# LiangZhaoPKUImperial/LinearSFM

Measured on AMD Instinct MI355X. Metric: hierarchical linear map-joining solve wall-clock, NC3500-like stereo (all transforms + joins), lower is better.
Workload: dtype f64

## Files before the change

### linearsfm_amd/csrc/lsfm_chol.hip

```cpp
#include <algorithm>
#include <climits>
#include <cmath>
#include <cstdlib>
#include <numeric>

#include "lsfm_device.hpp"
#include "lsfm_symbolic.hpp"
#include "lsfm_chol.hpp"

namespace lsfm {

#define FX_ONE 0x1p61
#define FX_INV 0x1p-61
__device__ __forceinline__ long long fx_from(double v) { return __double2ll_rn(fmin(fmax(v, -2.0), 2.0) * FX_ONE); }
__device__ __forceinline__ double fx_to(long long a) { return (double)a * FX_INV; }
__device__ __forceinline__ void fx_atomic_sub(double* slot, double t)
{
	__hip_atomic_fetch_add(reinterpret_cast<unsigned long long*>(slot), (unsigned long long)fx_from(-t), __ATOMIC_RELAXED, __HIP_MEMORY_SCOPE_AGENT);
}
__device__ __forceinline__ int scale_exp(double d)
{
	if (!(d > 0) || !(d < 1e300)) return 0;
	return (__builtin_amdgcn_frexp_exp(d) + 1) >> 1;
}
// ... 1076 lines not shown
	{
		const int k0 = 6 * t;
		if (tid >= k0 && tid < k0 + 6) sA[tid - k0] = acc;
		__syncthreads();
		if (tid >= k0 && tid < k0 + 6)
		{
			const int c = tid - k0;
			double x = 0.0;
			for (int k = c; k < 6; k++) x = fma(sDi[t * 36 + k * 6 + c], sA[k], x);
			sX[tid] = x;
		}
		__syncthreads();
		if (tid < k0)
		{
#pragma unroll
			for (int k = 0; k < 6; k++) acc = fma(-Ls[(k0 + k) * SN_XS + tid], sX[k0 + k], acc);
		}
	}
	if (tid < n6) v[(size_t)c0 * 6 + tid] = sX[tid];
}

__global__ void k_to_float(size_t n, const double* __restrict__ a, float* __restrict__ b)
{
	size_t i = (size_t)blockIdx.x * blockDim.x + threadIdx.x;
	if (i < n) b[i] = (float)a[i];
}

__global__ void k_perm_in(int M, const int* __restrict__ perm, const double* __restrict__ r, const unsigned char* __restrict__ fixed,
                          const double* __restrict__ dscale, double* __restrict__ v, int zero_from)
{
	size_t i = (size_t)blockIdx.x * blockDim.x + threadIdx.x;
	if (i >= (size_t)M * 6) return;
	const size_t src = (size_t)perm[i / 6] * 6 + i % 6;
	v[i] = ((fixed && fixed[src]) || (long)(i / 6) >= (long)zero_from) ? 0.0 : r[src] * dscale[i];
}
__global__ void k_perm_out_dot(int M, const int* __restrict__ pinv, const double* __restrict__ v, const double* __restrict__ r,
                               const unsigned char* __restrict__ fixed, const double* __restrict__ dscale, const int* __restrict__ pose_seg,
                               double* __restrict__ z, double* dot, int dot_stride, const int* __restrict__ col_owner, int rank)
{
	int row = blockIdx.x * blockDim.x + threadIdx.x;
	const bool ok = row < M;
	double acc = 0;
	int sg = 0;
	if (ok)
	{
		sg = pose_seg[row];
		const double* src = v + (size_t)pinv[row] * 6;
		const double* sc = dscale + (size_t)pinv[row] * 6;
		for (int i = 0; i < 6; i++)
		{
			double zz = src[i] * sc[i];
			if (fixed && fixed[(size_t)row * 6 + i]) zz = 0.0;
			if (col_owner) { const int ow = col_owner[pinv[row]]; if (!(ow == rank || (ow < 0 && rank == 0))) zz = 0.0; }
			z[(size_t)row * 6 + i] = zz;
			acc = fma(zz, r[(size_t)row * 6 + i], acc);
		}
	}
	if (dot) wave_scatter_add<1>(dot + (size_t)sg * dot_stride, &acc, ok);
}
__global__ void k_rz_dot(int M, const double* __restrict__ z, const double* __restrict__ r, const int* __restrict__ pose_seg, double* dot, int dot_stride)
{
	int row = blockIdx.x * blockDim.x + threadIdx.x;
	const bool ok = row < M;
	double acc = 0;
	int sg = 0;
	if (ok)
	{
		sg = pose_seg[row];
		for (int i = 0; i < 6; i++) acc = fma(z[(size_t)row * 6 + i], r[(size_t)row * 6 + i], acc);
	}
	wave_scatter_add<1>(dot + (size_t)sg * dot_stride, &acc, ok);
}

void chol_fetch(lsfm_context* ctx, const SchurSystem& sy, const int* d_origin, CholHostIn& in)
{
	const int M = sy.M, nnzb = sy.nnzb;
	in.keys.resize(nnzb);
	in.origin.resize(M);
	if (d_origin) LSFM_CHECK_HIP(hipMemcpyAsync(in.origin.data(), d_origin, (size_t)M * sizeof(int), hipMemcpyDeviceToHost, ctx->stream));
	else std::iota(in.origin.begin(), in.origin.end(), 0);
	d2h(ctx, in.keys.data(), sy.upper_keys, (size_t)nnzb * sizeof(unsigned long long));
}

void chol_alloc_values(lsfm_context* ctx, CholDev& ch)
{
	Arena& sc = ctx->scratch;
	ch.L = sc.alloc<double>((size_t)ch.nnzL * 36); ch.Dinv = sc.alloc<double>((size_t)ch.M * 36);
	ch.wv = sc.alloc<double>((size_t)ch.M * 6);
	ch.diag0 = sc.alloc<double>((size_t)ch.M * 6);
	ch.dscale = sc.alloc<double>((size_t)ch.M * 6);
	ch.Lg = ch.ngroups ? sc.alloc<double>((size_t)ch.nnzL * 36) : nullptr;
	dev_zero(ctx, ch.L, (size_t)ch.nnzL * 36 * sizeof(double));
	static const bool digest = getenv("LSFM_FACTOR_DIGEST") != nullptr;
	if (digest && ch.Lg) dev_zero(ctx, ch.Lg, (size_t)ch.nnzL * 36 * sizeof(double));
	ch.d_err = sc.alloc<int>(1);
	dev_zero(ctx, ch.d_err, sizeof(int));
}

static size_t chol_task_lds(const CholDev& ch) { return (size_t)ch.task0_maxsize * CHOL_TASK_LDS_PER_COL + 8; }
void chol_upload_index(lsfm_context* ctx, const CholSymbolic& sym, CholDev& ch)
{
	Arena& sc = ctx->scratch;
	ch.M = sym.M; ch.nnzL = sym.nnzL; ch.nlevels = sym.nlevels; ch.tail_begin = sym.tail_begin;
	ch.level_ptr = sym.level_ptr;
	if (!sym.tlevel_ptr.empty())
	{
		ch.ntask0 = sym.tlevel_ptr[1]; ch.ncol0 = sym.tlevel_col0[1];
		ch.task0_maxsize = sym.tlevel_maxsize[0]; ch.task0_lds = sym.tlevel_small_lds[0]; ch.task0_outer = sym.tlevel_outer[0];
		if (sym.tlevel_nsmall[0] != ch.ntask0 || chol_task_lds(ch) > CHOL_SOLVE_LDS)
			LSFM_FAIL(LSFM_ERR_INTERNAL, "a leaf task of the factorisation does not fit LDS (" + std::to_string(sym.tlevel_nsmall[0]) + " of " + std::to_string(ch.ntask0) +
			                                 " fit, " + std::to_string(ch.task0_maxsize) + " columns at most)");
	}
	ch.ngroups = sym.ngroups; ch.glevel_ptr = sym.glevel_ptr; ch.glevel_maxnr = sym.glevel_maxnr; ch.glevel_maxs = sym.glevel_maxs;
	ch.work_total = sym.work_total; ch.work_shared = sym.work_shared;
	ch.first_shared = sym.first_shared; ch.shared_blk0 = sym.colptr[sym.first_shared]; ch.glevel_owned = sym.glevel_owned; ch.glevel_shared = sym.glevel_shared;
	const struct { int** dst; const std::vector<int>* v; } parts[] = {
		{ &ch.grp_c0, &sym.grp_c0 }, { &ch.grp_s, &sym.grp_s }, { &ch.grp_nr, &sym.grp_nr }, { &ch.col_nin, &sym.col_nin }, { &ch.col_task, &sym.col_task },
		{ &ch.col_lpos, &sym.col_lpos }, { &ch.task_cols, &sym.task_cols }, { &ch.task_ptr, &sym.task_ptr }, { &ch.colptr, &sym.colptr },
		{ &ch.rowidx, &sym.rowidx }, { &ch.perm, &sym.perm }, { &ch.pinv, &sym.pinv }, { &ch.order, &sym.order }, { &ch.col_owner, &sym.col_owner } };
	size_t total = 0;
	for (const auto& pt : parts) total += pt.v->size();
	static thread_local std::vector<int> blob;
	blob.resize(total);
	int* d_blob = sc.alloc<int>(total);
	size_t off = 0;
	for (const auto& pt : parts)
	{
		if (!pt.v->empty()) memcpy(blob.data() + off, pt.v->data(), pt.v->size() * sizeof(int));
		*pt.dst = pt.v->empty() ? nullptr : d_blob + off;
		off += pt.v->size();
	}
	h2d(ctx, d_blob, blob.data(), total * sizeof(int));
	ch.blob = d_blob; ch.blob_ints = total;
}
void chol_upload_symbolic(lsfm_context* ctx, const CholSymbolic& sym, CholDev& ch)
{
	chol_upload_index(ctx, sym, ch);
	chol_alloc_values(ctx, ch);
	if (getenv("LSFM_DEBUG") && sym.ngroups > 50)
	{
		int hist[CHOL_GS + 1] = { 0 };
		for (int g = 0; g < sym.ngroups; g++) hist[sym.grp_s[g]]++;
		fprintf(stderr, "[lsfm] groups %d, group levels %d, sizes:", sym.ngroups, (int)sym.glevel_ptr.size() - 1);
		for (int q = 1; q <= CHOL_GS; q++) fprintf(stderr, " %d", hist[q]);
		fprintf(stderr, " | groups per level:");
		for (size_t l = 0; l + 1 < sym.glevel_ptr.size(); l++) fprintf(stderr, " %d", sym.glevel_ptr[l + 1] - sym.glevel_ptr[l]);
		fprintf(stderr, "\n");
	}
}
void chol_analyse(lsfm_context* ctx, const SchurSystem& sy, const CholHostIn& in, CholDev& ch)
{
	static thread_local CholSymbolic sym;
	chol_symbolic(in.keys.data(), sy.nnzb, in.origin.data(), sy.M, sym, ctx->comm ? ctx->comm->block_maps : 0);
	chol_upload_symbolic(ctx, sym, ch);
}

bool chol_distributed(const lsfm_context* ctx, const CholDev& ch)
{
	return ctx->comm && ctx->comm->world > 1 && ch.col_owner && ch.first_shared < ch.M;
}
static void comm_sum(lsfm_context* ctx, void* p, size_t count, int dtype)
{
	if (!count) return;
	Comm& cm = *ctx->comm;
	const size_t mk = cm.off;
	void* b = cm.alloc_bytes(count * 8);
	LSFM_CHECK_HIP(hipMemcpyAsync(b, p, count * 8, hipMemcpyDeviceToDevice, ctx->stream));
	cm.allreduce(ctx->stream, b, count, dtype);
	LSFM_CHECK_HIP(hipMemcpyAsync(p, b, count * 8, hipMemcpyDeviceToDevice, ctx->stream));
	cm.off = mk;
}
void comm_sum_host(lsfm_context* ctx, long long* h, int n)
{
	hipStream_t s = ctx->stream;
	Comm& cm = *ctx->comm;
	const size_t mk = cm.off;
	long long* d = cm.alloc<long long>(n);
	LSFM_CHECK_HIP(hipMemcpyAsync(d, h, n * sizeof(long long), hipMemcpyHostToDevice, s));
	LSFM_CHECK_HIP(hipStreamSynchronize(s));
// ... 226 lines not shown
```

### linearsfm_amd/csrc/lsfm_chol.hpp

```cpp
#pragma once
#include <vector>

#include "lsfm_internal.hpp"
#include "lsfm_solve.hpp"

namespace lsfm {

struct CholDev {
	int M = 0, nnzL = 0, nlevels = 0, tail_begin = 0;
	int* colptr = nullptr;
	int* rowidx = nullptr;
	int* perm = nullptr;
	int* pinv = nullptr;
	int* order = nullptr;
	std::vector<int> level_ptr;
	int* task_cols = nullptr;
	int* task_ptr = nullptr;
	int* col_task = nullptr;
	int* col_lpos = nullptr;
	int* col_nin = nullptr;
	int ntask0 = 0, ncol0 = 0;
	int task0_maxsize = 0;
	int task0_lds = 0;
	int task0_outer = 0;
	int ngroups = 0;
	int *grp_c0 = nullptr, *grp_s = nullptr, *grp_nr = nullptr;
	std::vector<int> glevel_ptr;
	std::vector<int> glevel_maxnr;
	std::vector<int> glevel_maxs;
	int sn_fused_levels = 0, sn_split_levels = 0;
	int* col_owner = nullptr;
	int first_shared = 0, shared_blk0 = 0;
	double work_total = 0, work_shared = 0;
	std::vector<char> glevel_owned, glevel_shared;
	int* blob = nullptr;
	size_t blob_ints = 0;
	float *Lf = nullptr, *Dinvf = nullptr;
	double* wv = nullptr;
	double* Lg = nullptr;
	float* Lgf = nullptr;
	double* L = nullptr;
	double* Dinv = nullptr;
	double* diag0 = nullptr;
	double* dscale = nullptr;
	int* d_err = nullptr;
};

struct OwnFilter {
	const int* col_owner = nullptr;
	int want = 0;
	__device__ __forceinline__ bool skip(int col) const { return col_owner && col_owner[col] != want; }
};
__device__ __forceinline__ int find_row(const int* __restrict__ rowidx, int lo, int hi, int target)
{
	while (lo < hi) { int mid = (lo + hi) >> 1; if (rowidx[mid] < target) lo = mid + 1; else hi = mid; }
	return lo;
}


struct CholSymbolic;
struct CholHostIn {
	std::vector<unsigned long long> keys;
	std::vector<int> origin;
};

void chol_fetch(lsfm_context* ctx, const SchurSystem& sy, const int* d_origin, CholHostIn& in);
void chol_analyse(lsfm_context* ctx, const SchurSystem& sy, const CholHostIn& in, CholDev& ch);
void chol_upload_index(lsfm_context* ctx, const CholSymbolic& sym, CholDev& ch);
void chol_upload_symbolic(lsfm_context* ctx, const CholSymbolic& sym, CholDev& ch);
void chol_alloc_values(lsfm_context* ctx, CholDev& ch);
void chol_scatter(lsfm_context* ctx, const SchurSystem& sy, const unsigned char* fixed, CholDev& ch);
void chol_factor(lsfm_context* ctx, const SchurSystem& sy, const unsigned char* fixed, CholDev& ch, double* fwd_v = nullptr);
void chol_merge_groups(lsfm_context* ctx, const CholDev& ch);
void chol_round_to_float(lsfm_context* ctx, CholDev& ch);
void chol_perm_in(lsfm_context* ctx, const CholDev& ch, const double* r, const unsigned char* fixed, double* v);
void chol_apply(lsfm_context* ctx, const CholDev& ch, const double* r, double* v, double* z, const unsigned char* fixed, const int* pose_seg, double* dot, int dot_stride, bool fwd_done = false);
bool chol_distributed(const lsfm_context* ctx, const CholDev& ch);
void comm_sum_host(lsfm_context* ctx, long long* h, int n);

}
```

### linearsfm_amd/csrc/lsfm_internal.hpp

```cpp
#pragma once
#include <hip/hip_runtime.h>

#include <cstdint>
#include <cstdio>
#include <condition_variable>
#include <cstring>
#include <exception>
#include <functional>
#include <memory>
#include <mutex>
#include <thread>
#include <string>
#include <vector>

#include "../../include/lsfm.h"

namespace lsfm {

struct Error { int code; std::string msg; };
struct DevBatch;
struct IndexHold;
struct SolvePlan;
struct PreLevel;
struct EarlyPattern;
// ... 131 lines not shown
			th = std::thread([this] {
				std::unique_lock<std::mutex> lk(m);
				for (;;)
				{
					cv.wait(lk, [&] { return quit || (busy && job); });
					if (quit) return;
					std::function<void()> j = std::move(job);
					job = nullptr;
					lk.unlock();
					std::exception_ptr e;
					try { j(); } catch (...) { e = std::current_exception(); }
					lk.lock();
					err = e; busy = false;
					cv.notify_all();
				}
			});
		cv.notify_all();
	}
	void wait()
	{
		std::unique_lock<std::mutex> l(m);
		cv.wait(l, [&] { return !busy; });
		if (err) { std::exception_ptr e = err; err = nullptr; std::rethrow_exception(e); }
	}
};

}

namespace lsfm {
struct Roctx {
	int (*push)(const char*) = nullptr;
	int (*pop)() = nullptr;
	void (*mark)(const char*) = nullptr;
	Roctx();
};
Roctx& roctx();
struct Range {
	bool on;
	explicit Range(const char* name) : on(roctx().push != nullptr) { if (on) roctx().push(name); }
	~Range() { if (on) roctx().pop(); }
	Range(const Range&) = delete;
	Range& operator=(const Range&) = delete;
};
}

struct lsfm_context {
	int device = 0;
	hipStream_t stream = nullptr;
	lsfm::Arena arena[3];
	lsfm::Arena scratch;
	int cur = 0;
	size_t arena_bytes = 0, arena_req = 0;
	lsfm::PcgOptions pcg;
	int covcols_panel = 0;
	int small_max = 5;
	std::string last_error;
	int* h_pinned = nullptr;
	char* h_stage = nullptr;
	char* d_stage = nullptr;
	size_t stage_size = 0, stage_off = 0;
	hipEvent_t ev_half[2] = { nullptr, nullptr };
	hipEvent_t ev0 = nullptr, ev1 = nullptr, ev2 = nullptr, ev3 = nullptr;
	hipEvent_t evs[4] = { nullptr, nullptr, nullptr, nullptr };
	unsigned long long generation = 0;
	hipStream_t stream2 = nullptr;
	hipEvent_t evA = nullptr, evB = nullptr;
	bool pattern_dep = false;
	const lsfm::DevBatch* tr_in = nullptr;
	const int* tr_hub = nullptr;
	std::shared_ptr<lsfm::EarlyPattern> early;
	hipEvent_t ev_k9[2] = { nullptr, nullptr };
	hipStream_t stream3 = nullptr;
	lsfm::Arena sarena[2];
	std::shared_ptr<lsfm::PreLevel> pre;
	lsfm::LevelPlan pre_plan;
	int pre_plan_level = -1;
	std::unique_ptr<lsfm::HostWorker> worker;
	void drop_prepared() { pre.reset(); pre_plan = lsfm::LevelPlan(); pre_plan_level = -1; }
	hipEvent_t ev_solve_end = nullptr;
	double dbg_gap_ms = 0.0;
	hipEvent_t evY = nullptr, evP = nullptr;
	hipEvent_t evU = nullptr;
	hipEvent_t evK = nullptr;
	const unsigned long long* solved_keys = nullptr;
	int solved_nnzb = 0;
	std::vector<std::pair<const char*, double>> timeline;
	bool timeline_on = false;
	void mark(const char* what);
	bool in_tree_run = false;
	int inject_level = -1;
	bool level_syncs = false;
	int step_hint = 0, steps_used = 0;
	hipEvent_t evC = nullptr;
	lsfm_stats* stats = nullptr;
	lsfm::LevelPlan* plan = nullptr;
	bool warm() const { return plan && plan->valid; }
	lsfm::RunStatsDev* d_run = nullptr;
	lsfm::Comm* comm = nullptr;
	std::vector<hipEvent_t> ev_pool;
	size_t ev_next = 0;
	struct Timed { hipEvent_t a, b; double* sink; };
	std::vector<Timed> timed;
	hipEvent_t pool_event();
	void defer_time(hipEvent_t a, hipEvent_t b, double* sink) { timed.push_back(Timed{ a, b, sink }); }
	void flush_times();
	void ensure_arenas(size_t bytes_each, bool start_small = false);
	bool grow_arenas();
	bool arena_small = false;
	size_t arena_bound = 0;
};

namespace lsfm {

struct OnStream {
	lsfm_context* c; hipStream_t& s; Arena* a;
	OnStream(lsfm_context* ctx, hipStream_t& other, Arena* arena = nullptr) : c(ctx), s(other), a(arena) { std::swap(c->stream, s); if (a) std::swap(c->scratch, *a); }
	~OnStream() { if (a) std::swap(c->scratch, *a); std::swap(c->stream, s); }
	OnStream(const OnStream&) = delete;
	OnStream& operator=(const OnStream&) = delete;
};

void dev_exclusive_scan(lsfm_context* ctx, const int* in, int* out, size_t n);
void dev_sort_pairs_u64(lsfm_context* ctx, unsigned long long* keys, int* vals, size_t n, int end_bit, int begin_bit = 0);
void dev_sort_keys_u64(lsfm_context* ctx, const unsigned long long* keys, unsigned long long* sorted, size_t n, int begin_bit, int end_bit);
int d2h_int(lsfm_context* ctx, const int* dptr);
void d2h_ints(lsfm_context* ctx, const int* dptr, int* h, size_t n);
void h2d(lsfm_context* ctx, void* d, const void* h, size_t bytes);
struct HostPiece { const void* p; size_t bytes; };
void h2d_gather(lsfm_context* ctx, void* d, const std::vector<HostPiece>& pieces);
struct CopyBatch {
	lsfm_context* ctx;
	struct Item { void* dst; const void* src; size_t bytes; bool host; };
	std::vector<Item> items;
	explicit CopyBatch(lsfm_context* c) : ctx(c) {}
	void h2d(void* d, const void* h, size_t bytes) { if (bytes) items.push_back(Item{ d, h, bytes, true }); }
	void d2d(void* d, const void* s, size_t bytes) { if (bytes) items.push_back(Item{ d, s, bytes, false }); }
	void flush();
};
void d2h(lsfm_context* ctx, void* h, const void* d, size_t bytes);
void dev_zero(lsfm_context* ctx, void* d, size_t bytes);
void fill_async(hipStream_t s, void* d, int byte, size_t bytes);

void batch_upload(lsfm_context* ctx, Arena& ar, const lsfm_map* maps, int N, bool mono, DevBatch& out);
void batch_download_map(lsfm_context* ctx, const DevBatch& b, int k, bool mono, lsfm_map* out);
template <class T> inline T* host_alloc(size_t n) { return static_cast<T*>(malloc((n ? n : 1) * sizeof(T))); }
struct CopyBatch;
void batch_set_offsets(lsfm_context* ctx, Arena& ar, DevBatch& b, CopyBatch* cb = nullptr);
void batch_fill_maps(lsfm_context* ctx, DevBatch& b);
struct PackHeader {
	int magic, version, mono, m, n, nU, nW, Ref, FRef, ScaP, Fix, Sign, FScaP, FFix, pad0, pad1;
	unsigned long long total;
	unsigned long long off[12];
	unsigned long long pad[11];
};
static_assert(sizeof(PackHeader) == 256, "the header is the first 256 bytes of a pack");
#define LSFM_PACK_MAGIC 0x4d46534c
size_t pack_layout(PackHeader& h);
void batch_pack_map(lsfm_context* ctx, const DevBatch& b, int k, bool mono, void* dst, size_t cap);
void batch_slice_counts(lsfm_context* ctx, const DevBatch& b, int nslices, std::vector<int>& nf, std::vector<int>& nw);
void batch_pack_slice(lsfm_context* ctx, const DevBatch& b, bool mono, int nslices, int slice, int nf, int nw, void* dst, size_t cap);
void batch_unpack_maps(lsfm_context* ctx, Arena& ar, const void* const* packed, const PackHeader* hdr, int N, bool mono, DevBatch& out);
unsigned long long batch_structure_digest(lsfm_context* ctx, const DevBatch& b);

inline bool map_in_frame(const DevBatch& X, int b, int tref, int tscap, bool mono) { return X.Ref[b] == tref && (!mono || X.ScaP[b] == tscap); }
int level_targets(const DevBatch& X, bool mono, std::vector<int>& tref, std::vector<int>& tscap, std::vector<int>& tfix);
struct TrRedirect {
	const int* wbase = nullptr;
	const int* newf = nullptr;
	double* W = nullptr;
	int *photo = nullptr, *feature = nullptr, *srcf = nullptr;
};
void transform_batch(lsfm_context* ctx, Arena& ar, const DevBatch& in, const std::vector<int>& target_ref,
                     const std::vector<int>& target_scap, const std::vector<int>& target_fix, bool mono, DevBatch& out,
                     bool alias_passthrough = false, const std::function<TrRedirect(DevBatch&)>* hook = nullptr);

struct JoinWork;
void join_batch_stereo(lsfm_context* ctx, Arena& ar, const DevBatch& in, DevBatch& out, double* eP_out, double* eF_out);
void join_batch_mono(lsfm_context* ctx, Arena& ar, const DevBatch& in, DevBatch& out, double* eP_out, double* eF_out);

struct SolveIO {
	int M = 0, NF = 0, NU = 0, NW = 0, nseg = 0;
	const int* d_pose_seg = nullptr;
	const int* d_feat_seg = nullptr;
	const unsigned char* d_seg_active = nullptr;
	const double* U = nullptr; const int *Ui = nullptr, *Uj = nullptr;
	const double* W = nullptr; const int *photo = nullptr, *fptr = nullptr;
	const double* V = nullptr;
	const double* ea = nullptr;
	const double* eb = nullptr;
	const double* x0 = nullptr;
	const unsigned char* d_fixed = nullptr;
	const int* d_pose_origin = nullptr;
	double* x_pose = nullptr;
	double* x_feat = nullptr;
	std::vector<int> seg_rows;
	const int *d_pose_off = nullptr, *d_feat_off = nullptr, *d_u_off = nullptr;
	const struct RhsFused* rhs = nullptr;
	const struct PatternSeed* seed = nullptr;
};
int small_level_strips(const lsfm_context* ctx, int most_rows);
inline int most_rows(const std::vector<int>& seg_rows) { int most = 0; for (int r : seg_rows) most = r > most ? r : most; return most; }
inline int small_level_strips(const lsfm_context* ctx, const std::vector<int>& seg_rows) { return small_level_strips(ctx, most_rows(seg_rows)); }
void small_level_offsets(lsfm_context* ctx, const DevBatch& out, SolveIO& io);
void small_solve_launch(lsfm_context* ctx, const SolveIO& io, int strips, int* status, double* max_rel);
int solve_batch(lsfm_context* ctx, const SolveIO& io);
int gn_polish(lsfm_context* ctx, const lsfm_map* maps, int N, bool mono, lsfm_map* x, int iters, int kind, double c, double* obj, double* gnorm,
              int* halvings, double* chi2, double* weight);
int map_chi2(lsfm_context* ctx, const lsfm_map* maps, int N, bool mono, const lsfm_map* x, double* chi2, int* dof);
int gn_linearise(lsfm_context* ctx, const lsfm_map* maps, int N, bool mono, const lsfm_map* x, const double* weight, lsfm_map* out, double* obj,
                 double* b, double* times, int* counts);
int map_covariance(lsfm_context* ctx, const lsfm_map* map, bool mono, double* pose_cov, double* feat_cov, double* pair_cov, int cap_blocks, int* nnzb,
                   double* times);
int map_covariance_columns(lsfm_context* ctx, const lsfm_map* map, bool mono, const int* poses, int k, double* pose_cols, double* feat_cols, double* joint,
                           int* steps, double* last_corr, double* times);
int inverse_v(lsfm_context* ctx, double* V, int n);
int solve_features(lsfm_context* ctx, const double* W, const double* IV, const double* eb, const double* dpa, double* dpb, int m, int n, const int* mapCor,
                   const int* photo);
bool no_timing_events();
#define LSFM_REC_T(e, s) do { if (!lsfm::no_timing_events()) LSFM_CHECK_HIP(hipEventRecord(e, s)); } while (0)
unsigned timing_event_flags();
unsigned order_event_flags();
void prefetch_next_level(lsfm_context* ctx, const DevBatch& Y, const std::vector<int>& target_ref, int next_level, int step_hint);
int spmv_external(lsfm_context* ctx, int m, const int* rowptr, const int* colidx, const double* val, const double* x, double* y, int reps,
                  double* avg_ms, double* bytes);
int chol_selftest(lsfm_context* ctx, int m, const int* rowptr, const int* colidx, const double* val, const int* origin, const unsigned char* fixed,
                  const int* pose_seg, int nseg, const double* r, int nrhs, int mode, double* z, double* dot, int* perm, int* colptr, int* rowidx,
                  double* L, double* Dinv, double* dscale, int cap_blocks, int* info);

int wstream_bench(lsfm_context* ctx, long long nblocks, int mode, int reps, double* avg_ms);
int prims_selftest(lsfm_context* ctx, int cases, unsigned seed);
}
```

### linearsfm_amd/csrc/lsfm_join.hip

```cpp
#include "lsfm_device.hpp"
#include "lsfm_internal.hpp"
#include <climits>
#include "lsfm_join.hpp"
#include "lsfm_solve.hpp"

namespace lsfm {

__device__ __forceinline__ unsigned long long jh_mix(unsigned long long x)
{
	x ^= x >> 33; x *= 0xff51afd7ed558ccdull; x ^= x >> 33; x *= 0xc4ceb9fe1a85ec53ull; x ^= x >> 33;
	return x;
}
__global__ void k_join_hash_insert(int NF, const int* __restrict__ feat_id, const int* __restrict__ feat_map, unsigned long long* tab,
                                   int* __restrict__ tval, unsigned long long mask)
{
	int f = blockIdx.x * blockDim.x + threadIdx.x;
	if (f >= NF) return;
	const int mp = feat_map[f];
	if (mp & 1) return;
	const unsigned long long key = ((unsigned long long)(mp >> 1) << 32) | (unsigned)feat_id[f];
	unsigned long long h = jh_mix(key) & mask;
	for (;;)
	{
		const unsigned long long old = atomicCAS(&tab[h], ~0ull, key);
// ... 275 lines not shown
		const int nun = pair ? rb[b + 1] - rb[b] : 0;
		out.feat_off[g + 1] = jg.FY0 + jg.nE + nun;
		out.pose_off[g] = in.pose_off[a]; out.u_off[g] = in.u_off[a]; out.w_off[g] = in.w_off[a];
		out.Ref[g] = pair ? in.Ref[b] : in.Ref[a];
		out.FRef[g] = in.FRef[a];
		seg_active[g] = pair ? 1 : 0;
		seg_rows[g] = (pair ? in.pose_off[b + 1] : in.pose_off[a + 1]) - in.pose_off[a];
	}
	out.pose_off[G] = in.M; out.u_off[G] = in.NU; out.w_off[G] = in.NW;
	out.NF = out.feat_off[G];
	const int NFY = out.NF;

	CopyBatch cb(ctx);
	JGroup* d_grp = ctx->scratch.alloc<JGroup>(G);
	cb.h2d(d_grp, grp.data(), sizeof(JGroup) * G);

	out.pose = ar.alloc<double>((size_t)in.M * 6);
	out.pose_id = ar.alloc<int>(in.M);
	out.pose_origin = ar.alloc<int>(in.M);
	cb.d2d(out.pose_origin, in.pose_origin, (size_t)in.M * sizeof(int));
	out.feat = ar.alloc<double>((size_t)NFY * 3);
	out.feat_id = ar.alloc<int>(NFY);
	out.U = ar.alloc<double>((size_t)in.NU * 36); out.Ui = ar.alloc<int>(in.NU); out.Uj = ar.alloc<int>(in.NU);
	out.W = ar.alloc<double>((size_t)in.NW * 18); out.photo = ar.alloc<int>(in.NW); out.feature = ar.alloc<int>(in.NW);
	out.fptr = ar.alloc<int>(NFY + 1);
	out.V = ar.alloc<double>((size_t)NFY * 9);
	batch_set_offsets(ctx, ar, out, &cb);
	cb.d2d(out.pose_id, in.pose_id, (size_t)in.M * sizeof(int));
	st.d_act = reinterpret_cast<unsigned char*>(ctx->scratch.alloc<int>((G + 3) / 4 + 1));
	st.act_padded.assign(((size_t)G + 3) / 4 * 4, 0);
	std::copy(seg_active.begin(), seg_active.end(), st.act_padded.begin());
	cb.h2d(st.d_act, st.act_padded.data(), st.act_padded.size());
	cb.flush();
	batch_fill_maps(ctx, out);
	int* newf = st.newf = ctx->scratch.alloc<int>(in.NF + 1);
	int* lens = ctx->scratch.alloc<int>(NFY + 2);
	st.srcf = ctx->scratch.alloc<int>(in.NW + 1);
	int* lenE = st.lenE = ctx->scratch.alloc<int>(NFY + 1);
	int* lenC = ctx->scratch.alloc<int>(NFY + 1);
	double* eF = st.eF = ctx->scratch.alloc<double>((size_t)NFY * 3);
	double* eP = st.eP = ctx->scratch.alloc<double>((size_t)in.M * 6);
	dev_zero(ctx, eP, (size_t)in.M * 6 * sizeof(double));
	const bool small_level = small_level_strips(ctx, seg_rows) > 0;
	const bool early = !small_level && !ctx->comm && !(ctx->pre && !ctx->pre_plan.valid) && ctx->tr_in && ctx->tr_hub && !ctx->warm() && ctx->tr_in->NF == in.NF && ctx->tr_in->M == in.M;
	st.fuse_rhs = !small_level && !ctx->comm && !ctx->pcg.mixed;
	int *srcE = nullptr, *srcC = nullptr;
	if (early || st.fuse_rhs)
	{
		srcE = ctx->scratch.alloc<int>(NFY + 1); srcC = ctx->scratch.alloc<int>(NFY + 1);
	}
	st.srcE = srcE; st.srcC = srcC;
	if (in.NF)
		for (int side = 0; side < 2; side++)
			hipLaunchKernelGGL(k_join_features, dim3(nb), dim3(256), 0, s, in.NF, in.feat_map, in.feat_id, in.feat, in.V, in.fptr, match, R, d_grp,
			                   newf, lenE, lenC, out.V, eF, out.feat_id, out.feat, srcE, srcC, side);
	if (early)
	{
		const DevBatch& X = *ctx->tr_in;
		EarlyPatternIn ei;
		ei.M = in.M; ei.NFY = NFY; ei.NU = X.NU;
		ei.Ui = X.Ui; ei.Uj = X.Uj; ei.pose_map = X.pose_map; ei.hub = ctx->tr_hub;
		ei.fptr = X.fptr; ei.photo = X.photo; ei.feat_map = X.feat_map; ei.srcE = srcE; ei.srcC = srcC;
		LSFM_CHECK_HIP(hipEventRecord(ctx->evC, s));
		schur_pattern_early_issue(ctx, ei);
	}
	else schur_pattern_early_drop(ctx);
	hipLaunchKernelGGL(k_add_lens, dim3((NFY + 256) / 256), dim3(256), 0, s, NFY, lenE, lenC, lens);
	dev_exclusive_scan(ctx, lens, out.fptr, NFY);
	if (early) LSFM_CHECK_HIP(hipEventRecord(ctx->evC, s));
	st.wbase = ctx->scratch.alloc<int>(in.NF + 1);
	if (in.NF) hipLaunchKernelGGL(k_join_wbase, dim3(nb), dim3(256), 0, s, in.NF, in.feat_map, newf, lenE, out.fptr, st.wbase);
	LSFM_CHECK_HIP(hipGetLastError());
	ctx->mark("jn_prep");
}

void join_stereo_finish(lsfm_context* ctx, const DevBatch& in, DevBatch& out, JoinState& st, double* eP_out, double* eF_out)
{
	hipStream_t s = ctx->stream;
	const int G = out.B, NFY = out.NF;
	double *eP = st.eP, *eF = st.eF;
	int* srcf = st.srcf;
	const std::vector<unsigned char>& seg_active = st.seg_active;
	const std::vector<int>& seg_rows = st.seg_rows;
	if (in.NU)
	{
		CopyBatch cu(ctx);
		cu.d2d(out.U, in.U, (size_t)in.NU * 36 * sizeof(double));
		cu.d2d(out.Ui, in.Ui, (size_t)in.NU * sizeof(int));
		cu.d2d(out.Uj, in.Uj, (size_t)in.NU * sizeof(int));
		cu.flush();
	}
	LSFM_CHECK_HIP(hipEventRecord(ctx->evY, s));
	if (!eP_out && !eF_out && !ctx->early && !ctx->comm)
	{
		LSFM_CHECK_HIP(hipEventRecord(ctx->evA, s));
		ctx->pattern_dep = true;
	}
	const bool fuse_rhs = st.fuse_rhs && !eP_out && !eF_out;
	if (NFY && !fuse_rhs)
		hipLaunchKernelGGL(k_join_rhs_w, dim3((NFY + RHS_TILE - 1) / RHS_TILE), dim3(256), 0, s, NFY, out.fptr, out.W, out.photo, srcf, in.pose, in.feat, eP, eF);
	if (in.NU && (!ctx->comm || ctx->comm->rank == 0))
		hipLaunchKernelGGL(k_join_rhs_u, dim3((in.NU + 127) / 128), dim3(128), 0, s, in.NU, in.U, in.Ui, in.Uj, in.pose, eP);
	LSFM_CHECK_HIP(hipGetLastError());
	if (eP_out) d2h(ctx, eP_out, eP, (size_t)in.M * 6 * sizeof(double));
	if (eF_out) d2h(ctx, eF_out, eF, (size_t)NFY * 3 * sizeof(double));

	unsigned char* d_act = st.d_act;
	SolveIO io;
	io.M = in.M; io.NF = NFY; io.NU = in.NU; io.NW = in.NW; io.nseg = G;
	io.d_pose_seg = out.pose_map; io.d_feat_seg = out.feat_map; io.d_seg_active = d_act;
	io.U = out.U; io.Ui = out.Ui; io.Uj = out.Uj; io.W = out.W; io.photo = out.photo; io.fptr = out.fptr; io.V = out.V;
	io.ea = eP; io.eb = eF; io.x0 = in.pose; io.d_fixed = nullptr; io.d_pose_origin = out.pose_origin;
	io.x_pose = out.pose; io.x_feat = out.feat;
	io.seg_rows = seg_rows;
	RhsFused rhs;
	if (fuse_rhs)
	{
		rhs.srcE = st.srcE; rhs.srcC = st.srcC; rhs.feat_src = in.feat; rhs.pose_src = in.pose; rhs.pose_map_src = in.pose_map;
		io.rhs = &rhs;
	}
	small_level_offsets(ctx, out, io);
	const bool warm = ctx->warm();
	ctx->solved_keys = nullptr; ctx->solved_nnzb = 0;
	int rc = solve_batch(ctx, io);
	if (!warm && !ctx->in_tree_run) LSFM_CHECK_HIP(hipStreamSynchronize(s));
	ctx->scratch.release(st.smark);
	if (rc > 0 && ctx->stats) ctx->stats->not_converged += rc;
	if (ctx->plan && !eP_out && !eF_out) ctx->plan->valid = true;
}

void join_batch_stereo(lsfm_context* ctx, Arena& ar, const DevBatch& in, DevBatch& out, double* eP_out, double* eF_out)
{
	JoinState st;
	join_stereo_prepare(ctx, ar, in, out, st);
	if (in.NW)
		hipLaunchKernelGGL(k_join_wcopy, dim3((in.NW + 255) / 256), dim3(256), 0, ctx->stream, in.NW, in.W, in.photo, in.feature, in.fptr, st.wbase,
		                   st.newf, out.W, out.photo, out.feature, st.srcf, in.W_alias, in.d_alias, in.feat_map);
	join_stereo_finish(ctx, in, out, st, eP_out, eF_out);
}

}
```

### linearsfm_amd/csrc/lsfm_level.hip

```cpp
#include <algorithm>
#include <chrono>
#include <cmath>
#include <cstdlib>

#include "lsfm_device.hpp"
#include "lsfm_symbolic.hpp"
#include "lsfm_pcg.hpp"

namespace lsfm {

struct SolvePlan {
	SchurSystem sy;
	CholDev ch;
	int its = 1;
	bool mixed = false;
	double rel_tol = 0;
	bool small = false;
	char* mem = nullptr;
	~SolvePlan() { if (mem) (void)hipFree(mem); }
};
static std::shared_ptr<SolvePlan> solve_plan_store(lsfm_context* ctx, const SchurSystem& sy, const CholDev& ch, int its)
{
	auto sp = std::make_shared<SolvePlan>();
	const size_t M = sy.M, nnzb = sy.nnzb, cap = (size_t)sy.mask + 1;
// ... 93 lines not shown
		PreLevel* raw = pl.get();
		ctx->worker->run([raw]() { chol_symbolic(raw->hin.keys.data(), raw->sy.nnzb, raw->hin.origin.data(), raw->sy.M, raw->sym); });
		pl->worker = ctx->worker.get();
		ctx->mark("pre_sym");
		pl->whole = whole; pl->level = next_level; pl->its = step_hint;
		ctx->pre = pl;
	}
	if (!whole) return;
	const int B = Y.B;
	ctx->pre_plan.tr_cnt.assign(counts.begin(), counts.begin() + 2 * (B + 1));
	ctx->pre_plan.join_rb.assign(counts.begin() + 2 * (B + 1), counts.end());
	ctx->pre_plan.solve.reset();
	ctx->pre_plan.idx = kept;
	ctx->pre_plan.valid = true;
	ctx->pre_plan_level = next_level;
	ctx->mark("pre_plan");
}
static std::shared_ptr<SolvePlan> pre_plan_complete(lsfm_context* ctx, PreLevel& pl)
{
	pl.wait();
	auto sp = std::make_shared<SolvePlan>();
	sp->sy = pl.sy;
	sp->its = pl.its; sp->mixed = ctx->pcg.mixed; sp->rel_tol = ctx->pcg.rel_tol;
	{
		OnStream on(ctx, ctx->stream3, &ctx->sarena[pl.level & 1]);
		chol_upload_index(ctx, pl.sym, sp->ch);
		LSFM_CHECK_HIP(hipEventRecord(ctx->evP, ctx->stream));
	}
	LSFM_CHECK_HIP(hipStreamWaitEvent(ctx->stream, ctx->evP, 0));
	return sp;
}

__global__ void k_dbg_absstats(size_t n, const double* __restrict__ a, double* __restrict__ out)
{
	double s = 0.0, m = 0.0;
	for (size_t i = (size_t)blockIdx.x * blockDim.x + threadIdx.x; i < n; i += (size_t)gridDim.x * blockDim.x)
	{
		const double v = fabs(a[i]);
		s += v; if (v > m || !(v == v)) m = v == v ? v : 1e300;
	}
	atomic_add_f64(out, s);
	atomicMax(reinterpret_cast<unsigned long long*>(out + 1), (unsigned long long)__double_as_longlong(m));
}
__global__ void k_dbg_dinv(int M, const double* __restrict__ Dinv, const double* __restrict__ diag0, const int* __restrict__ colptr, int first_group_col)
{
	int j = blockIdx.x * blockDim.x + threadIdx.x;
	if (j >= M) return;
	double m = 0.0;
	for (int q = 0; q < 36; q++) m = fmax(m, fabs(Dinv[(size_t)j * 36 + q]));
	if (m > 1e3 || !(m == m))
		printf("[lsfm conv] column %d (%s, %d blocks): max |Dinv| %.3e, Dinv diag %.3e %.3e %.3e %.3e %.3e %.3e, diag0 %.3e %.3e %.3e %.3e %.3e %.3e\n", j,
		       j >= first_group_col ? "group" : "leaf", colptr[j + 1] - colptr[j], m, Dinv[(size_t)j * 36], Dinv[(size_t)j * 36 + 7], Dinv[(size_t)j * 36 + 14],
		       Dinv[(size_t)j * 36 + 21], Dinv[(size_t)j * 36 + 28], Dinv[(size_t)j * 36 + 35], diag0[j * 6], diag0[j * 6 + 1], diag0[j * 6 + 2], diag0[j * 6 + 3],
		       diag0[j * 6 + 4], diag0[j * 6 + 5]);
}
__global__ void k_digest(size_t n, const unsigned long long* __restrict__ a, unsigned long long* out)
{
	unsigned long long h = 0;
	for (size_t i = (size_t)blockIdx.x * blockDim.x + threadIdx.x; i < n; i += (size_t)gridDim.x * blockDim.x)
	{
		unsigned long long b = a[i];
		if (b == 0x8000000000000000ull) b = 0;
		b ^= b >> 31; b *= 0x9E3779B97F4A7C15ull * (2 * (unsigned long long)i + 1); b ^= b >> 29;
		h += b;
	}
	atomicAdd(out, h);
}
__global__ void k_digest_compare(const unsigned long long* d, int* mismatch)
{
	if (d[0] != d[1]) atomicAdd(mismatch, 1);
}
__global__ void k_chol_err_to_run(const int* err, RunStatsDev* run)
{
	if (*err && !run->chol_err) run->chol_err = *err;
}

struct LevelStructure {
	SchurSystem sy;
	CholDev ch;
	SolvePlan* sp = nullptr;
	double tw0 = 0, tw1 = 0;
};
static double wall_ms() { return std::chrono::duration<double, std::milli>(std::chrono::steady_clock::now().time_since_epoch()).count(); }
static LevelStructure level_structure(lsfm_context* ctx, const SolveIO& io, SolvePlan* sp, PreLevel* pre, bool pending, hipEvent_t eb)
{
	hipStream_t s = ctx->stream;
	LevelStructure ls;
	SchurSystem& sy = ls.sy;
	CholDev& ch = ls.ch;
	const bool pattern_dep = ctx->pattern_dep;
	ctx->pattern_dep = false;
	auto assemble = [&]() {
		build_schur_values(ctx, io, sy);
		LSFM_REC_T(eb, s); if (roctx().mark) roctx().mark("lsfm factor + refine: begin");
		LSFM_CHECK_HIP(hipEventRecord(ctx->evK, s));
	};
	if (sp || pending)
	{
		sy = pending ? pre->sy : sp->sy;
		schur_vinv(ctx, io, sy);
		assemble();
		if (pending)
		{
			ctx->mark("k9_enq");
			ctx->plan->solve = pre_plan_complete(ctx, *pre);
			sp = ctx->plan->solve.get();
			ctx->mark("sym_wait");
		}
		ls.sp = sp;
		ch = sp->ch;
		chol_alloc_values(ctx, ch);
		return ls;
	}
	schur_vinv(ctx, io, sy);
	CholHostIn hin;
	bool have = false;
	if (pre && !(pre->M == io.M && !ctx->comm)) pre = nullptr;
	if (pre)
	{
		schur_pattern_early_drop(ctx);
		SchurSystem prepared = pre->sy;
		prepared.IV = sy.IV; prepared.LY = sy.LY; prepared.ymax = sy.ymax; prepared.uu = sy.uu;
		sy = prepared;
		have = true;
		LSFM_CHECK_HIP(hipStreamWaitEvent(s, ctx->evP, 0));
		if (getenv("LSFM_CHECK_EARLY_PATTERN")) schur_pattern_check(ctx, io, sy, "prefetched");
	}
	else if (ctx->early && !ctx->comm)
	{
		LSFM_CHECK_HIP(hipStreamWaitEvent(ctx->stream3, ctx->evC, 0));
		{
			OnStream on(ctx, ctx->stream3);
			ctx->mark("sv_start");
			have = schur_pattern_early_finish(ctx, io, sy);
			ctx->mark("pat_fin");
			if (have)
			{
				if (getenv("LSFM_CHECK_EARLY_PATTERN")) schur_pattern_check(ctx, io, sy, "early");
				chol_fetch(ctx, sy, io.d_pose_origin, hin);
				ctx->mark("fetch");
				schur_pattern_early_extras(ctx, sy);
				LSFM_CHECK_HIP(hipEventRecord(ctx->evB, ctx->stream));
			}
		}
		if (have) LSFM_CHECK_HIP(hipStreamWaitEvent(s, ctx->evB, 0));
	}
	else if (pattern_dep && !ctx->comm)
	{
		LSFM_CHECK_HIP(hipStreamWaitEvent(ctx->stream2, ctx->evA, 0));
		{
			OnStream on(ctx, ctx->stream2);
			build_schur_pattern(ctx, io, sy);
			chol_fetch(ctx, sy, io.d_pose_origin, hin);
			LSFM_CHECK_HIP(hipEventRecord(ctx->evB, ctx->stream));
		}
		LSFM_CHECK_HIP(hipStreamWaitEvent(s, ctx->evB, 0));
		have = true;
	}
	if (!have)
	{
		build_schur_pattern(ctx, io, sy);
		chol_fetch(ctx, sy, io.d_pose_origin, hin);
	}
	assemble();
	ls.tw0 = wall_ms();
	ctx->mark("k9_enq");
	if (pre) { pre->wait(); chol_upload_symbolic(ctx, pre->sym, ch); }
	else chol_analyse(ctx, sy, hin, ch);
	ctx->mark("analyse");
	ls.tw1 = wall_ms();
	return ls;
}

static int solve_level_dense(lsfm_context* ctx, const SolveIO& io, int strips, bool warm, hipEvent_t eb, hipEvent_t ec, hipEvent_t ed)
{
	hipStream_t s = ctx->stream;
	LevelPlan* lp = ctx->plan;
	ctx->pattern_dep = false;
	if (!warm) schur_pattern_early_drop(ctx);
	int* d_small = nullptr;
	auto enqueue = [&]() {
		d_small = ctx->scratch.alloc<int>(4);
		dev_zero(ctx, d_small, 4 * sizeof(int));
		hipEvent_t esm0 = nullptr, esm1 = nullptr;
		if (ctx->stats) { esm0 = ctx->pool_event(); esm1 = ctx->pool_event(); LSFM_REC_T(esm0, s); }
		small_solve_launch(ctx, io, strips, d_small, reinterpret_cast<double*>(d_small + 2));
		if (ctx->stats) { LSFM_REC_T(esm1, s); ctx->defer_time(esm0, esm1, &ctx->stats->t_small_ms); ctx->stats->small_levels++; }
	};
	if (!warm) enqueue();
	LSFM_REC_T(eb, s); if (warm && roctx().mark) roctx().mark("lsfm factor + refine: begin");
	LSFM_CHECK_HIP(hipEventRecord(ctx->evK, s));
	if (warm) enqueue();
	LSFM_REC_T(ec, s);
	LSFM_REC_T(ed, s); if (roctx().mark) roctx().mark("lsfm solve: end");
	ctx->ev_solve_end = ed;
	ctx->solved_keys = nullptr; ctx->solved_nnzb = 0;
	if (ctx->stats) ctx->stats->pcg_iterations += 1;
	ctx->steps_used = 1;
	const bool deferred = ctx->in_tree_run && ctx->d_run && (warm || !lp || lp == &ctx->pre_plan);
	if (deferred) return 0;
// ... 6 lines not shown
	if (lp && !lp->solve && hs[0] == 0)
	{
		auto small_plan = std::make_shared<SolvePlan>();
		small_plan->its = 1; small_plan->mixed = false; small_plan->rel_tol = ctx->pcg.rel_tol; small_plan->small = true;
		lp->solve = small_plan;
	}
	return hs[0];
}

static void factor_digest_check(lsfm_context* ctx, const SolveIO& io, const SchurSystem& sy, CholDev& ch)
{
	static const bool digest = getenv("LSFM_FACTOR_DIGEST") != nullptr;
	if (!digest || !ctx->d_run) return;
	hipStream_t s = ctx->stream;
	Arena& sc = ctx->scratch;
	const int M = io.M;
	auto dg = [&](const double* a, size_t n, unsigned long long* out) {
		if (a && n) hipLaunchKernelGGL(k_digest, dim3(256), dim3(256), 0, s, n, reinterpret_cast<const unsigned long long*>(a), out);
	};
	dg(sy.S, (size_t)sy.nnzb * 36, &ctx->d_run->s_digest);
	if (!ctx->comm)
	{
		SchurSystem sy2 = sy;
		build_schur_values(ctx, io, sy2);
		unsigned long long* d = sc.alloc<unsigned long long>(2);
		dev_zero(ctx, d, 2 * sizeof(unsigned long long));
		dg(sy.S, (size_t)sy.nnzb * 36, d); dg(sy.E, (size_t)M * 6, d);
		dg(sy2.S, (size_t)sy.nnzb * 36, d + 1); dg(sy2.E, (size_t)M * 6, d + 1);
		hipLaunchKernelGGL(k_digest_compare, dim3(1), dim3(1), 0, s, d, &ctx->d_run->s_rebuild_mismatch);
	}
	auto factor_digest = [&](unsigned long long* out) {
		dg(ch.Dinv, (size_t)ch.M * 36, out);
		dg(ch.L, (size_t)ch.nnzL * 36, out);
		if (ch.Lg) dg(ch.Lg, (size_t)ch.nnzL * 36, out);
	};
	factor_digest(&ctx->d_run->factor_digest);
	if (!ctx->comm)
	{
		unsigned long long* d = sc.alloc<unsigned long long>(2);
		dev_zero(ctx, d, 2 * sizeof(unsigned long long));
		factor_digest(d);
		dev_zero(ctx, ch.L, (size_t)ch.nnzL * 36 * sizeof(double));
		if (ch.Lg) dev_zero(ctx, ch.Lg, (size_t)ch.nnzL * 36 * sizeof(double));
		chol_scatter(ctx, sy, io.d_fixed, ch);
		chol_factor(ctx, sy, io.d_fixed, ch, nullptr);
		factor_digest(d + 1);
		hipLaunchKernelGGL(k_digest_compare, dim3(1), dim3(1), 0, s, d, &ctx->d_run->refactor_mismatch);
	}
}

static void debug_conv(lsfm_context* ctx, const SolveIO& io, const SchurSystem& sy, const CholDev& ch, const PcgSeg* seg)
{
	hipStream_t s = ctx->stream;
	const int M = io.M;
	hipLaunchKernelGGL(k_pcg_debug, dim3((io.nseg + 127) / 128), dim3(128), 0, s, io.nseg, M, seg);
	if (!(M > 10000 && io.nseg == 1)) return;
	double* d = ctx->scratch.alloc<double>(12);
	dev_zero(ctx, d, 12 * sizeof(double));
	auto st = [&](const double* a, size_t n, int k) { if (a && n) hipLaunchKernelGGL(k_dbg_absstats, dim3(512), dim3(256), 0, s, n, a, d + 2 * k); };
	st(sy.S, (size_t)sy.nnzb * 36, 0); st(sy.E, (size_t)M * 6, 1); st(ch.L, (size_t)ch.nnzL * 36, 2); st(ch.Lg, (size_t)ch.nnzL * 36, 3);
	st(ch.Dinv, (size_t)ch.M * 36, 4); st(io.x_pose, (size_t)M * 6, 5);
	hipLaunchKernelGGL(k_dbg_dinv, dim3((ch.M + 255) / 256), dim3(256), 0, s, ch.M, ch.Dinv, ch.diag0, ch.colptr, 0);
	double h[12];
	d2h(ctx, h, d, sizeof h);
	fprintf(stderr, "[lsfm conv] root M=%d: |S| sum %.15e max %.6e  |E| sum %.15e  |L| sum %.12e max %.3e  |Lg| sum %.12e max %.3e  |Dinv| sum %.6e max %.3e  |x| sum %.12e max %.3e\n",
	        M, h[0], h[1], h[2], h[4], h[5], h[6], h[7], h[8], h[9], h[10], h[11]);
}

int solve_batch(lsfm_context* ctx, const SolveIO& io)
{
	hipStream_t s = ctx->stream;
	const int M = io.M;
	LevelPlan* lp = ctx->plan;
	const int strips = (io.d_pose_off && io.d_feat_off && io.d_u_off) ? small_level_strips(ctx, io.seg_rows) : 0;
	SolvePlan* sp = lp ? lp->solve.get() : nullptr;
	if (sp && sp->small != (strips > 0)) { lp->solve.reset(); sp = nullptr; }
	std::shared_ptr<PreLevel> pre = std::move(ctx->pre);
	const bool pending = !strips && !sp && pre && pre->whole && lp == &ctx->pre_plan;
	if (pre && !pending && (strips || sp || pre->whole || pre->M != M || ctx->comm)) pre.reset();
	const bool warm = sp != nullptr || pending;
	hipEvent_t ea = ctx->pool_event(), eb = ctx->pool_event(), ec = ctx->pool_event(), ed = ctx->pool_event();
	LSFM_REC_T(ea, s); if (roctx().mark) roctx().mark("lsfm schur: begin");
	if (strips) return solve_level_dense(ctx, io, strips, warm, eb, ec, ed);
	LevelStructure ls = level_structure(ctx, io, sp, pre.get(), pending, eb);
	pre.reset();
	const SchurSystem& sy = ls.sy;
	CholDev& ch = ls.ch;
	sp = ls.sp;
	const bool dbg = getenv("LSFM_DEBUG") != nullptr;
	PcgWork w = pcg_begin(ctx, io, sy, ch);
	if (ctx->stats && chol_distributed(ctx, ch)) { ctx->stats->dist_solves++; ctx->stats->dist_work_total += ch.work_total; ctx->stats->dist_work_shared += ch.work_shared; }
	chol_scatter(ctx, sy, io.d_fixed, ch);
	if (w.fused_fwd) chol_perm_in(ctx, ch, w.r, io.d_fixed, w.v);
	chol_factor(ctx, sy, io.d_fixed, ch, w.fused_fwd ? w.v : nullptr);
	if (ctx->pcg.mixed) chol_round_to_float(ctx, ch);
	factor_digest_check(ctx, io, sy, ch);
	if (dbg) { LSFM_CHECK_HIP(hipStreamSynchronize(s)); }
	const double tw2 = wall_ms();
	const bool deferred = warm || (ctx->in_tree_run && ctx->d_run && !lp);
	ctx->solved_keys = sy.upper_keys; ctx->solved_nnzb = sy.nnzb;
	const PcgSteps steps{ warm, deferred, sp ? sp->its : 0, sp ? sp->mixed : false, sp ? sp->rel_tol : 0.0 };
	const PcgResult res = pcg_run(ctx, io, sy, ch, w, steps);
	if (dbg)
	{
		LSFM_CHECK_HIP(hipStreamSynchronize(s));
		fprintf(stderr, "[lsfm] solve M=%d nseg=%d nnzb=%d nnzL=%d etree levels=%d tail=%d leaf tasks=%d group levels=%d %s| analyse %.2f ms, factor %.2f ms, cg(%d its) %.2f ms\n", M, io.nseg,
		        sy.nnzb, ch.nnzL, ch.nlevels, ch.M - ch.tail_begin, ch.ntask0, (int)ch.glevel_ptr.size() - 1, warm ? "(plan) " : "", ls.tw1 - ls.tw0, tw2 - ls.tw1, res.its, wall_ms() - tw2);
	}
	if (ctx->comm)
	{
		Comm& cm = *ctx->comm;
		const size_t nscal = (size_t)M * 6;
		double *x = io.x_pose, *xb = cm.alloc<double>(nscal);
		if (cm.rank == 0) LSFM_CHECK_HIP(hipMemcpyAsync(xb, x, nscal * sizeof(double), hipMemcpyDeviceToDevice, s));
		else fill_async(s, xb, 0, nscal * sizeof(double));
		cm.allreduce(s, xb, nscal, LSFM_DTYPE_F64);
		LSFM_CHECK_HIP(hipMemcpyAsync(x, xb, nscal * sizeof(double), hipMemcpyDeviceToDevice, s));
	}
	pcg_final_residual(ctx, io, sy, w);
	LSFM_REC_T(ec, s); if (roctx().mark) roctx().mark("lsfm back-substitution: begin");
	launch_backsub(ctx, io, sy, io.x_pose);
	LSFM_CHECK_HIP(hipGetLastError());
	LSFM_REC_T(ed, s); if (roctx().mark) roctx().mark("lsfm solve: end");
	ctx->ev_solve_end = ed;
	if (ctx->stats)
	{
		lsfm_stats* st = ctx->stats;
		ctx->defer_time(ea, eb, &st->t_schur_ms);
		ctx->defer_time(eb, ec, &st->t_pcg_ms);
		ctx->defer_time(ec, ed, &st->t_backsub_ms);
		ctx->defer_time(w.es0, w.es1, &st->spmv_ms);
		st->pcg_iterations += res.its;
		st->spmv_launches += 1;
		st->spmv_bytes += spmv_bytes(sy);
		st->spmv_nnzb_upper_last = sy.nnzb; st->spmv_rows_last = M;
	}
	ctx->steps_used = res.planned ? 0 : std::max(res.its, 1);
	if (deferred)
	{
		if (warm && !res.planned) { sp->its = std::max(res.its, 1); sp->mixed = ctx->pcg.mixed; sp->rel_tol = ctx->pcg.rel_tol; }
		static const bool dbg_conv = getenv("LSFM_DEBUG_CONV") != nullptr;
		if (dbg_conv) debug_conv(ctx, io, sy, ch, w.seg);
		hipLaunchKernelGGL(k_pcg_run_stats, dim3((io.nseg + 127) / 128), dim3(128), 0, s, io.nseg, w.seg, ctx->d_run);
		return 0;
	}
	double maxrel = 0;
	int notconv = pcg_read_verdict(ctx, io, w, &maxrel);
	if (ctx->stats) ctx->stats->max_rel_residual = std::max(ctx->stats->max_rel_residual, maxrel);
	if (ctx->comm)
	{
		long long hv[2] = { notconv, 0 };
		comm_sum_host(ctx, hv, 2);
		notconv = (int)((hv[0] + ctx->comm->world - 1) / ctx->comm->world);
	}
	if (lp && !lp->solve && notconv == 0) lp->solve = solve_plan_store(ctx, sy, ch, std::max(res.its, 1));
	return notconv;
}

}
```

### linearsfm_amd/csrc/lsfm_pcg.hip

```cpp
#include <algorithm>
#include <cmath>
#include <cstdlib>

#include "lsfm_device.hpp"
#include "lsfm_pcg.hpp"

namespace lsfm {

struct PcgSeg {
	double rz[2];
	double pAp;
	double rr, ee, thresh, rr_prev;
	int done, its, row0, active;
	int slow, pad;
};
static_assert(sizeof(PcgSeg) % sizeof(double) == 0, "PcgSeg is strided in doubles by the fused dot products");
#define SEG_STRIDE ((int)(sizeof(PcgSeg) / sizeof(double)))

__global__ void k_x_init(int M, const double* __restrict__ x0, const unsigned char* __restrict__ fixed, double* __restrict__ x, double* __restrict__ y, int* __restrict__ misc)
{
	size_t i = (size_t)blockIdx.x * blockDim.x + threadIdx.x;
	if (i < 4) misc[i] = 0;
	if (i >= (size_t)M * 6) return;
	y[i] = 0.0;
// ... 45 lines not shown
__global__ void k_copy(size_t n, const double* __restrict__ a, double* __restrict__ b)
{
	size_t i = (size_t)blockIdx.x * blockDim.x + threadIdx.x;
	if (i < n) b[i] = a[i];
}

__global__ void k_pcg_update1(int M, int cur, const int* __restrict__ pose_seg, double* __restrict__ x, const double* __restrict__ p,
                              double* __restrict__ y, const PcgSeg* __restrict__ seg)
{
	int row = blockIdx.x * blockDim.x + threadIdx.x;
	if (row >= M) return;
	const PcgSeg& g = seg[pose_seg[row]];
	for (int i = 0; i < 6; i++) y[(size_t)row * 6 + i] = 0.0;
	if (g.done) return;
	const double alpha = g.rz[cur] / g.pAp;
	for (int i = 0; i < 6; i++) { const size_t o = (size_t)row * 6 + i; x[o] += alpha * p[o]; }
}

__global__ void k_pcg_update2(int M, int cur, const double* __restrict__ z, const int* __restrict__ pose_seg, double* __restrict__ p,
                              double* __restrict__ Ap, PcgSeg* seg, int* ndone)
{
	int row = blockIdx.x * blockDim.x + threadIdx.x;
	if (row >= M) return;
	const int sg = pose_seg[row];
	PcgSeg& g = seg[sg];
	const bool done = g.done;
	const double rzn = g.rz[cur ^ 1], rzc = g.rz[cur];
	for (int i = 0; i < 6; i++) Ap[(size_t)row * 6 + i] = 0.0;
	if (!done)
	{
		const double beta = rzn / rzc;
		for (int i = 0; i < 6; i++) { const size_t o = (size_t)row * 6 + i; p[o] = z[o] + beta * p[o]; }
	}
}
__global__ void k_pcg_check(int nseg, PcgSeg* seg, int* ndone)
{
	int s = blockIdx.x * blockDim.x + threadIdx.x;
	if (s >= nseg) return;
	PcgSeg& g = seg[s];
	if (g.done) return;
	const double rr = g.rr;
	g.its++;
	seg[nseg + s].rr = rr;
	const bool slow = !(rr < 0.25 * g.rr_prev);
	g.slow = slow ? g.slow + 1 : 0;
	if (!(rr > g.thresh) || !(rr == rr) || (slow && (!(rr > 1e-16 * g.ee) || g.slow >= 10))) { g.done = (rr == rr) ? 1 : 2; atomicAdd(ndone, 1); }
	g.rr_prev = rr;
}
__global__ void k_pcg_reset(int nseg, int cur, PcgSeg* seg)
{
	int s = blockIdx.x * blockDim.x + threadIdx.x;
	if (s >= nseg) return;
	PcgSeg& g = seg[s];
	if (g.done) return;
	g.pAp = 0; g.rr = 0; g.rz[cur] = 0;
}

__global__ void k_pcg_final_zero(int nseg, PcgSeg* fin)
{
	int s = blockIdx.x * blockDim.x + threadIdx.x;
	if (s < nseg) { fin[s].rr = 0.0; fin[s].ee = 0.0; }
}
__global__ void k_pcg_run_stats(int nseg, const PcgSeg* __restrict__ seg, RunStatsDev* run)
{
	int g = blockIdx.x * blockDim.x + threadIdx.x;
	if (g >= nseg || !seg[g].active) return;
	const PcgSeg& fin = seg[nseg + g];
	const double rel = fin.ee > 0 ? sqrt(fin.rr / fin.ee) : 0.0;
	if (!(rel < 1e-8) || (seg[g].done != 1 && !(rel < 1e-9))) atomicAdd(&run->not_converged, 1);
	if (seg[g].done == 0 && !(rel < 1e-10)) atomicAdd(&run->undone, 1);
	atomicMax(reinterpret_cast<unsigned long long*>(&run->max_rel_residual), (unsigned long long)__double_as_longlong(rel == rel ? rel : 1e300));
}
__global__ void k_pcg_debug(int nseg, int M, const PcgSeg* __restrict__ seg)
{
	int g = blockIdx.x * blockDim.x + threadIdx.x;
	if (g >= nseg || !seg[g].active) return;
	const PcgSeg& fin = seg[nseg + g];
	const double rel = fin.ee > 0 ? sqrt(fin.rr / fin.ee) : 0.0;
	if (!(rel < 1e-9))
		printf("[lsfm conv] M=%d nseg=%d system %d: rel %.3e its %d done %d slow %d rr_prev/ee %.3e thresh/ee %.3e ee %.3e pAp %.3e rz %.3e %.3e\n", M, nseg, g, rel, seg[g].its,
		       seg[g].done, seg[g].slow, seg[g].rr_prev / fin.ee, seg[g].thresh / fin.ee, fin.ee, seg[g].pAp, seg[g].rz[0], seg[g].rz[1]);
}

PcgWork pcg_begin(lsfm_context* ctx, const SolveIO& io, const SchurSystem& sy, const CholDev& ch)
{
	hipStream_t s = ctx->stream;
	Arena& sc = ctx->scratch;
	const int M = io.M, nseg = io.nseg;
	PcgWork w;
	w.d_misc = sc.alloc<int>(4);
	std::vector<PcgSeg> hseg(2 * (size_t)nseg);
	memset(hseg.data(), 0, sizeof(PcgSeg) * hseg.size());
	for (int g = 0, row = 0; g < nseg; g++) { hseg[g].row0 = hseg[nseg + g].row0 = row; row += io.seg_rows[g]; }
	w.seg = sc.alloc<PcgSeg>(hseg.size());
	h2d(ctx, w.seg, hseg.data(), sizeof(PcgSeg) * hseg.size());
	const size_t nscal = (size_t)M * 6;
	w.r = sc.alloc<double>(nscal); w.z = ctx->comm ? ctx->comm->alloc<double>(nscal) : sc.alloc<double>(nscal); w.p = sc.alloc<double>(nscal);
	w.Ap = sc.alloc<double>(nscal); w.v = sc.alloc<double>(nscal);
	const unsigned nbe = (unsigned)((nscal + 255) / 256);
	hipLaunchKernelGGL(k_x_init, dim3(std::max(1u, nbe)), dim3(256), 0, s, M, io.x0, io.d_fixed, io.x_pose, w.Ap, w.d_misc);
	launch_spmv(ctx, sy, io.x_pose, w.Ap, io.d_fixed, nullptr, nullptr, nullptr, 1);
	hipLaunchKernelGGL(k_pcg_resid, dim3((M + 127) / 128), dim3(128), 0, s, M, sy.E, w.Ap, io.d_pose_seg, io.d_fixed, w.r, w.seg, 1);
	static const bool no_fused_fwd = getenv("LSFM_NO_FUSED_FWD") != nullptr;
	w.fused_fwd = !ctx->pcg.mixed && !no_fused_fwd && ch.M > 0;
	return w;
}

PcgResult pcg_run(lsfm_context* ctx, const SolveIO& io, const SchurSystem& sy, const CholDev& ch, PcgWork& w, const PcgSteps& steps)
{
	hipStream_t s = ctx->stream;
	const int M = io.M, nseg = io.nseg;
	const size_t nscal = (size_t)M * 6;
	const int nbr = (M + 127) / 128, nbs = (nseg + 127) / 128;
	const unsigned nbe = (unsigned)((nscal + 255) / 256);
	double *x = io.x_pose, *r = w.r, *z = w.z, *p = w.p, *Ap = w.Ap, *v = w.v;
	PcgSeg* seg = w.seg;
	int* d_misc = w.d_misc;
	const bool mixed = ctx->pcg.mixed;
	chol_apply(ctx, ch, r, v, z, io.d_fixed, io.d_pose_seg, &seg[0].rz[0], SEG_STRIDE, w.fused_fwd);
	hipLaunchKernelGGL(k_copy, dim3(nbe), dim3(256), 0, s, nscal, z, p);
	const bool err_to_run = steps.deferred || (ctx->comm && ctx->d_run);
	hipLaunchKernelGGL(k_pcg_start, dim3(nbs), dim3(128), 0, s, nseg, seg, io.d_seg_active, ctx->pcg.rel_tol, d_misc + 1, ch.d_err, err_to_run ? ctx->d_run : (RunStatsDev*)nullptr);

	const int maxit = std::max(1, std::min(50, ctx->pcg.max_steps));
	const bool hinted = !steps.warm && steps.deferred && ctx->step_hint > 0 && ctx->step_hint <= maxit;
	const bool planned_run = hinted || (steps.warm && steps.mixed == mixed && steps.rel_tol == ctx->pcg.rel_tol && steps.its <= maxit);
	int its = 0, ndone = 0;
	w.es0 = ctx->pool_event(); w.es1 = ctx->pool_event();
	const bool ask_after = hinted && ctx->level_syncs && !ctx->comm;
	const int base_steps = hinted ? ctx->step_hint : (planned_run ? steps.its : maxit);
	const int planned = (planned_run && !ask_after && base_steps >= (mixed ? 3 : 2)) ? std::min(base_steps + 1, maxit) : base_steps;
	bool counting = planned_run;
	int cap = maxit;
	while ((counting ? its < planned : (ndone < nseg && its < cap)))
	{
		const int cur = its & 1;
		launch_spmv(ctx, sy, p, Ap, io.d_fixed, p, io.d_pose_seg, &seg[0].pAp, SEG_STRIDE);
		hipLaunchKernelGGL(k_pcg_update1, dim3(nbr), dim3(128), 0, s, M, cur, io.d_pose_seg, x, p, Ap, seg);
		if (!w.es_done) LSFM_REC_T(w.es0, s);
		launch_spmv(ctx, sy, x, Ap, io.d_fixed, nullptr, nullptr, nullptr, 1);
		if (!w.es_done) { LSFM_REC_T(w.es1, s); w.es_done = true; }
		hipLaunchKernelGGL(k_pcg_resid, dim3(nbr), dim3(128), 0, s, M, sy.E, Ap, io.d_pose_seg, io.d_fixed, r, seg, 0);
		hipLaunchKernelGGL(k_pcg_check, dim3(nbs), dim3(128), 0, s, nseg, seg, d_misc + 1);
		its++;
		if (counting)
		{
			if (its >= planned)
			{
				if (!ask_after) break;
				ndone = d2h_int(ctx, d_misc + 1);
				if (ndone >= nseg || its >= maxit) break;
				counting = false;
				cap = std::min(maxit, planned + 3);
			}
		}
		else
		{
			ctx->mark("cg_enq");
			ndone = d2h_int(ctx, d_misc + 1);
			ctx->mark("cg_sync");
			const int cerr = (its == 1 && !err_to_run) ? d2h_int(ctx, ch.d_err) : 0;
			if (cerr) LSFM_FAIL(LSFM_ERR_NOT_SPD, "Schur system is not positive definite (block column " + std::to_string(cerr - 1) + " of the factor)");
			if (ctx->comm && ctx->comm->world > 1)
			{
				long long more = ndone >= nseg ? 0 : 1;
				comm_sum_host(ctx, &more, 1);
				if (!more) break;
				ndone = std::min(ndone, nseg - 1);
			}
			else if (ndone >= nseg) break;
		}
		chol_apply(ctx, ch, r, v, z, io.d_fixed, io.d_pose_seg, &seg[0].rz[cur ^ 1], SEG_STRIDE);
		hipLaunchKernelGGL(k_pcg_update2, dim3(nbr), dim3(128), 0, s, M, cur, z, io.d_pose_seg, p, Ap, seg, d_misc + 1);
		hipLaunchKernelGGL(k_pcg_reset, dim3(nbs), dim3(128), 0, s, nseg, cur, seg);
	}
	return PcgResult{ its, planned_run };
}

void pcg_final_residual(lsfm_context* ctx, const SolveIO& io, const SchurSystem& sy, PcgWork& w)
{
	if (!ctx->comm && w.es_done) return;
	hipStream_t s = ctx->stream;
	const int M = io.M, nseg = io.nseg, nbr = (M + 127) / 128, nbs = (nseg + 127) / 128;
	PcgSeg* seg2 = w.seg + nseg;
	if (!w.es_done) LSFM_REC_T(w.es0, s);
	launch_spmv(ctx, sy, io.x_pose, w.Ap, io.d_fixed, nullptr, nullptr, nullptr, 1);
	if (!w.es_done) { LSFM_REC_T(w.es1, s); w.es_done = true; }
	hipLaunchKernelGGL(k_pcg_final_zero, dim3(nbs), dim3(128), 0, s, nseg, seg2);
	hipLaunchKernelGGL(k_pcg_resid, dim3(nbr), dim3(128), 0, s, M, sy.E, w.Ap, io.d_pose_seg, io.d_fixed, (double*)nullptr, seg2, 1);
}

int pcg_read_verdict(lsfm_context* ctx, const SolveIO& io, const PcgWork& w, double* maxrel)
{
	const int nseg = io.nseg;
	std::vector<PcgSeg> hs2(2 * (size_t)nseg);
	d2h(ctx, hs2.data(), w.seg, sizeof(PcgSeg) * 2 * nseg);
	int notconv = 0;
	*maxrel = 0;
	for (int g = 0; g < nseg; g++)
	{
		if (!hs2[g].active) continue;
		const PcgSeg& fin = hs2[nseg + g];
		const double rel = fin.ee > 0 ? sqrt(fin.rr / fin.ee) : 0.0;
// ... 8 lines not shown
```

### linearsfm_amd/csrc/lsfm_pcg.hpp

```cpp
#pragma once
#include "lsfm_chol.hpp"

namespace lsfm {

struct PcgSeg;

struct PcgWork {
	double *r = nullptr, *z = nullptr, *p = nullptr, *Ap = nullptr, *v = nullptr;
	PcgSeg* seg = nullptr;
	int* d_misc = nullptr;
	bool fused_fwd = false;
	hipEvent_t es0 = nullptr, es1 = nullptr;
	bool es_done = false;
};
struct PcgSteps { bool warm, deferred; int its; bool mixed; double rel_tol; };
struct PcgResult { int its; bool planned; };

PcgWork pcg_begin(lsfm_context* ctx, const SolveIO& io, const SchurSystem& sy, const CholDev& ch);
PcgResult pcg_run(lsfm_context* ctx, const SolveIO& io, const SchurSystem& sy, const CholDev& ch, PcgWork& w, const PcgSteps& steps);
void pcg_final_residual(lsfm_context* ctx, const SolveIO& io, const SchurSystem& sy, PcgWork& w);
__global__ void k_pcg_run_stats(int nseg, const PcgSeg* __restrict__ seg, RunStatsDev* run);
__global__ void k_pcg_debug(int nseg, int M, const PcgSeg* __restrict__ seg);
int pcg_read_verdict(lsfm_context* ctx, const SolveIO& io, const PcgWork& w, double* maxrel);

}
```

### linearsfm_amd/csrc/lsfm_prims.hip

```cpp
#include <dlfcn.h>
#include <algorithm>
#include <chrono>
#include <cstring>
#include <hip/hip_runtime.h>
#include <rocprim/rocprim.hpp>

#include "lsfm_internal.hpp"

namespace lsfm {

void Arena::init(size_t bytes)
{
	destroy();
	LSFM_CHECK_HIP(hipMalloc(&base, bytes));
	cap = bytes; off = 0; high = 0;
}
void Arena::destroy()
{
	if (base) (void)hipFree(base);
	base = nullptr; cap = off = 0;
}
__global__ void __launch_bounds__(256) k_fill_words(uint4* __restrict__ d16, size_t n16, unsigned* __restrict__ tail, int ntail, unsigned v)
{
	const size_t stride = (size_t)gridDim.x * blockDim.x;
// ... 246 lines not shown
			off += (it.bytes + 15) & ~(size_t)15;
		}
		else desc[i].src = (unsigned long long)(size_t)it.src;
	}
	if (!direct) LSFM_CHECK_HIP(hipMemcpyAsync(dev, slot, total, hipMemcpyHostToDevice, ctx->stream));
	const unsigned ny = (unsigned)std::min<size_t>(256, std::max<size_t>(1, most / (64 * 1024)));
	hipLaunchKernelGGL(k_copy_many, dim3((unsigned)items.size(), ny), dim3(256), 0, ctx->stream, reinterpret_cast<const CopyDesc*>(dev));
	items.clear();
}
void d2h(lsfm_context* ctx, void* h, const void* d, size_t bytes)
{
	if (bytes) LSFM_CHECK_HIP(hipMemcpyAsync(h, d, bytes, hipMemcpyDeviceToHost, ctx->stream));
	LSFM_CHECK_HIP(hipStreamSynchronize(ctx->stream));
}
void dev_zero(lsfm_context* ctx, void* d, size_t bytes)
{
	fill_async(ctx->stream, d, 0, bytes);
}

__global__ void k_comm_header(long long* h, long long failed, long long healthy, long long count, long long what)
{
	h[0] = failed; h[1] = healthy; h[2] = count; h[3] = what;
}
void Comm::allreduce(hipStream_t s, void* p, size_t count, int dtype, int kind)
{
	if (!count) return;
	if (broken) throw Error{ LSFM_ERR_INTERNAL, "the caller's all-reduce failed earlier in this run" };
	hipLaunchKernelGGL(k_comm_header, dim3(1), dim3(1), 0, s, reinterpret_cast<long long*>(buf), 0ll, 1ll, (long long)count, (long long)(dtype | (kind << 8)));
	call(s, 0, 4, LSFM_DTYPE_I64);
	call(s, (size_t)(static_cast<char*>(p) - buf), count, dtype);
}
bool Comm::follow(hipStream_t s)
{
	if (broken || !fn) return false;
	for (int guard = 0; guard < (1 << 20); guard++)
	{
		long long h[4] = { 0, 0, 0, 0 };
		hipLaunchKernelGGL(k_comm_header, dim3(1), dim3(1), 0, s, reinterpret_cast<long long*>(buf), 1ll, 0ll, 0ll, 0ll);
		call(s, 0, 4, LSFM_DTYPE_I64);
		LSFM_CHECK_HIP(hipMemcpyAsync(h, buf, sizeof h, hipMemcpyDeviceToHost, s));
		LSFM_CHECK_HIP(hipStreamSynchronize(s));
		if (h[1] <= 0) return false;
		const long long count = h[2] / h[1], what = h[3] / h[1];
		if ((what >> 8) == KIND_FINAL) return true;
		if (count <= 0 || HDR_BYTES + (size_t)count * 8 > cap) { broken = true; return false; }
		fill_async(s, buf + HDR_BYTES, 0, (size_t)count * 8);
		call(s, HDR_BYTES, (size_t)count, (int)(what & 0xff));
	}
	broken = true;
	return false;
}

}

namespace lsfm {
Roctx::Roctx()
{
	if (!getenv("LSFM_ROCTX")) return;
	for (const char* name : { "librocprofiler-sdk-roctx.so", "librocprofiler-sdk-roctx.so.1", "libroctx64.so", "libroctx64.so.4" })
	{
		void* h = dlopen(name, RTLD_NOW | RTLD_GLOBAL);
		if (!h) continue;
		push = reinterpret_cast<int (*)(const char*)>(dlsym(h, "roctxRangePushA"));
		pop = reinterpret_cast<int (*)()>(dlsym(h, "roctxRangePop"));
		mark = reinterpret_cast<void (*)(const char*)>(dlsym(h, "roctxMarkA"));
		if (push && pop) return;
		push = nullptr; pop = nullptr; mark = nullptr;
	}
	fprintf(stderr, "liblsfm_hip: LSFM_ROCTX is set but no roctx library could be loaded -- no ranges\n");
}
Roctx& roctx() { static Roctx r; return r; }
}

void lsfm_context::mark(const char* what)
{
	if (lsfm::roctx().mark) lsfm::roctx().mark(what);
	if (!timeline_on) return;
	timeline.emplace_back(what, std::chrono::duration<double, std::milli>(std::chrono::steady_clock::now().time_since_epoch()).count());
}
namespace lsfm {
bool no_timing_events() { static const bool v = getenv("LSFM_NO_TIMING_EVENTS") != nullptr; return v; }
unsigned timing_event_flags() { return hipEventDisableSystemFence; }
unsigned order_event_flags() { return hipEventDisableTiming | hipEventReleaseToDevice; }
}
hipEvent_t lsfm_context::pool_event()
{
	if (ev_next == ev_pool.size())
	{
		hipEvent_t e = nullptr;
		LSFM_CHECK_HIP(hipEventCreateWithFlags(&e, lsfm::timing_event_flags()));
		ev_pool.push_back(e);
	}
	return ev_pool[ev_next++];
}
void lsfm_context::flush_times()
{
	for (const Timed& t : timed)
	{
		float ms = 0;
		if (hipEventElapsedTime(&ms, t.a, t.b) == hipSuccess && t.sink) *t.sink += ms;
	}
	timed.clear();
	ev_next = 0;
	(void)hipGetLastError();
}

static void alloc_arenas(lsfm_context* c, size_t bytes_each)
{
	c->drop_prepared();
	c->early.reset(); c->solved_keys = nullptr; c->solved_nnzb = 0;
	c->arena[0].destroy(); c->arena[1].destroy(); c->arena[2].destroy(); c->scratch.destroy(); c->sarena[0].destroy(); c->sarena[1].destroy();
	c->pre.reset();
	c->arena[0].init(bytes_each);
	c->arena[1].init(bytes_each);
	c->arena[2].init(bytes_each);
	c->scratch.init(bytes_each);
	c->sarena[0].init(std::max<size_t>((size_t)96 << 20, bytes_each / 6));
	c->sarena[1].init(std::max<size_t>((size_t)96 << 20, bytes_each / 6));
	c->arena_bytes = bytes_each;
}
void lsfm_context::ensure_arenas(size_t bytes_each, bool start_small)
{
	generation++;
	if (arena[0].base && (arena_bytes >= bytes_each || (start_small && arena_req >= bytes_each))) return;
	LSFM_CHECK_HIP(hipDeviceSynchronize());
	const size_t requested = bytes_each;
	drop_prepared();
	arena[0].destroy(); arena[1].destroy(); arena[2].destroy(); scratch.destroy(); sarena[0].destroy(); sarena[1].destroy();
	size_t free_b = 0, total_b = 0;
	if (hipMemGetInfo(&free_b, &total_b) == hipSuccess && free_b > ((size_t)4 << 30))
		bytes_each = std::min(bytes_each, (free_b - ((size_t)2 << 30)) / 5);
	arena_bound = bytes_each;
	static const int div = getenv("LSFM_ARENA_DIV") ? std::max(1, atoi(getenv("LSFM_ARENA_DIV"))) : 8;
	arena_small = start_small && div > 1;
	static const size_t floor_b = (size_t)(getenv("LSFM_ARENA_MIN_MB") ? std::max(1, atoi(getenv("LSFM_ARENA_MIN_MB"))) : 1024) << 20;
	if (arena_small) bytes_each = std::min(bytes_each, std::max<size_t>(floor_b, bytes_each / div));
	alloc_arenas(this, bytes_each);
	arena_req = requested;
}
bool lsfm_context::grow_arenas()
{
	if (!arena_small || arena_bytes >= arena_bound) return false;
	(void)hipDeviceSynchronize();
	(void)hipGetLastError();
	alloc_arenas(this, std::min(arena_bound, 2 * arena_bytes));
	generation++;
	return true;
}

namespace lsfm {
int prims_selftest(lsfm_context* ctx, int cases, unsigned seed)
{
	ctx->ensure_arenas((size_t)64 << 20);
	ctx->scratch.reset();
	const size_t cap = (size_t)1 << 20;
	unsigned char* buf = ctx->scratch.alloc<unsigned char>(cap);
	std::vector<unsigned char> ref(cap), got(cap);
	unsigned long long st = seed * 2654435761ull + 12345ull;
	auto rnd = [&]() { st = st * 6364136223846793005ull + 1442695040888963407ull; return (unsigned)(st >> 33); };
	LSFM_CHECK_HIP(hipMemset(buf, 0xA5, cap));
	std::fill(ref.begin(), ref.end(), (unsigned char)0xA5);
	auto compare = [&](const char* what, int c) {
		d2h(ctx, got.data(), buf, cap);
		for (size_t i = 0; i < cap; i++)
			if (got[i] != ref[i])
				LSFM_FAIL(LSFM_ERR_INTERNAL, std::string("lsfm_selftest_prims: ") + what + " case " + std::to_string(c) + ": byte " + std::to_string(i) + " is " +
				                                 std::to_string(got[i]) + ", expected " + std::to_string(ref[i]));
	};
	for (int c = 0; c < cases; c++)
	{
		const size_t len = (c % 3 == 0) ? rnd() % 70 : rnd() % (cap / 2);
		const size_t off = rnd() % (cap - len);
		const int byte = (c % 4 == 0) ? 0 : (c % 4 == 1 ? 0xff : (int)(rnd() & 0xff));
		fill_async(ctx->stream, buf + off, byte, len);
		std::fill(ref.begin() + off, ref.begin() + off + len, (unsigned char)byte);
		if (c % 8 == 7 || c + 1 == cases) compare("fill", c);
	}
	std::vector<unsigned> src(cap / 4);
	for (unsigned& v : src) v = rnd();
	for (int c = 0; c < cases; c++)
	{
		const size_t nw = 1 + rnd() % (c % 2 ? 300 : 60000), offw = rnd() % (cap / 4 - nw), from = rnd() % (cap / 4 - nw);
		h2d(ctx, buf + 4 * offw, src.data() + from, 4 * nw);
		memcpy(ref.data() + 4 * offw, src.data() + from, 4 * nw);
		if (c % 8 == 7 || c + 1 == cases) compare("copy", c);
	}
	for (int c = 0; c < cases; c += 4)
	{
		CopyBatch cb(ctx);
		size_t at = 0;
		const size_t half = cap / 2;
		for (int i = 0; i < 5 && at + 70000 < half; i++)
		{
			const size_t nw = 4 * (1 + rnd() % 4000), from = rnd() % (cap / 4 - nw);
			if (i % 2 == 0) { cb.h2d(buf + at, src.data() + from, 4 * nw); memcpy(ref.data() + at, src.data() + from, 4 * nw); }
			else { cb.d2d(buf + at, buf + half + 4 * (from % (half / 4 - nw)), 4 * nw); memcpy(ref.data() + at, ref.data() + half + 4 * (from % (half / 4 - nw)), 4 * nw); }
			at += 4 * nw + 4 * (rnd() % 5);
		}
		cb.flush();
		compare("batch", c);
	}
	return LSFM_OK;
}
}

extern "C" {

int lsfm_context_create(int device, size_t arena_bytes, lsfm_context** out)
{
	if (!out) return LSFM_ERR_ARG;
	*out = nullptr;
	int ndev = 0;
	if (hipGetDeviceCount(&ndev) != hipSuccess || ndev <= 0 || device < 0 || device >= ndev)
	{
		fprintf(stderr, "liblsfm_hip: no usable HIP device (count=%d, requested %d) -- this library has no CPU path\n", ndev, device);
		return LSFM_ERR_NO_DEVICE;
	}
	lsfm_context* c = new lsfm_context();
	try
	{
		c->device = device;
		if (getenv("LSFM_SMALL_MAX")) c->small_max = std::max(0, std::min(16, atoi(getenv("LSFM_SMALL_MAX"))));
		LSFM_CHECK_HIP(hipSetDevice(device));
		LSFM_CHECK_HIP(hipStreamCreateWithFlags(&c->stream, hipStreamNonBlocking));
		LSFM_CHECK_HIP(hipStreamCreateWithFlags(&c->stream2, hipStreamNonBlocking));
		{
			int least = 0, greatest = 0;
			(void)hipDeviceGetStreamPriorityRange(&least, &greatest);
			LSFM_CHECK_HIP(hipStreamCreateWithPriority(&c->stream3, hipStreamNonBlocking, greatest));
		}
		for (auto& e : c->ev_k9) LSFM_CHECK_HIP(hipEventCreateWithFlags(&e, lsfm::order_event_flags()));
		LSFM_CHECK_HIP(hipEventCreateWithFlags(&c->evA, lsfm::order_event_flags()));
		LSFM_CHECK_HIP(hipEventCreateWithFlags(&c->evB, lsfm::order_event_flags()));
		LSFM_CHECK_HIP(hipEventCreateWithFlags(&c->evC, lsfm::order_event_flags()));
		LSFM_CHECK_HIP(hipEventCreateWithFlags(&c->evY, lsfm::order_event_flags()));
		LSFM_CHECK_HIP(hipEventCreateWithFlags(&c->evP, lsfm::order_event_flags()));
		LSFM_CHECK_HIP(hipEventCreateWithFlags(&c->evK, lsfm::order_event_flags()));
		LSFM_CHECK_HIP(hipEventCreateWithFlags(&c->evU, lsfm::order_event_flags()));
		LSFM_CHECK_HIP(hipHostMalloc((void**)&c->h_pinned, 4096));
		c->stage_size = (size_t)64 << 20;
		LSFM_CHECK_HIP(hipHostMalloc((void**)&c->h_stage, c->stage_size));
		{
			void* dp = nullptr;
			if (hipHostGetDevicePointer(&dp, c->h_stage, 0) == hipSuccess) c->d_stage = static_cast<char*>(dp);
			else (void)hipGetLastError();
		}
		LSFM_CHECK_HIP(hipEventCreateWithFlags(&c->ev0, lsfm::timing_event_flags()));
		LSFM_CHECK_HIP(hipEventCreateWithFlags(&c->ev1, lsfm::timing_event_flags()));
		LSFM_CHECK_HIP(hipEventCreateWithFlags(&c->ev2, lsfm::timing_event_flags()));
		LSFM_CHECK_HIP(hipEventCreateWithFlags(&c->ev3, lsfm::timing_event_flags()));
		for (auto& e : c->evs) LSFM_CHECK_HIP(hipEventCreateWithFlags(&e, lsfm::timing_event_flags()));
		LSFM_CHECK_HIP(hipMalloc((void**)&c->d_run, sizeof(lsfm::RunStatsDev)));
		LSFM_CHECK_HIP(hipMemset(c->d_run, 0, sizeof(lsfm::RunStatsDev)));
		if (arena_bytes) c->ensure_arenas(arena_bytes);
	}
	catch (const lsfm::Error& e)
	{
		fprintf(stderr, "liblsfm_hip: %s\n", e.msg.c_str());
		int code = e.code;
		delete c;
		return code;
	}
	*out = c;
	return LSFM_OK;
}

void lsfm_context_destroy(lsfm_context* c)
{
	if (!c) return;
	c->drop_prepared();
	c->worker.reset();
	(void)hipSetDevice(c->device);
	if (c->stream) (void)hipStreamSynchronize(c->stream);
	c->arena[0].destroy(); c->arena[1].destroy(); c->arena[2].destroy(); c->scratch.destroy();
	if (c->h_pinned) (void)hipHostFree(c->h_pinned);
	if (c->h_stage) (void)hipHostFree(c->h_stage);
	for (auto& e : c->ev_half) if (e) (void)hipEventDestroy(e);
	if (c->ev0) (void)hipEventDestroy(c->ev0);
	if (c->ev1) (void)hipEventDestroy(c->ev1);
	if (c->ev2) (void)hipEventDestroy(c->ev2);
	if (c->ev3) (void)hipEventDestroy(c->ev3);
	for (auto& e : c->evs) if (e) (void)hipEventDestroy(e);
	for (auto& e : c->ev_pool) if (e) (void)hipEventDestroy(e);
	if (c->d_run) (void)hipFree(c->d_run);
	if (c->stream) (void)hipStreamDestroy(c->stream);
	if (c->stream2) (void)hipStreamDestroy(c->stream2);
	if (c->stream3) (void)hipStreamDestroy(c->stream3);
	for (auto& e : c->ev_k9) if (e) (void)hipEventDestroy(e);
	if (c->evA) (void)hipEventDestroy(c->evA);
	if (c->evB) (void)hipEventDestroy(c->evB);
	if (c->evC) (void)hipEventDestroy(c->evC);
	if (c->evY) (void)hipEventDestroy(c->evY);
	if (c->evP) (void)hipEventDestroy(c->evP);
	if (c->evK) (void)hipEventDestroy(c->evK);
	if (c->evU) (void)hipEventDestroy(c->evU);
	c->pre.reset();
	c->sarena[0].destroy(); c->sarena[1].destroy();
	c->early.reset();
	delete c;
}

int lsfm_set_pcg(lsfm_context* ctx, double rel_tol, int max_steps)
{
	if (!ctx || !(rel_tol > 0) || max_steps > 50) return LSFM_ERR_ARG;
	ctx->pcg.rel_tol = rel_tol;
	ctx->pcg.max_steps = max_steps <= 0 ? 50 : max_steps;
	return LSFM_OK;
}

int lsfm_set_precision(lsfm_context* ctx, int mode)
{
	if (!ctx || (mode != 0 && mode != 1)) return LSFM_ERR_ARG;
	ctx->pcg.mixed = mode == 1;
	return LSFM_OK;
}

int lsfm_set_small_solve(lsfm_context* ctx, int max_poses)
{
	if (!ctx || max_poses < 0 || max_poses > 16) return LSFM_ERR_ARG;
	ctx->small_max = max_poses;
	return LSFM_OK;
}

int lsfm_set_spmv_variant(lsfm_context* ctx, int variant)
{
	if (!ctx || variant < 0 || variant > 2) return LSFM_ERR_ARG;
	ctx->pcg.spmv_variant = variant;
	return LSFM_OK;
}

int lsfm_set_covcols_panel(lsfm_context* ctx, int variant)
{
	if (!ctx || variant < 0 || variant > 2) return LSFM_ERR_ARG;
	ctx->covcols_panel = variant;
	return LSFM_OK;
}

const char* lsfm_last_error(lsfm_context* ctx) { return ctx ? ctx->last_error.c_str() : "null context"; }
void* lsfm_stream(lsfm_context* ctx) { return ctx ? (void*)ctx->stream : nullptr; }

}
```

### linearsfm_amd/csrc/lsfm_solve.hip

```cpp
#include <algorithm>
#include <cmath>

#include "lsfm_device.hpp"
#include "lsfm_internal.hpp"
#include "lsfm_solve.hpp"

namespace lsfm {

__global__ void __launch_bounds__(256) k_vinv(int NF, const double* __restrict__ V, const double* __restrict__ eb, double* __restrict__ IV, double* __restrict__ LY,
                                               double* __restrict__ ymax, RhsFused rhs, double* __restrict__ uu)
{
	__shared__ double wmax[4];
	int f = blockIdx.x * blockDim.x + threadIdx.x;
	double y2 = 0.0;
	if (f < NF)
	{
	double a[9], o[9];
	ld<9>(a, V + (size_t)f * 9);
	inv3_sym(a, o);
	st<9>(IV + (size_t)f * 9, o);
	const double* e = eb + (size_t)f * 3;
	double l[9];
	const double d0 = o[0];
	l[0] = sqrt(d0);
// ... 510 lines not shown
				const double* h = xhat + (size_t)photo[j] * 6;
#pragma unroll
				for (int r = 0; r < 6; r++) a6[r] -= h[r];
			}
#pragma unroll
			for (int c = 0; c < 3; c++)
			{
				double sacc = 0.0;
#pragma unroll
				for (int r = 0; r < 6; r++) sacc = fma(w[3 * r + c], a6[r], sacc);
				out[c] = sacc;
			}
		},
		[&](int fl, int q, double sum, bool) { sS[fl * 3 + q] += sum; });
	for (int fl = threadIdx.x; fl < nft; fl += blockDim.x)
	{
		const int f = f0 + fl;
		if (active && !active[feat_seg[f]]) continue;
		if (xhat)
		{
			const double* l = LY + (size_t)f * 9;
			const double s0 = sS[fl * 3], s1 = sS[fl * 3 + 1], s2 = sS[fl * 3 + 2];
			const double d0 = l[6] - (l[0] * s0 + l[1] * s1 + l[3] * s2), d1 = l[7] - (l[2] * s1 + l[4] * s2),
			             d2 = l[8] - l[5] * s2;
			xf[(size_t)f * 3] = l[0] * d0; xf[(size_t)f * 3 + 1] = l[1] * d0 + l[2] * d1; xf[(size_t)f * 3 + 2] = l[3] * d0 + l[4] * d1 + l[5] * d2;
			continue;
		}
		const double* iv = IV + (size_t)f * 9;
		const double d[3] = { eb[(size_t)f * 3] - sS[fl * 3], eb[(size_t)f * 3 + 1] - sS[fl * 3 + 1], eb[(size_t)f * 3 + 2] - sS[fl * 3 + 2] };
		for (int r = 0; r < 3; r++) xf[(size_t)f * 3 + r] = iv[3 * r] * d[0] + iv[3 * r + 1] * d[1] + iv[3 * r + 2] * d[2];
	}
}

__global__ void k_low_words(int n, const unsigned long long* __restrict__ keys, int* __restrict__ out)
{
	int i = blockIdx.x * blockDim.x + threadIdx.x;
	if (i < n) out[i] = (int)(keys[i] & 0xffffffffull);
}

void build_spmv_index(lsfm_context* ctx, SchurSystem& sy, const unsigned long long* sorted_upper)
{
	hipStream_t s = ctx->stream;
	Arena& sc = ctx->scratch;
	const int M = sy.M, cnt = sy.nnzb;
	if (!sy.rowptr)
	{
		sy.rowptr = sc.alloc<int>(M + 1);
		rowptr_from_keys(ctx, M, cnt, sorted_upper, sy.rowptr);
	}
	if (!sy.colidx)
	{
		sy.colidx = sc.alloc<int>(cnt + 1);
		if (cnt) hipLaunchKernelGGL(k_low_words, dim3((cnt + 255) / 256), dim3(256), 0, s, cnt, sorted_upper, sy.colidx);
	}
	int* nl = sc.alloc<int>(1);
	sy.longrows = sc.alloc<int>(M + 1);
	dev_zero(ctx, nl, sizeof(int));
	if (M) hipLaunchKernelGGL(k_spmv_long_rows, dim3((M + 255) / 256), dim3(256), 0, s, M, sy.rowptr, nl, sy.longrows);
	sy.d_nlong = nl;
	sy.gent = nullptr; sy.goth = nullptr;
	const int variant = ctx->pcg.spmv_variant;
	if (cnt && variant != 1 && (variant == 2 || (size_t)cnt * 288 <= SPMV_CACHED_BYTES))
	{
		unsigned long long* ent = sc.alloc<unsigned long long>((size_t)2 * cnt);
		int* oth = sc.alloc<int>((size_t)2 * cnt);
		hipLaunchKernelGGL(k_spmv_gather_keys, dim3((cnt + 255) / 256), dim3(256), 0, s, cnt, sorted_upper, ent, oth);
		int rb = 1;
		while ((1 << rb) <= M) rb++;
		dev_sort_pairs_u64(ctx, ent, oth, (size_t)2 * cnt, 32 + rb, 32);
		sy.gent = ent; sy.goth = oth;
	}
}

void schur_vinv(lsfm_context* ctx, const SolveIO& io, SchurSystem& sy)
{
	sy.IV = ctx->scratch.alloc<double>((size_t)io.NF * 9);
	sy.LY = ctx->scratch.alloc<double>((size_t)io.NF * 9);
	sy.ymax = ctx->scratch.alloc<double>((size_t)(io.NF + 255) / 256 + 1);
	sy.uu = nullptr;
	if (io.rhs) sy.uu = ctx->scratch.alloc<double>((size_t)io.NF * 6);
	if (io.NF) hipLaunchKernelGGL(k_vinv, dim3((io.NF + 255) / 256), dim3(256), 0, ctx->stream, io.NF, io.V, io.eb, sy.IV, sy.LY, sy.ymax, io.rhs ? *io.rhs : RhsFused(), sy.uu);
}

void build_schur_values(lsfm_context* ctx, const SolveIO& io, SchurSystem& sy)
{
	hipStream_t s = ctx->stream;
	Arena& sc = ctx->scratch;
	const int M = io.M, NF = io.NF, cnt = sy.nnzb;
	const unsigned long long* tab = sy.tab;
	const int* hval = sy.hval;
	const unsigned long long mask = sy.mask;
	const int ntiles = (NF + SCHUR_TILE - 1) / SCHUR_TILE;
	unsigned char* fb;
	const size_t nacc = 1 + (size_t)cnt * 36 + (size_t)M * 12;
	if (ctx->comm)
	{
		ctx->comm->restart();
		sy.acc = ctx->comm->alloc<long long>(nacc);
		sy.E = ctx->comm->alloc<double>((size_t)M * 6);
		fill_async(s, sy.acc, 0, nacc * sizeof(long long));
		ZeroSpan zs(sc);
		sy.S = sc.alloc<double>((size_t)cnt * 36);
		fb = sc.alloc<unsigned char>(ntiles + 1);
		zs.zero(s);
	}
	else
	{
		ZeroSpan zs(sc);
		sy.S = sc.alloc<double>((size_t)cnt * 36);
		fb = sc.alloc<unsigned char>(ntiles + 1);
		sy.acc = sc.alloc<long long>(nacc);
		zs.zero(s);
		sy.E = sc.alloc<double>((size_t)M * 6);
	}
	sy.sexp = sc.alloc<int>((size_t)M * 6 + 1);
	if (io.NU) hipLaunchKernelGGL(k_schur_u, dim3((io.NU + 255) / 256), dim3(256), 0, s, io.NU, io.U, io.Ui, io.Uj, tab, hval, mask, sy.S);
	hipLaunchKernelGGL(k_schur_scale, dim3((6 * M + 255) / 256 + 1), dim3(256), 0, s, M, sy.rowptr, sy.S, NF, NF ? (NF + 255) / 256 : 0, sy.ymax, io.d_fixed, sy.sexp, io.ea, sy.E);
	K9Out ko;
	ko.poison = sy.acc; ko.S = sy.acc + 1; ko.Ehi = ko.S + (size_t)cnt * 36; ko.Elo = ko.Ehi + (size_t)M * 6;
	ko.sexp = sy.sexp; ko.ey = sy.sexp + (size_t)M * 6;
	if (io.rhs) { ko.xpose = io.rhs->pose_src; ko.pside = io.rhs->pose_map_src; ko.uu = sy.uu; }
	if (NF)
	{
		hipEvent_t e2 = nullptr, e3 = nullptr;
		if (ctx->stats) { e2 = ctx->pool_event(); e3 = ctx->pool_event(); LSFM_REC_T(e2, s); }
		static_assert(LSFM_PM_TILE % SCHUR_TILE == 0, "a tile of the panel kernel must be whole tiles of the fallback kernel");
		bool fresh_lists = false;
		if (!sy.k9.ns)
		{
			fresh_lists = true;
			sy.k9.ns = sc.alloc<int>(ntiles + 1);
			sy.k9.pose = sc.alloc<int>((size_t)ntiles * 64 + 1);
			sy.k9.eslot = sc.alloc<unsigned char>((size_t)io.NW + 1);
			sy.k9.wlist = sc.alloc<int>((size_t)3 * ntiles + 1);
			sy.k9.wcnt = sc.alloc<int>(8);
			sy.k9_tiles = ntiles; sy.k9_NW = io.NW;
			launch_schur_slots(ctx, NF, io.fptr, io.photo, fb, sy.k9);
		}
		launch_schur_panel(ctx, NF, io.fptr, io.photo, io.W, sy.LY, tab, hval, mask, ko, fb, most_rows(io.seg_rows), sy.k9, fresh_lists);
		hipLaunchKernelGGL(k_schur_w, dim3(ntiles), dim3(SCHUR_TILE), 0, s, NF, io.fptr, io.photo, io.W, sy.IV, io.eb, tab, hval, mask, ko, fb, sy.LY);
		if (ctx->stats)
		{
			LSFM_REC_T(e3, s);
			ctx->defer_time(e2, e3, &ctx->stats->schur_ms);
			ctx->stats->schur_launches++;
			ctx->stats->schur_bytes += (double)io.NW * (144 + 4) + (double)io.NF * (72 + 24 + 4) + (double)sy.nnzb * 288 + (double)io.M * 48;
			ctx->stats->schur_flops += (double)io.NW * (144.0 + 108.0);
			if (io.rhs) { ctx->stats->schur_flops += (double)io.NW * 72.0; ctx->stats->schur_bytes += (double)io.NF * (48 + 24) + (double)io.M * 48; }
			if (ctx->in_tree_run && ctx->d_run)
			{
				LSFM_CHECK_HIP(hipEventRecord(ctx->ev_k9[0], s));
				LSFM_CHECK_HIP(hipStreamWaitEvent(ctx->stream2, ctx->ev_k9[0], 0));
				hipLaunchKernelGGL(k_sum_run_squares, dim3(std::min((NF + 255) / 256, 512)), dim3(256), 0, ctx->stream2, NF, io.fptr, &ctx->d_run->k2);
			}
		}
	}
	if (ctx->comm) ctx->comm->allreduce(s, sy.acc, 1 + (size_t)cnt * 36, LSFM_DTYPE_I64);
	{
		const size_t n = (size_t)cnt * 36 + (size_t)M * 6;
		hipLaunchKernelGGL(k_schur_finish, dim3((unsigned)((n + 255) / 256)), dim3(256), 0, s, cnt, M, sy.upper_keys, sy.acc, sy.sexp, sy.S, sy.E);
	}
	if (ctx->comm) ctx->comm->allreduce(s, sy.E, (size_t)M * 6, LSFM_DTYPE_F64);
	LSFM_CHECK_HIP(hipGetLastError());
}

void launch_spmv(lsfm_context* ctx, const SchurSystem& sy, const double* x, double* y, const unsigned char* fixed,
                 const double* dotw, const int* pose_seg, double* dot, int dot_stride)
{
	if (!sy.M) return;
	if (sy.gent)
	{
		const int nent = 2 * sy.nnzb;
		hipLaunchKernelGGL(k_spmv_gather, dim3((nent + SPG_ENT - 1) / SPG_ENT), dim3(256), 0, ctx->stream, sy.M, nent, sy.gent, sy.goth, sy.S, x, y, fixed,
		                   dotw, pose_seg, dot, dot_stride);
		return;
	}
	hipLaunchKernelGGL(k_spmv, dim3((sy.M + SPT - 1) / SPT), dim3(256), 0, ctx->stream, sy.M, sy.rowptr, sy.colidx, sy.d_nlong, sy.longrows, sy.S, x, y,
	                   fixed, dotw, pose_seg, dot, dot_stride);
}

double spmv_bytes(const SchurSystem& sy) { return (double)sy.nnzb * (288 + 4) + 4.0 * (sy.M + 1) + 2.0 * 48 * sy.M; }

void launch_backsub(lsfm_context* ctx, const SolveIO& io, const SchurSystem& sy, const double* x)
{
	if (io.NF)
		hipLaunchKernelGGL(k_backsub, dim3((io.NF + BSUB_TILE - 1) / BSUB_TILE), dim3(256), 0, ctx->stream, io.NF, io.fptr, io.photo, io.W, sy.IV, io.eb, x,
		                   io.d_feat_seg, io.d_seg_active, io.x_feat, sy.LY, io.rhs ? io.rhs->pose_src : (const double*)nullptr);
}

int inverse_v(lsfm_context* ctx, double* V, int n)
{
	ctx->ensure_arenas((size_t)n * 400 + ((size_t)64 << 20));
	ctx->arena[0].reset(); ctx->scratch.reset();
	double* dV = ctx->arena[0].alloc<double>((size_t)n * 9);
	double* dIV = ctx->arena[0].alloc<double>((size_t)n * 9);
	h2d(ctx, dV, V, (size_t)n * 9 * sizeof(double));
	if (n)
	{
		double* LY = ctx->scratch.alloc<double>((size_t)n * 9);
		double* eb = ctx->scratch.alloc<double>((size_t)n * 3);
		dev_zero(ctx, eb, (size_t)n * 3 * sizeof(double));
		hipLaunchKernelGGL(k_vinv, dim3((n + 255) / 256), dim3(256), 0, ctx->stream, n, dV, eb, dIV, LY, (double*)nullptr, RhsFused(), (double*)nullptr);
		LSFM_CHECK_HIP(hipStreamSynchronize(ctx->stream));
	}
	d2h(ctx, V, dIV, (size_t)n * 9 * sizeof(double));
	return LSFM_OK;
}
int solve_features(lsfm_context* ctx, const double* W, const double* IV, const double* eb, const double* dpa, double* dpb, int m, int n, const int* mapCor,
                   const int* photo)
{
	std::vector<int> fptr((size_t)n + 1, 0);
	for (int f = 0; f < n; f++)
	{
		if (mapCor[f] < 0) LSFM_FAIL(LSFM_ERR_ARG, "negative block count of a feature");
		fptr[f + 1] = fptr[f] + mapCor[f];
	}
	const int nW = fptr[n];
	for (int j = 0; j < nW; j++) if (photo[j] < 0 || photo[j] >= m) LSFM_FAIL(LSFM_ERR_ARG, "photo index out of range");
	ctx->ensure_arenas((size_t)nW * 200 + (size_t)n * 300 + (size_t)m * 100 + ((size_t)64 << 20));
	ctx->arena[0].reset(); ctx->scratch.reset();
	Arena& ar = ctx->arena[0];
	double* dW = ar.alloc<double>((size_t)nW * 18); int* dph = ar.alloc<int>(nW); int* dfp = ar.alloc<int>((size_t)n + 1);
	double* dIV = ar.alloc<double>((size_t)n * 9); double* deb = ar.alloc<double>((size_t)n * 3);
	double* dxp = ar.alloc<double>((size_t)m * 6); double* dxf = ar.alloc<double>((size_t)n * 3);
	h2d(ctx, dW, W, (size_t)nW * 18 * sizeof(double)); h2d(ctx, dph, photo, (size_t)nW * sizeof(int));
	h2d(ctx, dfp, fptr.data(), ((size_t)n + 1) * sizeof(int)); h2d(ctx, dIV, IV, (size_t)n * 9 * sizeof(double));
	h2d(ctx, deb, eb, (size_t)n * 3 * sizeof(double)); h2d(ctx, dxp, dpa, (size_t)m * 6 * sizeof(double));
	if (n)
		hipLaunchKernelGGL(k_backsub, dim3((n + BSUB_TILE - 1) / BSUB_TILE), dim3(256), 0, ctx->stream, n, dfp, dph, dW, dIV, deb, dxp,
		                   (const int*)nullptr, (const unsigned char*)nullptr, dxf, (const double*)nullptr, (const double*)nullptr);
	d2h(ctx, dpb, dxf, (size_t)n * 3 * sizeof(double));
	return LSFM_OK;
}

int spmv_external(lsfm_context* ctx, int m, const int* rowptr, const int* colidx, const double* val, const double* x, double* y, int reps,
                  double* avg_ms, double* bytes)
// ... 39 lines not shown
```

### linearsfm_amd/csrc/lsfm_solve.hpp

```cpp
#pragma once
#include "lsfm_device.hpp"
#include "lsfm_internal.hpp"

#ifndef LSFM_PM_TILE
#define LSFM_PM_TILE 128
#endif

namespace lsfm {

struct K9Cache {
	int* ns = nullptr;
	int* pose = nullptr;
	unsigned char* eslot = nullptr;
	int* wlist = nullptr;
	int* wcnt = nullptr;
};

struct SchurSystem {
	int M = 0, nnzb = 0;
	int *rowptr = nullptr, *colidx = nullptr;
	const unsigned long long* upper_keys = nullptr;
	double* S = nullptr;
	double* E = nullptr;
	double* IV = nullptr;
	double* LY = nullptr;
	int* longrows = nullptr;
	const int* d_nlong = nullptr;
	const unsigned long long* gent = nullptr;
	const int* goth = nullptr;
	const unsigned long long* tab = nullptr;
	const int* hval = nullptr;
	unsigned long long mask = 0;
	long long* acc = nullptr;
	int* sexp = nullptr;
	double* uu = nullptr;
	double* ymax = nullptr;
	K9Cache k9;
	int k9_tiles = 0, k9_NW = 0;
	double k9_flops = 0;
};

struct PatternSeed {
	const unsigned long long* prev_keys = nullptr;
	int prev_nnzb = 0;
	const int* pnew = nullptr;
	const unsigned char* dropped = nullptr;
	int NFY = 0;
	const int *srcE = nullptr, *srcC = nullptr;
	const int *fptr_in = nullptr, *photo_in = nullptr;
};
struct EarlyPatternIn {
	int M = 0, NFY = 0, NU = 0;
	const int *Ui = nullptr, *Uj = nullptr, *pose_map = nullptr, *hub = nullptr;
	const int *fptr = nullptr, *photo = nullptr, *feat_map = nullptr, *srcE = nullptr, *srcC = nullptr;
};
void build_schur_pattern(lsfm_context* ctx, const SolveIO& io, SchurSystem& sy);
void schur_pattern_only(lsfm_context* ctx, const SolveIO& io, int* nnzb, const int** rowptr, const int** colidx);
void schur_pattern_early_issue(lsfm_context* ctx, const EarlyPatternIn& in);
void schur_pattern_early_drop(lsfm_context* ctx);
bool schur_pattern_early_finish(lsfm_context* ctx, const SolveIO& io, SchurSystem& sy);
void schur_pattern_early_extras(lsfm_context* ctx, SchurSystem& sy);
bool schur_pattern_prefetch(lsfm_context* ctx, const DevBatch& Y, const int* d_tref, const unsigned long long* prev_keys, int prev_nnzb, SchurSystem& sy,
                            std::vector<int>* counts = nullptr, bool want_pattern = true, LevelIndex* keep = nullptr);
void schur_pattern_check(lsfm_context* ctx, const SolveIO& io, const SchurSystem& sy, const char* what);
void rowptr_from_keys(lsfm_context* ctx, int M, int cnt, const unsigned long long* sorted_upper, int* rowptr);

void build_schur_values(lsfm_context* ctx, const SolveIO& io, SchurSystem& sy);
void schur_vinv(lsfm_context* ctx, const SolveIO& io, SchurSystem& sy);
void build_spmv_index(lsfm_context* ctx, SchurSystem& sy, const unsigned long long* sorted_upper);
void launch_spmv(lsfm_context* ctx, const SchurSystem& sy, const double* x, double* y, const unsigned char* fixed, const double* dotw,
                 const int* pose_seg, double* dot, int dot_stride);
double spmv_bytes(const SchurSystem& sy);
void launch_schur_slots(lsfm_context* ctx, int NF, const int* fptr, const int* photo, unsigned char* fallback, K9Cache kc);
struct K9Out {
	long long* S = nullptr;
	long long *Ehi = nullptr, *Elo = nullptr;
	long long* poison = nullptr;
	const int* sexp = nullptr;
	const int* ey = nullptr;
	const double* xpose = nullptr;
	const int* pside = nullptr;
	const double* uu = nullptr;
};
struct RhsFused {
	const int *srcE = nullptr, *srcC = nullptr;
	const double* feat_src = nullptr;
	const double* pose_src = nullptr;
	const int* pose_map_src = nullptr;
};
void launch_schur_panel(lsfm_context* ctx, int NF, const int* fptr, const int* photo, const double* W, const double* LY,
                        const unsigned long long* tab, const int* val, unsigned long long mask, K9Out out, unsigned char* fallback,
                        int max_poses_per_system, K9Cache kc, bool fresh_lists = false);
void launch_backsub(lsfm_context* ctx, const SolveIO& io, const SchurSystem& sy, const double* x);

static const unsigned long long HEMPTY = ~0ull;
__device__ __forceinline__ unsigned long long mix64(unsigned long long x)
{
	x ^= x >> 33; x *= 0xff51afd7ed558ccdull; x ^= x >> 33; x *= 0xc4ceb9fe1a85ec53ull; x ^= x >> 33;
	return x;
}
__device__ __forceinline__ void hash_insert_mixed(unsigned long long* tab, unsigned long long mask, unsigned long long key, unsigned long long hm, int* overflow)
{
	unsigned long long h = hm & mask;
	for (int probe = 0; probe < 4096; probe++)
	{
		unsigned long long cur = tab[h];
		if (cur == key) return;
		if (cur == HEMPTY)
		{
			unsigned long long old = atomicCAS(&tab[h], HEMPTY, key);
			if (old == HEMPTY || old == key) return;
		}
		h = (h + 1) & mask;
	}
	*overflow = 1;
}
__device__ __forceinline__ void hash_insert(unsigned long long* tab, unsigned long long mask, unsigned long long key, int* overflow)
{
	hash_insert_mixed(tab, mask, key, mix64(key), overflow);
}
constexpr int PAIRSET_SLOTS = 2048;
constexpr int PAIRSET_PROBES = 8;
__device__ __forceinline__ void pairset_clear(unsigned long long* set)
{
	for (int i = threadIdx.x; i < PAIRSET_SLOTS; i += blockDim.x) set[i] = HEMPTY;
}
__device__ __forceinline__ void pairset_insert(unsigned long long* set, unsigned long long* tab, unsigned long long mask, unsigned long long key, int* overflow)
{
	const unsigned long long hm = mix64(key);
	unsigned s = (unsigned)(hm >> 40) & (PAIRSET_SLOTS - 1);
	for (int probe = 0; probe < PAIRSET_PROBES; probe++)
	{
		unsigned long long cur = set[s];
		if (cur == HEMPTY) cur = atomicCAS(&set[s], HEMPTY, key);
		if (cur == key) return;
		if (cur == HEMPTY) break;
		s = (s + 1) & (PAIRSET_SLOTS - 1);
	}
	hash_insert_mixed(tab, mask, key, hm, overflow);
}
__device__ __forceinline__ int hash_find(const unsigned long long* __restrict__ tab, const int* __restrict__ val, unsigned long long mask,
                                         unsigned long long key)
{
	unsigned long long h = mix64(key) & mask;
	for (int probe = 0; probe < 4096; probe++)
	{
		unsigned long long cur = tab[h];
		if (cur == key) return val[h];
		if (cur == HEMPTY) return -1;
		h = (h + 1) & mask;
// ... 10 lines not shown
```

### linearsfm_amd/csrc/lsfm_transform.hip

```cpp
#include <algorithm>
#include <climits>

#include "lsfm_device.hpp"
#include "lsfm_internal.hpp"

namespace lsfm {

struct TMap {
	int active, nh;
	int P0, m, F0, n;
	int U0, U0n, W0, W0n, kU0, kW0;
	int hub[2];
	int nref, nscap;
	int newFix, oldFix, newLabel;
	int c2fix, c3zero;
	int tref, tscap, oldref, oldscap;
	double R1[9], t1[3], scale1;
	int sign1;
	double R[9], dRA[9], dRB[9], dRG[9], t[3], dA[3], dB[3], dG[3];
	double Scale, Scale2, dSdA[3], dSdB[3], dSdG[3], dSdt[9], dSdtt[9];
};

__global__ void k_tr_find(const int* __restrict__ pose_id, const int* __restrict__ pose_map, int M, TMap* tm)
{
	int k = blockIdx.x * blockDim.x + threadIdx.x;
	if (k >= M) return;
	TMap& t = tm[pose_map[k]];
	if (!t.active) return;
	int id = pose_id[k];
	if (id == t.tref) t.nref = k;
	if (t.nh == 2)
	{
		if (id == t.tscap) t.nscap = k;
		if (id == t.oldref) t.hub[0] = k;
		if (id == t.oldscap) t.hub[1] = k;
	}
	else if (tr_stereo_hub(id, t.tref)) t.hub[0] = k;
}

__global__ void k_tr_params1(const double* __restrict__ pose, TMap* tm, int B, int* err)
{
	int b = blockIdx.x * blockDim.x + threadIdx.x;
	if (b >= B) return;
	TMap& t = tm[b];
	if (!t.active) return;
	if (t.nref < 0 || t.hub[0] < 0 || (t.nh == 2 && (t.nscap < 0 || t.hub[1] < 0))) { atomicExch(err, 1 + b); t.active = -1; return; }
	const double* p = pose + (size_t)t.nref * 6;
	t.t1[0] = p[0]; t.t1[1] = p[1]; t.t1[2] = p[2];
	rmat_ypr(t.R1, p[3], p[4], p[5]);
	t.scale1 = 1.0; t.sign1 = 1;
	if (t.nh == 2)
	{
		const double* q = pose + (size_t)t.nscap * 6;
		double d[3] = { q[0] - p[0], q[1] - p[1], q[2] - p[2] }, ts[3];
		mv3(t.R1, d, ts);
		t.scale1 = fabs(ts[t.newFix]);
		t.sign1 = ts[t.newFix] >= 0 ? 1 : -1;
		t.c2fix = (t.hub[0] == t.nscap);
		t.c3zero = (t.hub[1] == t.nref);
	}
}

__global__ void k_tr_new_poses(const double* __restrict__ pose, const int* __restrict__ pose_id, const int* __restrict__ pose_map,
                               int M, const TMap* __restrict__ tm, double* __restrict__ npose, int* __restrict__ npose_id)
{
	int k = blockIdx.x * blockDim.x + threadIdx.x;
	if (k >= M) return;
	const TMap& t = tm[pose_map[k]];
	const double* p = pose + (size_t)k * 6;
	double* o = npose + (size_t)k * 6;
	if (t.active <= 0)
	{
		for (int i = 0; i < 6; i++) o[i] = p[i];
		npose_id[k] = pose_id[k];
		return;
	}
	double R2[9], R3[9], a, b, g;
	if (t.nh == 1 && k == t.hub[0])
	{
		o[0] = -(t.R1[0] * t.t1[0] + t.R1[1] * t.t1[1] + t.R1[2] * t.t1[2]);
		o[1] = -(t.R1[3] * t.t1[0] + t.R1[4] * t.t1[1] + t.R1[5] * t.t1[2]);
		o[2] = -(t.R1[6] * t.t1[0] + t.R1[7] * t.t1[1] + t.R1[8] * t.t1[2]);
		inv_rmat_ypr_T(t.R1, a, b, g);
		o[3] = a; o[4] = b; o[5] = g;
		npose_id[k] = t.newLabel;
		return;
	}
	double d[3] = { p[0] - t.t1[0], p[1] - t.t1[1], p[2] - t.t1[2] }, v[3];
	mv3(t.R1, d, v);
	if (t.nh == 2) { v[0] = v[0] / t.scale1; v[1] = v[1] / t.scale1; v[2] = v[2] / t.scale1; }
	rmat_ypr(R2, p[3], p[4], p[5]);
	times_rrt(R3, R2, t.R1);
	inv_rmat_ypr(R3, a, b, g);
	o[0] = v[0]; o[1] = v[1]; o[2] = v[2]; o[3] = a; o[4] = b; o[5] = g;
	if (t.nh == 2)
	{
		if (k == t.nref) for (int i = 0; i < 6; i++) o[i] = 0.0;
		if (k == t.nscap) o[t.newFix] = (double)t.sign1;
	}
	npose_id[k] = pose_id[k];
}

__global__ void k_tr_params2(const double* __restrict__ npose, TMap* tm, int B, int* __restrict__ hub_out)
{
	int b = blockIdx.x * blockDim.x + threadIdx.x;
	if (b >= B) return;
	TMap& t = tm[b];
	if (hub_out) hub_out[b] = t.active > 0 ? t.hub[0] : -1;
	if (t.active <= 0) return;
	const double* p = npose + (size_t)t.hub[0] * 6;
	t.t[0] = p[0]; t.t[1] = p[1]; t.t[2] = p[2];
	r_derivation(p[3], p[4], p[5], t.R, t.dRA, t.dRB, t.dRG);
	ypr_rates<true>(t.dA, t.dRA, t.R); ypr_rates<true>(t.dB, t.dRB, t.R); ypr_rates<true>(t.dG, t.dRG, t.R);
	t.Scale = 1.0; t.Scale2 = 1.0;
	if (t.nh == 2)
	{
		const double* q = npose + (size_t)t.hub[1] * 6;
		double d[3] = { q[0] - p[0], q[1] - p[1], q[2] - p[2] }, ts[3];
		mv3(t.R, d, ts);
		t.Scale = fabs(ts[t.oldFix]);
		t.Scale2 = t.Scale * t.Scale;
		double Sign = ts[t.oldFix] >= 0 ? 1.0 : -1.0;
		for (int i = 0; i < 9; i++) { t.dSdt[i] = -t.R[i] * Sign; t.dSdtt[i] = t.R[i] * Sign; }
		mv3(t.dRA, d, t.dSdA); mv3(t.dRB, d, t.dSdB); mv3(t.dRG, d, t.dSdG);
		for (int i = 0; i < 3; i++) { t.dSdA[i] *= Sign; t.dSdB[i] *= Sign; t.dSdG[i] *= Sign; }
	}
}

__device__ __forceinline__ void mono_trans_jac(const TMap& t, const double* xn, double* dt2dt22, double* dt2dt, double* tmpc, double* dt2dtt)
{
	double t222[3] = { xn[0] - t.t[0], xn[1] - t.t[1], xn[2] - t.t[2] }, t22[3], v[3];
	const int mFix = t.oldFix;
	mv3(t.R, t222, t22);
	mv3(t.dRA, t222, v);
#pragma unroll
	for (int r = 0; r < 3; r++) tmpc[3 * r + 0] = (v[r] * t.Scale - t22[r] * t.dSdA[mFix]) / t.Scale2;
	mv3(t.dRB, t222, v);
#pragma unroll
	for (int r = 0; r < 3; r++) tmpc[3 * r + 1] = (v[r] * t.Scale - t22[r] * t.dSdB[mFix]) / t.Scale2;
	mv3(t.dRG, t222, v);
#pragma unroll
	for (int r = 0; r < 3; r++) tmpc[3 * r + 2] = (v[r] * t.Scale - t22[r] * t.dSdG[mFix]) / t.Scale2;
#pragma unroll
	for (int r = 0; r < 3; r++)
#pragma unroll
		for (int c = 0; c < 3; c++)
		{
			dt2dt22[3 * r + c] = t.R[3 * r + c] / t.Scale;
			dt2dt[3 * r + c] = (-t.R[3 * r + c] * t.Scale - t22[r] * t.dSdt[3 * mFix + c]) / t.Scale2;
			dt2dtt[3 * r + c] = (-t22[r] * t.dSdtt[3 * mFix + c]) / t.Scale2;
		}
}

template <int NH>
__global__ void __launch_bounds__(128, 1)
k_tr_pose_jac(const double* __restrict__ npose, const int* __restrict__ pose_map, int M, const TMap* __restrict__ tm,
                              double* __restrict__ Dp, double* __restrict__ Cp)
{
	int k = blockIdx.x * blockDim.x + threadIdx.x;
	if (k >= M) return;
	const TMap& t = tm[pose_map[k]];
	if (t.active <= 0 || t.nh != NH) return;
	double D[36], C1[36], C2[36];
	zero<36>(D); zero<36>(C1); zero<36>(C2);
	const double* p = npose + (size_t)k * 6;
	if (NH == 1 && k == t.hub[0])
	{
		double tmp1[3], tmp2[3], tmp3[3];
		mv3(t.dRA, t.t, tmp1); mv3(t.dRB, t.t, tmp2); mv3(t.dRG, t.t, tmp3);
#pragma unroll
		for (int r = 0; r < 3; r++)
		{
			D[6 * r + 0] = -t.R[3 * r]; D[6 * r + 1] = -t.R[3 * r + 1]; D[6 * r + 2] = -t.R[3 * r + 2];
			D[6 * r + 3] = -tmp1[r]; D[6 * r + 4] = -tmp2[r]; D[6 * r + 5] = -tmp3[r];
			D[6 * (3 + r) + 3] = t.dA[r]; D[6 * (3 + r) + 4] = t.dB[r]; D[6 * (3 + r) + 5] = t.dG[r];
		}
	}
	else
	{
		double R2[9], dRA2[9], dRB2[9], dRG2[9], Ri[9], dRi[9], ddA2[3], ddB2[3], ddG2[3], ddA[3], ddB[3], ddG[3];
		r_derivation(p[3], p[4], p[5], R2, dRA2, dRB2, dRG2);
		times_rrt(Ri, R2, t.R);
		times_rrt(dRi, dRA2, t.R); ypr_rates<false>(ddA2, dRi, Ri);
		times_rrt(dRi, dRB2, t.R); ypr_rates<false>(ddB2, dRi, Ri);
		times_rrt(dRi, dRG2, t.R); ypr_rates<false>(ddG2, dRi, Ri);
		times_rrt(dRi, R2, t.dRA); ypr_rates<false>(ddA, dRi, Ri);
		times_rrt(dRi, R2, t.dRB); ypr_rates<false>(ddB, dRi, Ri);
		times_rrt(dRi, R2, t.dRG); ypr_rates<false>(ddG, dRi, Ri);
// ... 634 lines not shown
                               int* __restrict__ nUj, double* __restrict__ PP)
{
	const int k0 = blockIdx.x * blockDim.x + threadIdx.x;
	const bool inb = k0 < M;
	const int k = inb ? k0 : 0;
	const int mp = pose_map[k];
	const TMap& t = tm[mp];
	const bool act = inb && t.active > 0 && t.nh == NH;
	double D[36];
	ld<36>(D, Dp + (size_t)k * 36);
	const int h0 = t.hub[0], h1 = NH == 2 ? t.hub[1] : -1;
	const int slot1 = t.U0n + (k - t.P0), slot2 = t.U0n + t.m + (k - t.P0);
	if (act)
	{
		if (k <= h0) { nUi[slot1] = k; nUj[slot1] = h0; } else { nUi[slot1] = h0; nUj[slot1] = k; }
		if (NH == 2) { if (k <= h0) { nUi[slot2] = k; nUj[slot2] = h1; } else { nUi[slot2] = h1; nUj[slot2] = k; } }
	}
#pragma unroll
	for (int s = 0; s < NH; s++)
	{
		double G[36], X[36];
		ld<36>(G, Gpose + (size_t)s * M * 36 + (size_t)k * 36);
		mtm<6, 6, 6, false>(D, G, X);
		const int hs = s == 0 ? h0 : h1;
		if (!act) {}
		else if (NH == 2 && s == 1 && k == h0)
		{
			double* dst = Un + (size_t)(t.U0n + (h1 - t.P0)) * 36;
			if (h0 < h1) { for (int q = 0; q < 36; q++) atomic_add_f64(dst + q, X[q]); }
			else { for (int i = 0; i < 6; i++) for (int j = 0; j < 6; j++) atomic_add_f64(dst + j * 6 + i, X[i * 6 + j]); }
		}
		else if (NH == 2 && s == 0 && k == h1)
		{
			double* dst = Un + (size_t)slot1 * 36;
			if (h1 < h0) { for (int q = 0; q < 36; q++) atomic_add_f64(dst + q, X[q]); }
			else { for (int i = 0; i < 6; i++) for (int j = 0; j < 6; j++) atomic_add_f64(dst + j * 6 + i, X[i * 6 + j]); }
		}
		else
		{
			double* dst = Un + (size_t)(s == 0 ? slot1 : slot2) * 36;
			add_oriented(dst, X, k, hs);
		}
#pragma unroll
		for (int s0 = 0; s0 <= s; s0++)
		{
			double C[36], P[36];
			ld<36>(C, Cp + (size_t)s0 * M * 36 + (size_t)k * 36);
			mtm<6, 6, 6, false>(C, G, P);
			const int idx = (s0 == 0 ? s : 2);
			wave_scatter_add<36>(PP + ((size_t)mp * 3 + idx) * 36, P, act);
		}
	}
}

template <int NH>
__global__ void k_tr_diag(int B, const TMap* __restrict__ tm, const double* __restrict__ PP, double* __restrict__ Un)
{
	int b = blockIdx.x * blockDim.x + threadIdx.x;
	if (b >= B) return;
	const TMap& t = tm[b];
	if (t.active <= 0 || t.nh != NH) return;
	const double* P = PP + (size_t)b * 3 * 36;
	double* d0 = Un + (size_t)(t.U0n + (t.hub[0] - t.P0)) * 36;
	for (int q = 0; q < 36; q++) d0[q] += P[q];
	if (NH == 2)
	{
		double* d2 = Un + (size_t)(t.U0n + t.m + (t.hub[1] - t.P0)) * 36;
		for (int q = 0; q < 36; q++) d2[q] += P[2 * 36 + q];
		double* d1 = Un + (size_t)(t.U0n + (t.hub[1] - t.P0)) * 36;
		const double* P01 = P + 36;
		if (t.hub[0] < t.hub[1]) { for (int q = 0; q < 36; q++) d1[q] += P01[q]; }
		else { for (int i = 0; i < 6; i++) for (int j = 0; j < 6; j++) d1[j * 6 + i] += P01[i * 6 + j]; }
	}
}

template <int NH>
static void launch_stage(lsfm_context* ctx, const DevBatch& in, DevBatch& out, const TMap* d_tm, const int* KU, const int* KW,
                         double* Dp, double* Cp, double* Gpose, double* PP, double nw_act_in, double nw_act_out, double nf_act,
                         const std::function<TrRedirect(DevBatch&)>* hook)
{
	hipStream_t s = ctx->stream;
	const int M = in.M;
	bool ev_entries = false, u_early = false;
	if (!in.NF && hook) (void)(*hook)(out);
	if (in.NF)
	{
		double* FD = ctx->scratch.alloc<double>((size_t)in.NF * (9 + 18 * NH));
		double* Gsum = ctx->scratch.alloc<double>((size_t)in.NF * 18 * NH);
		int* hubJ = ctx->scratch.alloc<int>((size_t)in.NF * NH);
		int4* finfo = ctx->scratch.alloc<int4>(in.NF);
		hipLaunchKernelGGL(k_tr_feat_pre<NH>, dim3((in.NF + 255) / 256), dim3(256), 0, s, in.NF, d_tm, in.feat_map, in.feat, in.fptr, in.V, KW, out.feat,
		                   out.fptr, out.V, FD, finfo, hubJ);
		TrRedirect rd;
		if (hook) rd = (*hook)(out);
		if (!rd.W) { rd = TrRedirect(); rd.wbase = out.fptr; rd.W = out.W; rd.photo = out.photo; rd.feature = out.feature; }
		if (!ctx->comm && in.NU)
		{
			LSFM_CHECK_HIP(hipEventRecord(ctx->evU, s));
			LSFM_CHECK_HIP(hipStreamWaitEvent(ctx->stream2, ctx->evU, 0));
			hipLaunchKernelGGL(k_tr_ublocks<NH>, dim3((in.NU + 127) / 128), dim3(128), 0, ctx->stream2, in.NU, M, d_tm, in.pose_map, in.U, in.Ui, in.Uj, KU,
			                   Dp, Cp, out.U, out.Ui, out.Uj, Gpose);
			u_early = true;
		}
		hipEvent_t e0 = nullptr, e1 = nullptr;
		if (ctx->stats) { e0 = ctx->pool_event(); e1 = ctx->pool_event(); LSFM_REC_T(e0, s); }
		hipLaunchKernelGGL(k_tr_entries<NH>, dim3((in.NF + TRE_TILE - 1) / TRE_TILE), dim3(TRE_ROUND), 0, s, in.NF, M, finfo, in.fptr, in.W,
		                   in.photo, KW, Dp, Cp, FD, rd.W, rd.photo, rd.feature, Gsum, Gpose, hubJ, out.W_alias ? 1 : 0, rd.wbase, rd.newf, rd.srcf);
		if (ctx->stats) LSFM_REC_T(e1, s);
		LSFM_CHECK_HIP(hipEventRecord(ctx->evA, s));
		ev_entries = true;
		hipLaunchKernelGGL(k_tr_feat_post<NH>, dim3((in.NF + 255) / 256), dim3(256), 0, s, in.NF, M, d_tm, in.feat_map, in.fptr, in.V, in.W, in.photo,
		                   Dp, FD, Gsum, hubJ, rd.wbase, rd.newf, rd.srcf, rd.W, rd.photo, rd.feature, PP);
		if (ctx->stats)
		{
			ctx->defer_time(e0, e1, &ctx->stats->trf_ms);
			ctx->stats->trf_launches++;
			const double nw_pass = (double)in.NW - nw_act_in;
			ctx->stats->trf_bytes += nw_act_in * (144 + 4 + 4) + nf_act * ((9 + 18 * NH) * 8 + 16 + 4) + (nw_act_out - NH * nf_act) * (144 + 8) +
			                         nf_act * 18 * NH * 8 + nw_pass * (4 + 8 + (out.W_alias ? 0 : 288)) + (double)(in.NF - nf_act) * (16 + 4);
		}
	}
	if (ctx->comm) ctx->comm->allreduce(s, Gpose, (size_t)M * 36 * NH + (size_t)in.B * 3 * 36, LSFM_DTYPE_F64);
	hipStream_t su = (ev_entries && !ctx->comm) ? ctx->stream2 : s;
	if (su != s) LSFM_CHECK_HIP(hipStreamWaitEvent(su, ctx->evA, 0));
	if (in.NU && !u_early)
		hipLaunchKernelGGL(k_tr_ublocks<NH>, dim3((in.NU + 127) / 128), dim3(128), 0, su, in.NU, M, d_tm, in.pose_map, in.U, in.Ui, in.Uj, KU,
		                   Dp, Cp, out.U, out.Ui, out.Uj, Gpose);
	if (M)
		hipLaunchKernelGGL(k_tr_poseslots<NH>, dim3((M + 127) / 128), dim3(128), 0, su, M, d_tm, in.pose_map, Dp, Cp, Gpose, out.U, out.Ui,
		                   out.Uj, PP);
	if (su != s)
	{
		LSFM_CHECK_HIP(hipEventRecord(ctx->evB, su));
		LSFM_CHECK_HIP(hipStreamWaitEvent(s, ctx->evB, 0));
	}
	hipLaunchKernelGGL(k_tr_diag<NH>, dim3((in.B + 127) / 128), dim3(128), 0, s, in.B, d_tm, PP, out.U);
}

__global__ void k_tr_patch(TMap* tm, const int4* __restrict__ offs, int B, int* __restrict__ fptr_last, int nw_total, const int* __restrict__ err, RunStatsDev* run)
{
	int b = blockIdx.x * blockDim.x + threadIdx.x;
	if (b == 0)
	{
		*fptr_last = nw_total;
		if (run && *err && !run->tr_err) run->tr_err = *err;
	}
	if (b >= B) return;
	const int4 o = offs[b];
	tm[b].kU0 = o.x; tm[b].kW0 = o.y; tm[b].U0n = o.z; tm[b].W0n = o.w;
}

__global__ void k_tr_sign_check(const TMap* __restrict__ tm, const int* __restrict__ planned, int B, RunStatsDev* run)
{
	int b = blockIdx.x * blockDim.x + threadIdx.x;
	if (b < B && tm[b].active > 0 && tm[b].sign1 != planned[b]) atomicExch(&run->plan_stale, 1);
}

int level_targets(const DevBatch& X, bool mono, std::vector<int>& tref, std::vector<int>& tscap, std::vector<int>& tfix)
{
	const int B = X.B;
	tref.assign(B, -1); tscap.assign(B, 0); tfix.assign(B, 0);
	int ntr = 0;
	for (int c = 1; c < B; c += 2)
	{
		const int e = c - 1;
		const bool re = X.Ref[c] > X.FRef[c];
		int cref = X.Ref[c], cscap = X.ScaP[c], cfix = X.Fix[c];
		if (re) { cref = X.FRef[c]; cscap = X.FScaP[c]; cfix = X.FFix[c]; tref[c] = cref; tscap[c] = cscap; tfix[c] = cfix; ntr++; }
		tref[e] = cref; tscap[e] = cscap; tfix[e] = cfix; ntr++;
	}
	for (int b = 0; b < B; b++) if (tref[b] >= 0 && map_in_frame(X, b, tref[b], tscap[b], mono)) tref[b] = -1;
	return ntr;
}

void transform_batch(lsfm_context* ctx, Arena& ar, const DevBatch& in, const std::vector<int>& target_ref,
                     const std::vector<int>& target_scap, const std::vector<int>& target_fix, bool mono, DevBatch& out,
                     bool alias_passthrough, const std::function<TrRedirect(DevBatch&)>* hook)
{
	hipStream_t s = ctx->stream;
	const int B = in.B, nh = mono ? 2 : 1;
	size_t smark = ctx->scratch.mark();
	std::vector<TMap> tm(B);
	for (int b = 0; b < B; b++)
	{
		TMap& t = tm[b];
		memset(&t, 0, sizeof t);
		t.nh = nh;
		t.P0 = in.pose_off[b]; t.m = in.pose_off[b + 1] - t.P0;
		t.F0 = in.feat_off[b]; t.n = in.feat_off[b + 1] - t.F0;
		t.U0 = in.u_off[b]; t.W0 = in.w_off[b];
		t.hub[0] = t.hub[1] = t.nref = t.nscap = -1;
		t.active = target_ref[b] >= 0 && !map_in_frame(in, b, target_ref[b], mono ? target_scap[b] : 0, mono);
		t.tref = target_ref[b]; t.tscap = mono ? target_scap[b] : 0; t.newFix = mono ? target_fix[b] : 0;
		t.oldref = in.Ref[b]; t.oldscap = mono ? in.ScaP[b] : 0; t.oldFix = mono ? in.Fix[b] : 0;
		t.newLabel = in.Ref[b];
	}
	TMap* d_tm = ctx->scratch.alloc<TMap>(B);
	int* d_err;
	double *Gpose, *PP;
	{
		const size_t ngp = (size_t)in.M * 36 * nh, npp = (size_t)B * 3 * 36;
		ZeroSpan zs(ctx->scratch);
		d_err = ctx->scratch.alloc<int>(1);
		if (ctx->comm)
		{
			ctx->comm->restart();
			Gpose = ctx->comm->alloc<double>(ngp + npp);
			PP = Gpose + ngp;
			fill_async(s, Gpose, 0, (ngp + npp) * sizeof(double));
		}
		else
		{
			Gpose = ctx->scratch.alloc<double>(ngp);
			PP = ctx->scratch.alloc<double>(npp);
		}
		zs.zero(s);
	}
	CopyBatch cb(ctx);
	cb.h2d(d_tm, tm.data(), sizeof(TMap) * B);

	out = DevBatch();
	out.B = B; out.M = in.M; out.NF = in.NF;
	if (mono) { out.s_keys = in.s_keys; out.s_nnzb = in.s_nnzb; }
	out.pose_off = in.pose_off; out.feat_off = in.feat_off;
	out.Ref = in.Ref; out.FRef = in.FRef; out.ScaP = in.ScaP; out.Fix = in.Fix; out.Sign = in.Sign; out.FScaP = in.FScaP; out.FFix = in.FFix;
	batch_set_offsets(ctx, ar, out, &cb);
	out.feat_id = ar.alloc<int>(in.NF);
	cb.d2d(out.feat_id, in.feat_id, (size_t)in.NF * sizeof(int));
	out.pose = ar.alloc<double>((size_t)in.M * 6);
	out.pose_id = ar.alloc<int>(in.M);
	out.pose_origin = ar.alloc<int>(in.M);
	cb.d2d(out.pose_origin, in.pose_origin, (size_t)in.M * sizeof(int));
	out.feat = ar.alloc<double>((size_t)in.NF * 3);
	out.V = ar.alloc<double>((size_t)in.NF * 9);
	out.fptr = ar.alloc<int>(in.NF + 1);
	int* d_uoff = ctx->scratch.alloc<int>(B + 1);
	int* d_woff = ctx->scratch.alloc<int>(B + 1);
	cb.h2d(d_uoff, in.u_off.data(), (B + 1) * sizeof(int));
	cb.h2d(d_woff, in.w_off.data(), (B + 1) * sizeof(int));
	cb.flush();
	batch_fill_maps(ctx, out);

	const int M = in.M;
	if (M)
	{
		hipLaunchKernelGGL(k_tr_find, dim3((M + 255) / 256), dim3(256), 0, s, in.pose_id, in.pose_map, M, d_tm);
		hipLaunchKernelGGL(k_tr_params1, dim3((B + 127) / 128), dim3(128), 0, s, in.pose, d_tm, B, d_err);
		hipLaunchKernelGGL(k_tr_new_poses, dim3((M + 255) / 256), dim3(256), 0, s, in.pose, in.pose_id, in.pose_map, M, d_tm, out.pose, out.pose_id);
		int* d_hub = (hook && !mono && B) ? ctx->scratch.alloc<int>(B) : nullptr;
		hipLaunchKernelGGL(k_tr_params2, dim3((B + 127) / 128), dim3(128), 0, s, out.pose, d_tm, B, d_hub);
		ctx->tr_in = nullptr; ctx->tr_hub = nullptr;
		if (d_hub) { ctx->tr_in = &in; ctx->tr_hub = d_hub; }
	}
	else { ctx->tr_in = nullptr; ctx->tr_hub = nullptr; }
	double* Dp = ctx->scratch.alloc<double>((size_t)M * 36);
	double* Cp = ctx->scratch.alloc<double>((size_t)M * 36 * nh + (nh == 1 ? (size_t)M * 27 : (size_t)M * 63));
	if (M)
	{
		if (mono) hipLaunchKernelGGL(k_tr_pose_jac<2>, dim3((M + 127) / 128), dim3(128), 0, s, out.pose, in.pose_map, M, d_tm, Dp, Cp);
		else hipLaunchKernelGGL(k_tr_pose_jac<1>, dim3((M + 127) / 128), dim3(128), 0, s, out.pose, in.pose_map, M, d_tm, Dp, Cp);
	}
	LevelPlan* plan = ctx->plan;
	const bool warm = ctx->warm();
	const int *KU = nullptr, *KW = nullptr;
	if (warm && plan->idx.KW && plan->idx.KU && plan->idx.NU == in.NU && plan->idx.NW == in.NW) { KU = plan->idx.KU; KW = plan->idx.KW; }
	else
	{
		int* keepU = ctx->scratch.alloc<int>(in.NU + 1);
		int* keepW = ctx->scratch.alloc<int>(in.NW + 1);
		int* kU = ctx->scratch.alloc<int>(in.NU + 2);
		int* kW = ctx->scratch.alloc<int>(in.NW + 2);
		int nmax = std::max(std::max(in.NU, in.NW), 1);
		hipLaunchKernelGGL(k_tr_flags, dim3((nmax + 255) / 256), dim3(256), 0, s, in.Ui, in.Uj, in.NU, in.photo, in.NW, in.pose_map, d_tm, keepU, keepW);
		dev_exclusive_scan(ctx, keepU, kU, in.NU);
		dev_exclusive_scan(ctx, keepW, kW, in.NW);
		KU = kU; KW = kW;
		if (plan && !warm && plan != &ctx->pre_plan && ctx->in_tree_run)
		{
			plan->idx.KU = level_index_keep(ctx, plan->idx, kU, (size_t)in.NU + 2);
			plan->idx.KW = level_index_keep(ctx, plan->idx, kW, (size_t)in.NW + 2);
			plan->idx.NU = in.NU; plan->idx.NW = in.NW;
		}
	}
	int* d_cnt = ctx->scratch.alloc<int>(3 * (B + 1));
	std::vector<int> cnt(2 * (B + 1)), dev_sign;
	if (warm) cnt = plan->tr_cnt;
	else
	{
		hipLaunchKernelGGL(k_tr_gather_counts, dim3((B + 1 + 127) / 128), dim3(128), 0, s, KU, KW, d_uoff, d_woff, B, d_cnt, d_tm, d_err);
		ctx->mark("tr_enq");
		std::vector<int> all(3 * (size_t)(B + 1));
		d2h_ints(ctx, d_cnt, all.data(), all.size());
		std::copy(all.begin(), all.begin() + 2 * (B + 1), cnt.begin());
		dev_sign.assign(all.begin() + 2 * (B + 1), all.begin() + 2 * (B + 1) + B);
		const int err = all[3 * (size_t)(B + 1) - 1];
		ctx->mark("tr_cnt");
		if (err) LSFM_FAIL(LSFM_ERR_ARG, "transform: target pose id not found in map " + std::to_string(err - 1));
		if (plan) plan->tr_cnt = cnt;
	}
	out.u_off.assign(B + 1, 0); out.w_off.assign(B + 1, 0);
	for (int b = 0; b < B; b++)
	{
		TMap& t = tm[b];
		t.kU0 = cnt[b]; t.kW0 = cnt[B + 1 + b];
		int keptU = cnt[b + 1] - cnt[b], keptW = cnt[B + 1 + b + 1] - cnt[B + 1 + b];
		t.U0n = out.u_off[b]; t.W0n = out.w_off[b];
		out.u_off[b + 1] = t.U0n + (t.active ? nh * t.m : 0) + keptU;
		out.w_off[b + 1] = t.W0n + (t.active ? nh * t.n : 0) + keptW;
		if (t.active)
		{
			out.Ref[b] = t.tref;
			if (mono) { out.ScaP[b] = t.tscap; out.Fix[b] = t.newFix; }
		}
	}
	out.NU = out.u_off[B]; out.NW = out.w_off[B];
	if (alias_passthrough && !in.W_alias && !hook)
	{
		std::vector<int> delta(B);
		for (int b = 0; b < B; b++) delta[b] = tm[b].active ? INT_MIN : in.w_off[b] - out.w_off[b];
		int* d_alias = ar.alloc<int>(B);
		h2d(ctx, d_alias, delta.data(), B * sizeof(int));
		out.d_alias = d_alias;
		out.W_alias = in.W;
	}
	{
		std::vector<int4> offs(B);
		for (int b = 0; b < B; b++) offs[b] = make_int4(tm[b].kU0, tm[b].kW0, tm[b].U0n, tm[b].W0n);
		int4* d_offs = ctx->scratch.alloc<int4>(B);
		h2d(ctx, d_offs, offs.data(), sizeof(int4) * B);
		hipLaunchKernelGGL(k_tr_patch, dim3(std::max(1, (B + 127) / 128)), dim3(128), 0, s, d_tm, d_offs, B, out.fptr + in.NF, out.NW, d_err, (warm && ctx->d_run) ? ctx->d_run : (RunStatsDev*)nullptr);
	}
	if (mono)
	{
		if (warm)
		{
			for (int b = 0; b < B; b++) if (tm[b].active) out.Sign[b] = plan->tr_sign[b];
			if (ctx->d_run)
			{
				int* d_sign = ctx->scratch.alloc<int>(B);
				h2d(ctx, d_sign, plan->tr_sign.data(), sizeof(int) * B);
				hipLaunchKernelGGL(k_tr_sign_check, dim3((B + 127) / 128), dim3(128), 0, s, d_tm, d_sign, B, ctx->d_run);
			}
		}
		else
		{
			for (int b = 0; b < B; b++) if (tm[b].active && dev_sign[b]) out.Sign[b] = dev_sign[b];
			if (plan) plan->tr_sign = out.Sign;
		}
	}
	out.U = ar.alloc<double>((size_t)out.NU * 36); out.Ui = ar.alloc<int>(out.NU); out.Uj = ar.alloc<int>(out.NU);
	if (!hook) { out.W = ar.alloc<double>((size_t)out.NW * 18); out.photo = ar.alloc<int>(out.NW); out.feature = ar.alloc<int>(out.NW); }
	dev_zero(ctx, out.U, (size_t)out.NU * 36 * sizeof(double));
	double nw_act_in = 0, nw_act_out = 0, nf_act = 0;
	for (int b = 0; b < B; b++)
		if (tm[b].active)
		{
			nw_act_in += in.w_off[b + 1] - in.w_off[b]; nw_act_out += out.w_off[b + 1] - out.w_off[b];
			nf_act += in.feat_off[b + 1] - in.feat_off[b];
		}
	if (mono) launch_stage<2>(ctx, in, out, d_tm, KU, KW, Dp, Cp, Gpose, PP, nw_act_in, nw_act_out, nf_act, hook);
	else launch_stage<1>(ctx, in, out, d_tm, KU, KW, Dp, Cp, Gpose, PP, nw_act_in, nw_act_out, nf_act, hook);
	ctx->mark("tr_done");
	LSFM_CHECK_HIP(hipGetLastError());
	ctx->tr_in = nullptr; ctx->tr_hub = nullptr;
	if (!warm && !hook && !ctx->in_tree_run) LSFM_CHECK_HIP(hipStreamSynchronize(s));
	if (!hook) ctx->scratch.release(smark);
}

}
```

### linearsfm_amd/csrc/lsfm_tree.hip

```cpp
#include <algorithm>
#include <cstdlib>
#include <cstring>

#include "lsfm_join.hpp"
#include "lsfm_tree.hpp"

namespace lsfm {

namespace {

bool level_plan(lsfm_context* ctx, lsfm_tree* t, int level)
{
	ctx->plan = (t->use_plans && level < (int)t->plans.size()) ? &t->plans[level] : nullptr;
	const bool analysing = !(ctx->plan && ctx->plan->valid);
	if (!ctx->plan && !t->mono && ctx->pre_plan.valid && ctx->pre_plan_level == level)
	{
		ctx->plan = &ctx->pre_plan;
		LSFM_CHECK_HIP(hipStreamWaitEvent(ctx->stream, ctx->evP, 0));
	}
	return analysing;
}

void level_gap(lsfm_context* ctx, hipEvent_t level_begin)
{
	static const bool gaps = getenv("LSFM_LEVEL_GAPS") != nullptr;
	if (gaps && ctx->ev_solve_end && ctx->in_tree_run) ctx->defer_time(ctx->ev_solve_end, level_begin, &ctx->dbg_gap_ms);
	ctx->ev_solve_end = nullptr;
}

void run_level(lsfm_context* ctx, lsfm_tree* t, lsfm_stats* st, int level)
{
	const bool analysing = level_plan(ctx, t, level);
	char rname[48];
	snprintf(rname, sizeof rname, "lsfm level %d (%d maps)", level, t->level.B);
	Range rlevel(rname);
	ctx->mark("level");
	if ((int)t->step_hint.size() <= level) t->step_hint.resize(level + 1, 0);
	ctx->step_hint = t->step_hint[level];
	ctx->steps_used = 0;
	DevBatch& X = t->level;
	const int npairs = X.B / 2;
	std::vector<int> tref, tscap, tfix;
	const int ntr = level_targets(X, t->mono, tref, tscap, tfix);
	hipEvent_t e_t0 = ctx->pool_event(), e_t1 = ctx->pool_event(), e_t2 = ctx->pool_event();
	LSFM_REC_T(e_t0, ctx->stream);
	level_gap(ctx, e_t0);
	const int so = t->slot < 0 ? 0 : (t->slot + 1) % 3, sm = t->slot < 0 ? 1 : (t->slot + 2) % 3;
	Arena& other = ctx->arena[so];
	Arena& mine = ctx->arena[sm];
	other.reset();
	mine.reset();
	DevBatch Xt, Y;
	const bool inject = ctx->inject_level == level;
	if (t->mono)
	{
		{ Range r("lsfm transform"); transform_batch(ctx, other, X, tref, tscap, tfix, true, Xt, true); }
		if (inject) LSFM_FAIL(LSFM_ERR_INTERNAL, "injected failure of this rank (LSFM_TEST_FAIL_RANK)");
		LSFM_REC_T(e_t1, ctx->stream);
		Range r("lsfm join + solve");
		join_batch_mono(ctx, mine, Xt, Y, nullptr, nullptr);
	}
	else
	{
		JoinState js;
		const size_t smark = ctx->scratch.mark();
		std::function<TrRedirect(DevBatch&)> hook = [&](DevBatch& mid) {
			join_stereo_prepare(ctx, mine, mid, Y, js);
			TrRedirect rd;
			rd.wbase = js.wbase; rd.newf = js.newf; rd.W = Y.W; rd.photo = Y.photo; rd.feature = Y.feature; rd.srcf = js.srcf;
			return rd;
		};
		{ Range r("lsfm transform"); transform_batch(ctx, other, X, tref, tscap, tfix, false, Xt, false, &hook); }
		if (inject) LSFM_FAIL(LSFM_ERR_INTERNAL, "injected failure of this rank (LSFM_TEST_FAIL_RANK)");
		LSFM_REC_T(e_t1, ctx->stream);
		Range r("lsfm join + solve");
		js.smark = smark;
		join_stereo_finish(ctx, Xt, Y, js, nullptr, nullptr);
		ctx->pre_plan = LevelPlan();
		ctx->pre_plan_level = -1;
		if (analysing && Y.B > 1 && !ctx->comm)
		{
			std::vector<int> nref, nscap, nfix;
			level_targets(Y, false, nref, nscap, nfix);
			prefetch_next_level(ctx, Y, nref, level + 1, level + 1 < (int)t->step_hint.size() ? t->step_hint[level + 1] : 0);
		}
		else ctx->drop_prepared();
	}
	LSFM_REC_T(e_t2, ctx->stream);
	if (ctx->steps_used > 0) t->step_hint[level] = ctx->steps_used;
	ctx->step_hint = 0;
	ctx->plan = nullptr;
	t->level = Y;
	t->slot = sm;
	if (st)
	{
		ctx->defer_time(e_t0, e_t1, &st->t_transform_ms);
		ctx->defer_time(e_t1, e_t2, &st->t_join_ms);
		st->levels++; st->joins += npairs; st->transforms += ntr;
	}
}

void tree_pass(lsfm_context* ctx, lsfm_tree* t, lsfm_stats* st)
{
	Range rrun("lsfm tree run");
	t->slot = -1;
	t->done = false;
	ctx->generation++;
	ctx->arena[0].reset(); ctx->arena[1].reset(); ctx->arena[2].reset(); ctx->scratch.reset();
	ctx->stage_off = 0;
	ctx->drop_prepared(); ctx->early.reset(); ctx->solved_keys = nullptr; ctx->solved_nnzb = 0;
	ctx->ev_solve_end = nullptr;
	LSFM_CHECK_HIP(hipMemsetAsync(ctx->d_run, 0, sizeof(RunStatsDev), ctx->stream));
	static const bool poison = getenv("LSFM_POISON") != nullptr;
	if (poison)
	{
		for (int i = 0; i < 3; i++) LSFM_CHECK_HIP(hipMemsetAsync(ctx->arena[i].base, 0xFF, ctx->arena[i].cap, ctx->stream));
		LSFM_CHECK_HIP(hipMemsetAsync(ctx->scratch.base, 0xFF, ctx->scratch.cap, ctx->stream));
		for (int i = 0; i < 2; i++) if (ctx->sarena[i].base) LSFM_CHECK_HIP(hipMemsetAsync(ctx->sarena[i].base, 0xFF, ctx->sarena[i].cap, ctx->stream));
	}
	t->level = t->input;
	const int nlev = tree_levels(t->N);
	if ((int)t->plans.size() != nlev + 1) t->plans.assign(nlev + 1, LevelPlan());
	int level = 0;
	while (t->level.B > 1 && (t->stop_level <= 0 || level < t->stop_level)) run_level(ctx, t, st, level++);
	DevBatch& X = t->level;
	if (t->final_reanchor && X.B == 1 && X.Ref[0] > X.FRef[0])
	{
		std::vector<int> tref(1, X.FRef[0]), tscap(1, X.FScaP[0]), tfix(1, X.FFix[0]);
		const int so = t->slot < 0 ? 0 : (t->slot + 1) % 3;
		Arena& other = ctx->arena[so];
		other.reset();
		DevBatch Xt;
		hipEvent_t e0 = ctx->pool_event(), e1 = ctx->pool_event();
		LSFM_REC_T(e0, ctx->stream);
		ctx->plan = t->use_plans ? &t->plans[nlev] : nullptr;
		transform_batch(ctx, other, X, tref, tscap, tfix, t->mono, Xt);
		if (ctx->plan) ctx->plan->valid = true;
		ctx->plan = nullptr;
		LSFM_REC_T(e1, ctx->stream);
		ctx->defer_time(e0, e1, &st->t_transform_ms);
		st->transforms++;
		t->level = Xt;
		t->slot = so;
	}
	LSFM_CHECK_HIP(hipStreamSynchronize(ctx->stream));
}

struct Inject { int level = -1; bool undone = false; };
Inject test_switches(const lsfm_context* ctx, int attempt)
{
	Inject inj;
	if (!ctx->comm) return inj;
	static const char* frank = getenv("LSFM_TEST_FAIL_RANK");
	static int injected = 0;
	if (frank && attempt == 0 && atoi(frank) == ctx->comm->rank && !injected++)
	{
		const char* kind = getenv("LSFM_TEST_FAIL_KIND");
		if (kind && !strcmp(kind, "undone")) inj.undone = true;
		else inj.level = getenv("LSFM_TEST_FAIL_LEVEL") ? atoi(getenv("LSFM_TEST_FAIL_LEVEL")) : 0;
	}
	return inj;
}

enum class Pass { DONE, AGAIN, AGAIN_GROWN };
Pass run_pass(lsfm_context* ctx, lsfm_tree* t, lsfm_stats* st, int attempt, int inject_level, std::unique_ptr<Error>& pass_error)
{
	ctx->inject_level = inject_level;
	try { tree_pass(ctx, t, st); }
	catch (const Error& e)
	{
		ctx->inject_level = -1;
		if (ctx->comm)
		{
			pass_error.reset(new Error(e));
			(void)hipStreamSynchronize(ctx->stream); (void)hipGetLastError();
			ctx->drop_prepared();
			return Pass::DONE;
		}
		if (e.code == LSFM_ERR_NOT_SPD && attempt < 3)
		{
			(void)hipStreamSynchronize(ctx->stream); (void)hipGetLastError();
			ctx->stats = st; ctx->plan = nullptr;
			t->step_hint.clear(); t->plans.clear();
			if (getenv("LSFM_DEBUG_CONV")) fprintf(stderr, "[lsfm conv] attempt %d: %s -- joining the tree again\n", attempt, e.msg.c_str());
			return Pass::AGAIN;
		}
		if (e.code != LSFM_ERR_OOM || !ctx->grow_arenas()) throw;
		if (getenv("LSFM_DEBUG")) fprintf(stderr, "[lsfm] arenas grown to %zu MiB each after: %s\n", ctx->arena_bytes >> 20, e.msg.c_str());
		return Pass::AGAIN_GROWN;
	}
	ctx->inject_level = -1;
	return Pass::DONE;
}

void print_timeline(const lsfm_context* ctx)
{
	double prev = ctx->timeline.empty() ? 0 : ctx->timeline[0].second;
	for (const auto& m : ctx->timeline)
	{
		if (!strcmp(m.first, "level")) fprintf(stderr, "\n[tl]");
		fprintf(stderr, " %s+%.0f", m.first, 1e3 * (m.second - prev));
		prev = m.second;
	}
	fprintf(stderr, "\n");
}

void exchange_flags(lsfm_context* ctx, lsfm_tree* t, RunStatsDev& rs, lsfm_stats* st, bool inject_undone, const Error* pass_error)
{
	Comm& cm = *ctx->comm;
	if (inject_undone) rs.undone++;
	if (pass_error)
	{
		bool there = false;
		try { there = cm.follow(ctx->stream); } catch (const Error&) { there = false; }
		if (!there) throw *pass_error;
	}
	cm.restart();
	long long* d_fl = cm.alloc<long long>(8);
	long long fl[8] = { rs.tr_err != 0, rs.chol_err != 0, rs.plan_stale != 0, rs.not_converged, rs.undone, st->not_converged, pass_error ? 1 : 0, 0 };
	LSFM_CHECK_HIP(hipMemcpyAsync(d_fl, fl, sizeof fl, hipMemcpyHostToDevice, ctx->stream));
	LSFM_CHECK_HIP(hipStreamSynchronize(ctx->stream));
	if (pass_error) cm.call(ctx->stream, (size_t)(reinterpret_cast<char*>(d_fl) - cm.buf), 8, LSFM_DTYPE_I64);
	else cm.allreduce(ctx->stream, d_fl, 8, LSFM_DTYPE_I64, Comm::KIND_FINAL);
	LSFM_CHECK_HIP(hipMemcpyAsync(fl, d_fl, sizeof fl, hipMemcpyDeviceToHost, ctx->stream));
	LSFM_CHECK_HIP(hipStreamSynchronize(ctx->stream));
	if (fl[0] && !rs.tr_err) rs.tr_err = 1;
	if (fl[1] && !rs.chol_err) rs.chol_err = 1;
	rs.plan_stale = fl[2] != 0;
	rs.not_converged = (int)((fl[3] + cm.world - 1) / cm.world);
	rs.undone = (int)((fl[4] + cm.world - 1) / cm.world);
	st->not_converged = (int)((fl[5] + cm.world - 1) / cm.world);
	if (pass_error || fl[6]) { t->plans.clear(); t->step_hint.clear(); }
	if (pass_error) throw *pass_error;
	if (fl[6]) LSFM_FAIL(LSFM_ERR_INTERNAL, "another rank of the feature-sharded run failed");
}

enum class Verdict { ACCEPT, AGAIN_WITHOUT_PLANS, AGAIN_WITHOUT_PLANS_AND_HINTS };
Verdict run_verdict(const RunStatsDev& rs, const lsfm_stats& st, int attempt)
{
	const bool more = attempt < 3;
	if (rs.tr_err) LSFM_FAIL(LSFM_ERR_ARG, "transform: target pose id not found in map " + std::to_string(rs.tr_err - 1));
	if (rs.chol_err && !more)
		LSFM_FAIL(LSFM_ERR_NOT_SPD, "Schur system is not positive definite (block column " + std::to_string(rs.chol_err - 1) + " of the factor)");
	if (rs.plan_stale)
	{
		if (!more) LSFM_FAIL(LSFM_ERR_INTERNAL, "level plans kept being reported stale");
		return Verdict::AGAIN_WITHOUT_PLANS;
	}
	if ((rs.chol_err || rs.not_converged || rs.undone || st.not_converged) && more) return Verdict::AGAIN_WITHOUT_PLANS_AND_HINTS;
	return Verdict::ACCEPT;
}

void run_attempts(lsfm_context* ctx, lsfm_tree* t, lsfm_stats* st)
{
	const double t_begin = now_ms();
	for (int attempt = 0;; attempt++)
	{
		memset(st, 0, sizeof *st);
		st->attempts = attempt + 1;
		ctx->timed.clear(); ctx->ev_next = 0;
		ctx->timeline_on = getenv("LSFM_TIMELINE") != nullptr;
		ctx->timeline.clear();
		ctx->mark("run");
		const Inject inj = test_switches(ctx, attempt);
		std::unique_ptr<Error> pass_error;
		const Pass pass = run_pass(ctx, t, st, attempt, inj.level, pass_error);
		if (pass == Pass::AGAIN_GROWN) attempt--;
		if (pass != Pass::DONE) continue;
		st->t_total_ms = now_ms() - t_begin;
		ctx->mark("end");
		if (ctx->timeline_on) print_timeline(ctx);
		RunStatsDev rs;
		LSFM_CHECK_HIP(hipStreamSynchronize(ctx->stream2));
		LSFM_CHECK_HIP(hipMemcpy(&rs, ctx->d_run, sizeof rs, hipMemcpyDeviceToHost));
		if (ctx->comm) exchange_flags(ctx, t, rs, st, inj.undone, pass_error.get());
		if (rs.floored && getenv("LSFM_DEBUG_CONV")) fprintf(stderr, "[lsfm conv] %d pivot(s) of the separators held at their lower bound in this run\n", rs.floored);
		const Verdict v = run_verdict(rs, *st, attempt);
		if (v == Verdict::ACCEPT)
		{
			st->not_converged += rs.not_converged;
			st->max_rel_residual = std::max(st->max_rel_residual, rs.max_rel_residual);
			st->upload_ms = t->upload_ms;
			st->schur_flops += 108.0 * (double)rs.k2;
			st->s_digest = rs.s_digest; st->factor_digest = rs.factor_digest; st->refactor_mismatch = rs.refactor_mismatch; st->s_rebuild_mismatch = rs.s_rebuild_mismatch;
			return;
		}
		if (v == Verdict::AGAIN_WITHOUT_PLANS_AND_HINTS)
		{
			if (rs.chol_err && getenv("LSFM_DEBUG_CONV")) fprintf(stderr, "[lsfm conv] attempt %d: pivot of block column %d far below zero, joining the tree again\n", attempt, rs.chol_err - 1);
			t->step_hint.clear();
		}
		t->plans.clear();
	}
}

}

int tree_run(lsfm_context* ctx, lsfm_tree* t, lsfm_stats* stats)
{
	lsfm_stats local;
	memset(&local, 0, sizeof local);
	lsfm_stats* st = stats ? stats : &local;
	ctx->stats = st;
	struct InRun { lsfm_context* c; InRun(lsfm_context* x, Comm* cm) : c(x) { c->in_tree_run = true; c->comm = cm; } ~InRun() { c->in_tree_run = false; c->comm = nullptr; } }
		in_run(ctx, t->comm.fn ? &t->comm : nullptr);
	LSFM_CHECK_HIP(hipStreamSynchronize(ctx->stream));
	try
	{
		run_attempts(ctx, t, st);
		ctx->flush_times();
		if (getenv("LSFM_LEVEL_GAPS")) { fprintf(stderr, "[lsfm] device idle between the levels of this run: %.3f ms\n", ctx->dbg_gap_ms); ctx->dbg_gap_ms = 0.0; }
	}
	catch (...) { ctx->stats = nullptr; throw; }
	ctx->stats = nullptr;
	t->done = true;
	t->generation = ctx->generation;
	return st->not_converged ? LSFM_NOT_CONVERGED : LSFM_OK;
}

}
```

Before: 31.74.

## Move PCG setup, Cholesky zeroing and k9 slot build onto side streams

Splits PCG workspace allocation from its setup, and launches the setup together with Cholesky value zeroing and the Schur k9 slot structure on secondary streams, joined back through events. The aim is to overlap these small launches and host-to-device copies with Schur assembly on the main stream. It also writes the transformed U directly into the join target, which avoids a device-to-device copy, and computes transform offsets from the cached plan before the kernels run. It drops a z-to-p copy in PCG by writing the preconditioner output straight into p. The cost is more cross-stream synchronisation and extra side-stream syncs on error paths, with a risk of ordering bugs.

```diff
diff --git a/linearsfm_amd/csrc/lsfm_chol.hip b/linearsfm_amd/csrc/lsfm_chol.hip
--- a/linearsfm_amd/csrc/lsfm_chol.hip
+++ b/linearsfm_amd/csrc/lsfm_chol.hip
@@ -1182,19 +1182,27 @@
 	d2h(ctx, in.keys.data(), sy.upper_keys, (size_t)nnzb * sizeof(unsigned long long));
 }
 
-void chol_alloc_values(lsfm_context* ctx, CholDev& ch)
+void chol_alloc_values(lsfm_context* ctx, CholDev& ch, bool zero)
 {
 	Arena& sc = ctx->scratch;
-	ch.L = sc.alloc<double>((size_t)ch.nnzL * 36); ch.Dinv = sc.alloc<double>((size_t)ch.M * 36);
+	static const bool digest = getenv("LSFM_FACTOR_DIGEST") != nullptr;
+	{
+		ZeroSpan zs(sc);
+		ch.L = sc.alloc<double>((size_t)ch.nnzL * 36);
+		ch.d_err = sc.alloc<int>(4);
+		ch.Lg = (ch.ngroups && digest) ? sc.alloc<double>((size_t)ch.nnzL * 36) : nullptr;
+		ch.zero0 = sc.base + zs.from; ch.zero_bytes = sc.off - zs.from;
+	}
+	if (ch.ngroups && !ch.Lg) ch.Lg = sc.alloc<double>((size_t)ch.nnzL * 36);
+	ch.Dinv = sc.alloc<double>((size_t)ch.M * 36);
 	ch.wv = sc.alloc<double>((size_t)ch.M * 6);
 	ch.diag0 = sc.alloc<double>((size_t)ch.M * 6);
 	ch.dscale = sc.alloc<double>((size_t)ch.M * 6);
-	ch.Lg = ch.ngroups ? sc.alloc<double>((size_t)ch.nnzL * 36) : nullptr;
-	dev_zero(ctx, ch.L, (size_t)ch.nnzL * 36 * sizeof(double));
-	static const bool digest = getenv("LSFM_FACTOR_DIGEST") != nullptr;
-	if (digest && ch.Lg) dev_zero(ctx, ch.Lg, (size_t)ch.nnzL * 36 * sizeof(double));
-	ch.d_err = sc.alloc<int>(1);
-	dev_zero(ctx, ch.d_err, sizeof(int));
+	if (zero) chol_zero_values(ctx, ch);
+}
+void chol_zero_values(lsfm_context* ctx, const CholDev& ch)
+{
+	fill_async(ctx->stream, ch.zero0, 0, ch.zero_bytes);
 }
 
 static size_t chol_task_lds(const CholDev& ch) { return (size_t)ch.task0_maxsize * CHOL_TASK_LDS_PER_COL + 8; }
diff --git a/linearsfm_amd/csrc/lsfm_chol.hpp b/linearsfm_amd/csrc/lsfm_chol.hpp
--- a/linearsfm_amd/csrc/lsfm_chol.hpp
+++ b/linearsfm_amd/csrc/lsfm_chol.hpp
@@ -44,6 +44,8 @@
 	double* diag0 = nullptr;
 	double* dscale = nullptr;
 	int* d_err = nullptr;
+	void* zero0 = nullptr;
+	size_t zero_bytes = 0;
 };
 
 struct OwnFilter {
@@ -68,7 +70,8 @@
 void chol_analyse(lsfm_context* ctx, const SchurSystem& sy, const CholHostIn& in, CholDev& ch);
 void chol_upload_index(lsfm_context* ctx, const CholSymbolic& sym, CholDev& ch);
 void chol_upload_symbolic(lsfm_context* ctx, const CholSymbolic& sym, CholDev& ch);
-void chol_alloc_values(lsfm_context* ctx, CholDev& ch);
+void chol_alloc_values(lsfm_context* ctx, CholDev& ch, bool zero = true);
+void chol_zero_values(lsfm_context* ctx, const CholDev& ch);
 void chol_scatter(lsfm_context* ctx, const SchurSystem& sy, const unsigned char* fixed, CholDev& ch);
 void chol_factor(lsfm_context* ctx, const SchurSystem& sy, const unsigned char* fixed, CholDev& ch, double* fwd_v = nullptr);
 void chol_merge_groups(lsfm_context* ctx, const CholDev& ch);
diff --git a/linearsfm_amd/csrc/lsfm_internal.hpp b/linearsfm_amd/csrc/lsfm_internal.hpp
--- a/linearsfm_amd/csrc/lsfm_internal.hpp
+++ b/linearsfm_amd/csrc/lsfm_internal.hpp
@@ -237,6 +237,10 @@
 	hipEvent_t evY = nullptr, evP = nullptr;
 	hipEvent_t evU = nullptr;
 	hipEvent_t evK = nullptr;
+	hipEvent_t ev_side[4] = { nullptr, nullptr, nullptr, nullptr };
+	bool side_k2 = false;
+	bool side_chains() const { return in_tree_run && !comm; }
+	void sync_side_streams();
 	const unsigned long long* solved_keys = nullptr;
 	int solved_nnzb = 0;
 	std::vector<std::pair<const char*, double>> timeline;
@@ -324,6 +328,8 @@
 	const int* newf = nullptr;
 	double* W = nullptr;
 	int *photo = nullptr, *feature = nullptr, *srcf = nullptr;
+	double* U = nullptr;
+	int *Ui = nullptr, *Uj = nullptr;
 };
 void transform_batch(lsfm_context* ctx, Arena& ar, const DevBatch& in, const std::vector<int>& target_ref,
                      const std::vector<int>& target_scap, const std::vector<int>& target_fix, bool mono, DevBatch& out,
diff --git a/linearsfm_amd/csrc/lsfm_join.hip b/linearsfm_amd/csrc/lsfm_join.hip
--- a/linearsfm_amd/csrc/lsfm_join.hip
+++ b/linearsfm_amd/csrc/lsfm_join.hip
@@ -381,7 +381,7 @@
 	int* srcf = st.srcf;
 	const std::vector<unsigned char>& seg_active = st.seg_active;
 	const std::vector<int>& seg_rows = st.seg_rows;
-	if (in.NU)
+	if (in.NU && in.U != out.U)
 	{
 		CopyBatch cu(ctx);
 		cu.d2d(out.U, in.U, (size_t)in.NU * 36 * sizeof(double));
diff --git a/linearsfm_amd/csrc/lsfm_level.hip b/linearsfm_amd/csrc/lsfm_level.hip
--- a/linearsfm_amd/csrc/lsfm_level.hip
+++ b/linearsfm_amd/csrc/lsfm_level.hip
@@ -199,7 +199,41 @@
 	double tw0 = 0, tw1 = 0;
 };
 static double wall_ms() { return std::chrono::duration<double, std::milli>(std::chrono::steady_clock::now().time_since_epoch()).count(); }
-static LevelStructure level_structure(lsfm_context* ctx, const SolveIO& io, SolvePlan* sp, PreLevel* pre, bool pending, hipEvent_t eb)
+static void level_side_chains(lsfm_context* ctx, const SolveIO& io, bool want_k9, bool beside_pattern, CholDev* ch_planned, PcgWork& w, K9Structure& ks)
+{
+	if (ctx->comm) want_k9 = false;
+	if (!ctx->comm) w = pcg_alloc(ctx, io);
+	if (want_k9) ks = schur_k9_alloc(ctx, io);
+	if (ch_planned) chol_alloc_values(ctx, *ch_planned, false);
+	const bool side = ctx->side_chains();
+	if (side) LSFM_CHECK_HIP(hipEventRecord(ctx->ev_side[0], ctx->stream));
+	auto setup = [&]() {
+		if (!ctx->comm) pcg_setup(ctx, io, w);
+		if (ch_planned) chol_zero_values(ctx, *ch_planned);
+	};
+	if (side)
+	{
+		hipStream_t& q = ctx->early ? ctx->stream2 : ctx->stream3;
+		LSFM_CHECK_HIP(hipStreamWaitEvent(q, ctx->ev_side[0], 0));
+		OnStream on(ctx, q);
+		setup();
+		LSFM_CHECK_HIP(hipEventRecord(ctx->ev_side[2], ctx->stream));
+		w.side = true;
+	}
+	else setup();
+	if (!want_k9) return;
+	if (side && !beside_pattern)
+	{
+		LSFM_CHECK_HIP(hipStreamWaitEvent(ctx->stream2, ctx->ev_side[0], 0));
+		OnStream on(ctx, ctx->stream2);
+		schur_k9_enqueue(ctx, io, ks);
+		LSFM_CHECK_HIP(hipEventRecord(ctx->ev_side[1], ctx->stream));
+		ks.side = true;
+	}
+	else schur_k9_enqueue(ctx, io, ks);
+}
+
+static LevelStructure level_structure(lsfm_context* ctx, const SolveIO& io, SolvePlan* sp, PreLevel* pre, bool pending, hipEvent_t eb, PcgWork& w)
 {
 	hipStream_t s = ctx->stream;
 	LevelStructure ls;
@@ -207,14 +241,17 @@
 	CholDev& ch = ls.ch;
 	const bool pattern_dep = ctx->pattern_dep;
 	ctx->pattern_dep = false;
+	K9Structure ks;
 	auto assemble = [&]() {
-		build_schur_values(ctx, io, sy);
+		build_schur_values(ctx, io, sy, &ks);
 		LSFM_REC_T(eb, s); if (roctx().mark) roctx().mark("lsfm factor + refine: begin");
 		LSFM_CHECK_HIP(hipEventRecord(ctx->evK, s));
 	};
 	if (sp || pending)
 	{
 		sy = pending ? pre->sy : sp->sy;
+		if (!pending) ch = sp->ch;
+		level_side_chains(ctx, io, !sy.k9.ns, false, pending ? nullptr : &ch, w, ks);
 		schur_vinv(ctx, io, sy);
 		assemble();
 		if (pending)
@@ -223,16 +260,17 @@
 			ctx->plan->solve = pre_plan_complete(ctx, *pre);
 			sp = ctx->plan->solve.get();
 			ctx->mark("sym_wait");
+			ch = sp->ch;
+			chol_alloc_values(ctx, ch);
 		}
 		ls.sp = sp;
-		ch = sp->ch;
-		chol_alloc_values(ctx, ch);
 		return ls;
 	}
+	if (pre && !(pre->M == io.M && !ctx->comm)) pre = nullptr;
+	level_side_chains(ctx, io, true, !pre && !(ctx->early && !ctx->comm) && pattern_dep && !ctx->comm, nullptr, w, ks);
 	schur_vinv(ctx, io, sy);
 	CholHostIn hin;
 	bool have = false;
-	if (pre && !(pre->M == io.M && !ctx->comm)) pre = nullptr;
 	if (pre)
 	{
 		schur_pattern_early_drop(ctx);
@@ -405,13 +443,14 @@
 	hipEvent_t ea = ctx->pool_event(), eb = ctx->pool_event(), ec = ctx->pool_event(), ed = ctx->pool_event();
 	LSFM_REC_T(ea, s); if (roctx().mark) roctx().mark("lsfm schur: begin");
 	if (strips) return solve_level_dense(ctx, io, strips, warm, eb, ec, ed);
-	LevelStructure ls = level_structure(ctx, io, sp, pre.get(), pending, eb);
+	PcgWork w;
+	LevelStructure ls = level_structure(ctx, io, sp, pre.get(), pending, eb, w);
 	pre.reset();
 	const SchurSystem& sy = ls.sy;
 	CholDev& ch = ls.ch;
 	sp = ls.sp;
 	const bool dbg = getenv("LSFM_DEBUG") != nullptr;
-	PcgWork w = pcg_begin(ctx, io, sy, ch);
+	pcg_begin(ctx, io, sy, ch, w);
 	if (ctx->stats && chol_distributed(ctx, ch)) { ctx->stats->dist_solves++; ctx->stats->dist_work_total += ch.work_total; ctx->stats->dist_work_shared += ch.work_shared; }
 	chol_scatter(ctx, sy, io.d_fixed, ch);
 	if (w.fused_fwd) chol_perm_in(ctx, ch, w.r, io.d_fixed, w.v);
diff --git a/linearsfm_amd/csrc/lsfm_pcg.hip b/linearsfm_amd/csrc/lsfm_pcg.hip
--- a/linearsfm_amd/csrc/lsfm_pcg.hip
+++ b/linearsfm_amd/csrc/lsfm_pcg.hip
@@ -151,28 +151,39 @@
 		       seg[g].done, seg[g].slow, seg[g].rr_prev / fin.ee, seg[g].thresh / fin.ee, fin.ee, seg[g].pAp, seg[g].rz[0], seg[g].rz[1]);
 }
 
-PcgWork pcg_begin(lsfm_context* ctx, const SolveIO& io, const SchurSystem& sy, const CholDev& ch)
-{
-	hipStream_t s = ctx->stream;
+PcgWork pcg_alloc(lsfm_context* ctx, const SolveIO& io)
+{
 	Arena& sc = ctx->scratch;
 	const int M = io.M, nseg = io.nseg;
 	PcgWork w;
 	w.d_misc = sc.alloc<int>(4);
+	w.seg = sc.alloc<PcgSeg>(2 * (size_t)nseg);
+	const size_t nscal = (size_t)M * 6;
+	w.r = sc.alloc<double>(nscal); w.z = ctx->comm ? ctx->comm->alloc<double>(nscal) : sc.alloc<double>(nscal); w.p = sc.alloc<double>(nscal);
+	w.Ap = sc.alloc<double>(nscal); w.v = sc.alloc<double>(nscal);
+	return w;
+}
+void pcg_setup(lsfm_context* ctx, const SolveIO& io, PcgWork& w)
+{
+	const int M = io.M, nseg = io.nseg;
 	std::vector<PcgSeg> hseg(2 * (size_t)nseg);
 	memset(hseg.data(), 0, sizeof(PcgSeg) * hseg.size());
 	for (int g = 0, row = 0; g < nseg; g++) { hseg[g].row0 = hseg[nseg + g].row0 = row; row += io.seg_rows[g]; }
-	w.seg = sc.alloc<PcgSeg>(hseg.size());
 	h2d(ctx, w.seg, hseg.data(), sizeof(PcgSeg) * hseg.size());
-	const size_t nscal = (size_t)M * 6;
-	w.r = sc.alloc<double>(nscal); w.z = ctx->comm ? ctx->comm->alloc<double>(nscal) : sc.alloc<double>(nscal); w.p = sc.alloc<double>(nscal);
-	w.Ap = sc.alloc<double>(nscal); w.v = sc.alloc<double>(nscal);
-	const unsigned nbe = (unsigned)((nscal + 255) / 256);
-	hipLaunchKernelGGL(k_x_init, dim3(std::max(1u, nbe)), dim3(256), 0, s, M, io.x0, io.d_fixed, io.x_pose, w.Ap, w.d_misc);
+	const unsigned nbe = (unsigned)(((size_t)M * 6 + 255) / 256);
+	hipLaunchKernelGGL(k_x_init, dim3(std::max(1u, nbe)), dim3(256), 0, ctx->stream, M, io.x0, io.d_fixed, io.x_pose, w.Ap, w.d_misc);
+	w.set_up = true;
+}
+void pcg_begin(lsfm_context* ctx, const SolveIO& io, const SchurSystem& sy, const CholDev& ch, PcgWork& w)
+{
+	hipStream_t s = ctx->stream;
+	const int M = io.M;
+	if (!w.set_up) { w = pcg_alloc(ctx, io); pcg_setup(ctx, io, w); }
+	if (w.side) LSFM_CHECK_HIP(hipStreamWaitEvent(s, ctx->ev_side[2], 0));
 	launch_spmv(ctx, sy, io.x_pose, w.Ap, io.d_fixed, nullptr, nullptr, nullptr, 1);
 	hipLaunchKernelGGL(k_pcg_resid, dim3((M + 127) / 128), dim3(128), 0, s, M, sy.E, w.Ap, io.d_pose_seg, io.d_fixed, w.r, w.seg, 1);
 	static const bool no_fused_fwd = getenv("LSFM_NO_FUSED_FWD") != nullptr;
 	w.fused_fwd = !ctx->pcg.mixed && !no_fused_fwd && ch.M > 0;
-	return w;
 }
 
 PcgResult pcg_run(lsfm_context* ctx, const SolveIO& io, const SchurSystem& sy, const CholDev& ch, PcgWork& w, const PcgSteps& steps)
@@ -186,8 +197,8 @@
 	PcgSeg* seg = w.seg;
 	int* d_misc = w.d_misc;
 	const bool mixed = ctx->pcg.mixed;
-	chol_apply(ctx, ch, r, v, z, io.d_fixed, io.d_pose_seg, &seg[0].rz[0], SEG_STRIDE, w.fused_fwd);
-	hipLaunchKernelGGL(k_copy, dim3(nbe), dim3(256), 0, s, nscal, z, p);
+	chol_apply(ctx, ch, r, v, ctx->comm ? z : p, io.d_fixed, io.d_pose_seg, &seg[0].rz[0], SEG_STRIDE, w.fused_fwd);
+	if (ctx->comm) hipLaunchKernelGGL(k_copy, dim3(nbe), dim3(256), 0, s, nscal, z, p);
 	const bool err_to_run = steps.deferred || (ctx->comm && ctx->d_run);
 	hipLaunchKernelGGL(k_pcg_start, dim3(nbs), dim3(128), 0, s, nseg, seg, io.d_seg_active, ctx->pcg.rel_tol, d_misc + 1, ch.d_err, err_to_run ? ctx->d_run : (RunStatsDev*)nullptr);
 
diff --git a/linearsfm_amd/csrc/lsfm_pcg.hpp b/linearsfm_amd/csrc/lsfm_pcg.hpp
--- a/linearsfm_amd/csrc/lsfm_pcg.hpp
+++ b/linearsfm_amd/csrc/lsfm_pcg.hpp
@@ -12,11 +12,15 @@
 	bool fused_fwd = false;
 	hipEvent_t es0 = nullptr, es1 = nullptr;
 	bool es_done = false;
+	bool set_up = false;
+	bool side = false;
 };
 struct PcgSteps { bool warm, deferred; int its; bool mixed; double rel_tol; };
 struct PcgResult { int its; bool planned; };
 
-PcgWork pcg_begin(lsfm_context* ctx, const SolveIO& io, const SchurSystem& sy, const CholDev& ch);
+PcgWork pcg_alloc(lsfm_context* ctx, const SolveIO& io);
+void pcg_setup(lsfm_context* ctx, const SolveIO& io, PcgWork& w);
+void pcg_begin(lsfm_context* ctx, const SolveIO& io, const SchurSystem& sy, const CholDev& ch, PcgWork& w);
 PcgResult pcg_run(lsfm_context* ctx, const SolveIO& io, const SchurSystem& sy, const CholDev& ch, PcgWork& w, const PcgSteps& steps);
 void pcg_final_residual(lsfm_context* ctx, const SolveIO& io, const SchurSystem& sy, PcgWork& w);
 __global__ void k_pcg_run_stats(int nseg, const PcgSeg* __restrict__ seg, RunStatsDev* run);
diff --git a/linearsfm_amd/csrc/lsfm_prims.hip b/linearsfm_amd/csrc/lsfm_prims.hip
--- a/linearsfm_amd/csrc/lsfm_prims.hip
+++ b/linearsfm_amd/csrc/lsfm_prims.hip
@@ -352,6 +352,12 @@
 bool no_timing_events() { static const bool v = getenv("LSFM_NO_TIMING_EVENTS") != nullptr; return v; }
 unsigned timing_event_flags() { return hipEventDisableSystemFence; }
 unsigned order_event_flags() { return hipEventDisableTiming | hipEventReleaseToDevice; }
+}
+void lsfm_context::sync_side_streams()
+{
+	if (stream2) (void)hipStreamSynchronize(stream2);
+	if (stream3) (void)hipStreamSynchronize(stream3);
+	side_k2 = false;
 }
 hipEvent_t lsfm_context::pool_event()
 {
@@ -507,6 +513,7 @@
 		LSFM_CHECK_HIP(hipEventCreateWithFlags(&c->evP, lsfm::order_event_flags()));
 		LSFM_CHECK_HIP(hipEventCreateWithFlags(&c->evK, lsfm::order_event_flags()));
 		LSFM_CHECK_HIP(hipEventCreateWithFlags(&c->evU, lsfm::order_event_flags()));
+		for (auto& e : c->ev_side) LSFM_CHECK_HIP(hipEventCreateWithFlags(&e, lsfm::order_event_flags()));
 		LSFM_CHECK_HIP(hipHostMalloc((void**)&c->h_pinned, 4096));
 		c->stage_size = (size_t)64 << 20;
 		LSFM_CHECK_HIP(hipHostMalloc((void**)&c->h_stage, c->stage_size));
@@ -542,6 +549,7 @@
 	c->worker.reset();
 	(void)hipSetDevice(c->device);
 	if (c->stream) (void)hipStreamSynchronize(c->stream);
+	c->sync_side_streams();
 	c->arena[0].destroy(); c->arena[1].destroy(); c->arena[2].destroy(); c->scratch.destroy();
 	if (c->h_pinned) (void)hipHostFree(c->h_pinned);
 	if (c->h_stage) (void)hipHostFree(c->h_stage);
@@ -564,6 +572,7 @@
 	if (c->evP) (void)hipEventDestroy(c->evP);
 	if (c->evK) (void)hipEventDestroy(c->evK);
 	if (c->evU) (void)hipEventDestroy(c->evU);
+	for (auto& e : c->ev_side) if (e) (void)hipEventDestroy(e);
 	c->pre.reset();
 	c->sarena[0].destroy(); c->sarena[1].destroy();
 	c->early.reset();
diff --git a/linearsfm_amd/csrc/lsfm_solve.hip b/linearsfm_amd/csrc/lsfm_solve.hip
--- a/linearsfm_amd/csrc/lsfm_solve.hip
+++ b/linearsfm_amd/csrc/lsfm_solve.hip
@@ -616,11 +616,34 @@
 	if (io.NF) hipLaunchKernelGGL(k_vinv, dim3((io.NF + 255) / 256), dim3(256), 0, ctx->stream, io.NF, io.V, io.eb, sy.IV, sy.LY, sy.ymax, io.rhs ? *io.rhs : RhsFused(), sy.uu);
 }
 
-void build_schur_values(lsfm_context* ctx, const SolveIO& io, SchurSystem& sy)
+K9Structure schur_k9_alloc(lsfm_context* ctx, const SolveIO& io)
+{
+	Arena& sc = ctx->scratch;
+	K9Structure ks;
+	if (!io.NF) return ks;
+	const int ntiles = (io.NF + SCHUR_TILE - 1) / SCHUR_TILE;
+	ks.fb = sc.alloc<unsigned char>(((size_t)ntiles + 1 + 15) & ~(size_t)15);
+	ks.k9.ns = sc.alloc<int>(ntiles + 1);
+	ks.k9.pose = sc.alloc<int>((size_t)ntiles * 64 + 1);
+	ks.k9.eslot = sc.alloc<unsigned char>((size_t)io.NW + 1);
+	ks.k9.wlist = sc.alloc<int>((size_t)3 * ntiles + 1);
+	ks.k9.wcnt = sc.alloc<int>(8);
+	ks.tiles = ntiles; ks.NW = io.NW;
+	return ks;
+}
+void schur_k9_enqueue(lsfm_context* ctx, const SolveIO& io, const K9Structure& ks)
+{
+	if (!ks.fb) return;
+	dev_zero(ctx, ks.fb, ((size_t)ks.tiles + 1 + 15) & ~(size_t)15);
+	launch_schur_slots(ctx, io.NF, io.fptr, io.photo, ks.fb, ks.k9);
+}
+
+void build_schur_values(lsfm_context* ctx, const SolveIO& io, SchurSystem& sy, const K9Structure* fresh)
 {
 	hipStream_t s = ctx->stream;
 	Arena& sc = ctx->scratch;
 	const int M = io.M, NF = io.NF, cnt = sy.nnzb;
+	if (fresh && (sy.k9.ns || !fresh->fb)) fresh = nullptr;
 	const unsigned long long* tab = sy.tab;
 	const int* hval = sy.hval;
 	const unsigned long long mask = sy.mask;
@@ -635,14 +658,14 @@
 		fill_async(s, sy.acc, 0, nacc * sizeof(long long));
 		ZeroSpan zs(sc);
 		sy.S = sc.alloc<double>((size_t)cnt * 36);
-		fb = sc.alloc<unsigned char>(ntiles + 1);
+		fb = fresh ? fresh->fb : sc.alloc<unsigned char>(ntiles + 1);
 		zs.zero(s);
 	}
 	else
 	{
 		ZeroSpan zs(sc);
 		sy.S = sc.alloc<double>((size_t)cnt * 36);
-		fb = sc.alloc<unsigned char>(ntiles + 1);
+		fb = fresh ? fresh->fb : sc.alloc<unsigned char>(ntiles + 1);
 		sy.acc = sc.alloc<long long>(nacc);
 		zs.zero(s);
 		sy.E = sc.alloc<double>((size_t)M * 6);
@@ -660,7 +683,13 @@
 		if (ctx->stats) { e2 = ctx->pool_event(); e3 = ctx->pool_event(); LSFM_REC_T(e2, s); }
 		static_assert(LSFM_PM_TILE % SCHUR_TILE == 0, "a tile of the panel kernel must be whole tiles of the fallback kernel");
 		bool fresh_lists = false;
-		if (!sy.k9.ns)
+		if (fresh)
+		{
+			fresh_lists = true;
+			sy.k9 = fresh->k9; sy.k9_tiles = fresh->tiles; sy.k9_NW = fresh->NW;
+			if (fresh->side) LSFM_CHECK_HIP(hipStreamWaitEvent(s, ctx->ev_side[1], 0));
+		}
+		else if (!sy.k9.ns)
 		{
 			fresh_lists = true;
 			sy.k9.ns = sc.alloc<int>(ntiles + 1);
@@ -686,6 +715,8 @@
 				LSFM_CHECK_HIP(hipEventRecord(ctx->ev_k9[0], s));
 				LSFM_CHECK_HIP(hipStreamWaitEvent(ctx->stream2, ctx->ev_k9[0], 0));
 				hipLaunchKernelGGL(k_sum_run_squares, dim3(std::min((NF + 255) / 256, 512)), dim3(256), 0, ctx->stream2, NF, io.fptr, &ctx->d_run->k2);
+				LSFM_CHECK_HIP(hipEventRecord(ctx->ev_side[3], ctx->stream2));
+				ctx->side_k2 = true;
 			}
 		}
 	}
diff --git a/linearsfm_amd/csrc/lsfm_solve.hpp b/linearsfm_amd/csrc/lsfm_solve.hpp
--- a/linearsfm_amd/csrc/lsfm_solve.hpp
+++ b/linearsfm_amd/csrc/lsfm_solve.hpp
@@ -65,7 +65,15 @@
 void schur_pattern_check(lsfm_context* ctx, const SolveIO& io, const SchurSystem& sy, const char* what);
 void rowptr_from_keys(lsfm_context* ctx, int M, int cnt, const unsigned long long* sorted_upper, int* rowptr);
 
-void build_schur_values(lsfm_context* ctx, const SolveIO& io, SchurSystem& sy);
+struct K9Structure {
+	K9Cache k9;
+	unsigned char* fb = nullptr;
+	int tiles = 0, NW = 0;
+	bool side = false;
+};
+K9Structure schur_k9_alloc(lsfm_context* ctx, const SolveIO& io);
+void schur_k9_enqueue(lsfm_context* ctx, const SolveIO& io, const K9Structure& ks);
+void build_schur_values(lsfm_context* ctx, const SolveIO& io, SchurSystem& sy, const K9Structure* fresh = nullptr);
 void schur_vinv(lsfm_context* ctx, const SolveIO& io, SchurSystem& sy);
 void build_spmv_index(lsfm_context* ctx, SchurSystem& sy, const unsigned long long* sorted_upper);
 void launch_spmv(lsfm_context* ctx, const SchurSystem& sy, const double* x, double* y, const unsigned char* fixed, const double* dotw,
diff --git a/linearsfm_amd/csrc/lsfm_transform.hip b/linearsfm_amd/csrc/lsfm_transform.hip
--- a/linearsfm_amd/csrc/lsfm_transform.hip
+++ b/linearsfm_amd/csrc/lsfm_transform.hip
@@ -101,9 +101,15 @@
 	npose_id[k] = pose_id[k];
 }
 
-__global__ void k_tr_params2(const double* __restrict__ npose, TMap* tm, int B, int* __restrict__ hub_out)
+__global__ void k_tr_params2(const double* __restrict__ npose, TMap* tm, int B, int* __restrict__ hub_out, int* __restrict__ fptr_last, int nw_total,
+                             const int* __restrict__ err, RunStatsDev* run)
 {
 	int b = blockIdx.x * blockDim.x + threadIdx.x;
+	if (b == 0 && fptr_last)
+	{
+		*fptr_last = nw_total;
+		if (run && *err && !run->tr_err) run->tr_err = *err;
+	}
 	if (b >= B) return;
 	TMap& t = tm[b];
 	if (hub_out) hub_out[b] = t.active > 0 ? t.hub[0] : -1;
@@ -904,7 +910,16 @@
 	hipStream_t s = ctx->stream;
 	const int M = in.M;
 	bool ev_entries = false, u_early = false;
-	if (!in.NF && hook) (void)(*hook)(out);
+	auto place_u = [&](const TrRedirect& rd) {
+		if (rd.U) { out.U = rd.U; out.Ui = rd.Ui; out.Uj = rd.Uj; }
+		dev_zero(ctx, out.U, (size_t)out.NU * 36 * sizeof(double));
+	};
+	if (!in.NF)
+	{
+		TrRedirect rd;
+		if (hook) rd = (*hook)(out);
+		place_u(rd);
+	}
 	if (in.NF)
 	{
 		double* FD = ctx->scratch.alloc<double>((size_t)in.NF * (9 + 18 * NH));
@@ -915,6 +930,7 @@
 		                   out.fptr, out.V, FD, finfo, hubJ);
 		TrRedirect rd;
 		if (hook) rd = (*hook)(out);
+		place_u(rd);
 		if (!rd.W) { rd = TrRedirect(); rd.wbase = out.fptr; rd.W = out.W; rd.photo = out.photo; rd.feature = out.feature; }
 		if (!ctx->comm && in.NU)
 		{
@@ -1046,6 +1062,28 @@
 	if (mono) { out.s_keys = in.s_keys; out.s_nnzb = in.s_nnzb; }
 	out.pose_off = in.pose_off; out.feat_off = in.feat_off;
 	out.Ref = in.Ref; out.FRef = in.FRef; out.ScaP = in.ScaP; out.Fix = in.Fix; out.Sign = in.Sign; out.FScaP = in.FScaP; out.FFix = in.FFix;
+	auto lay_out = [&](const std::vector<int>& cnt) {
+		out.u_off.assign(B + 1, 0); out.w_off.assign(B + 1, 0);
+		for (int b = 0; b < B; b++)
+		{
+			TMap& t = tm[b];
+			t.kU0 = cnt[b]; t.kW0 = cnt[B + 1 + b];
+			int keptU = cnt[b + 1] - cnt[b], keptW = cnt[B + 1 + b + 1] - cnt[B + 1 + b];
+			t.U0n = out.u_off[b]; t.W0n = out.w_off[b];
+			out.u_off[b + 1] = t.U0n + (t.active ? nh * t.m : 0) + keptU;
+			out.w_off[b + 1] = t.W0n + (t.active ? nh * t.n : 0) + keptW;
+			if (t.active)
+			{
+				out.Ref[b] = t.tref;
+				if (mono) { out.ScaP[b] = t.tscap; out.Fix[b] = t.newFix; }
+			}
+		}
+		out.NU = out.u_off[B]; out.NW = out.w_off[B];
+	};
+	LevelPlan* plan = ctx->plan;
+	const bool warm = ctx->warm();
+	const bool offsets_first = warm && in.M > 0 && plan->tr_cnt.size() == 2 * (size_t)(B + 1);
+	if (offsets_first) lay_out(plan->tr_cnt);
 	batch_set_offsets(ctx, ar, out, &cb);
 	out.feat_id = ar.alloc<int>(in.NF);
 	cb.d2d(out.feat_id, in.feat_id, (size_t)in.NF * sizeof(int));
@@ -1070,7 +1108,8 @@
 		hipLaunchKernelGGL(k_tr_params1, dim3((B + 127) / 128), dim3(128), 0, s, in.pose, d_tm, B, d_err);
 		hipLaunchKernelGGL(k_tr_new_poses, dim3((M + 255) / 256), dim3(256), 0, s, in.pose, in.pose_id, in.pose_map, M, d_tm, out.pose, out.pose_id);
 		int* d_hub = (hook && !mono && B) ? ctx->scratch.alloc<int>(B) : nullptr;
-		hipLaunchKernelGGL(k_tr_params2, dim3((B + 127) / 128), dim3(128), 0, s, out.pose, d_tm, B, d_hub);
+		hipLaunchKernelGGL(k_tr_params2, dim3((B + 127) / 128), dim3(128), 0, s, out.pose, d_tm, B, d_hub, offsets_first ? out.fptr + in.NF : (int*)nullptr,
+		                   out.NW, d_err, ctx->d_run);
 		ctx->tr_in = nullptr; ctx->tr_hub = nullptr;
 		if (d_hub) { ctx->tr_in = &in; ctx->tr_hub = d_hub; }
 	}
@@ -1082,8 +1121,6 @@
 		if (mono) hipLaunchKernelGGL(k_tr_pose_jac<2>, dim3((M + 127) / 128), dim3(128), 0, s, out.pose, in.pose_map, M, d_tm, Dp, Cp);
 		else hipLaunchKernelGGL(k_tr_pose_jac<1>, dim3((M + 127) / 128), dim3(128), 0, s, out.pose, in.pose_map, M, d_tm, Dp, Cp);
 	}
-	LevelPlan* plan = ctx->plan;
-	const bool warm = ctx->warm();
 	const int *KU = nullptr, *KW = nullptr;
 	if (warm && plan->idx.KW && plan->idx.KU && plan->idx.NU == in.NU && plan->idx.NW == in.NW) { KU = plan->idx.KU; KW = plan->idx.KW; }
 	else
@@ -1120,22 +1157,7 @@
 		if (err) LSFM_FAIL(LSFM_ERR_ARG, "transform: target pose id not found in map " + std::to_string(err - 1));
 		if (plan) plan->tr_cnt = cnt;
 	}
-	out.u_off.assign(B + 1, 0); out.w_off.assign(B + 1, 0);
-	for (int b = 0; b < B; b++)
-	{
-		TMap& t = tm[b];
-		t.kU0 = cnt[b]; t.kW0 = cnt[B + 1 + b];
-		int keptU = cnt[b + 1] - cnt[b], keptW = cnt[B + 1 + b + 1] - cnt[B + 1 + b];
-		t.U0n = out.u_off[b]; t.W0n = out.w_off[b];
-		out.u_off[b + 1] = t.U0n + (t.active ? nh * t.m : 0) + keptU;
-		out.w_off[b + 1] = t.W0n + (t.active ? nh * t.n : 0) + keptW;
-		if (t.active)
-		{
-			out.Ref[b] = t.tref;
-			if (mono) { out.ScaP[b] = t.tscap; out.Fix[b] = t.newFix; }
-		}
-	}
-	out.NU = out.u_off[B]; out.NW = out.w_off[B];
+	if (!offsets_first) lay_out(cnt);
 	if (alias_passthrough && !in.W_alias && !hook)
 	{
 		std::vector<int> delta(B);
@@ -1145,6 +1167,7 @@
 		out.d_alias = d_alias;
 		out.W_alias = in.W;
 	}
+	if (!offsets_first)
 	{
 		std::vector<int4> offs(B);
 		for (int b = 0; b < B; b++) offs[b] = make_int4(tm[b].kU0, tm[b].kW0, tm[b].U0n, tm[b].W0n);
@@ -1172,7 +1195,6 @@
 	}
 	out.U = ar.alloc<double>((size_t)out.NU * 36); out.Ui = ar.alloc<int>(out.NU); out.Uj = ar.alloc<int>(out.NU);
 	if (!hook) { out.W = ar.alloc<double>((size_t)out.NW * 18); out.photo = ar.alloc<int>(out.NW); out.feature = ar.alloc<int>(out.NW); }
-	dev_zero(ctx, out.U, (size_t)out.NU * 36 * sizeof(double));
 	double nw_act_in = 0, nw_act_out = 0, nf_act = 0;
 	for (int b = 0; b < B; b++)
 		if (tm[b].active)
diff --git a/linearsfm_amd/csrc/lsfm_tree.hip b/linearsfm_amd/csrc/lsfm_tree.hip
--- a/linearsfm_amd/csrc/lsfm_tree.hip
+++ b/linearsfm_amd/csrc/lsfm_tree.hip
@@ -45,6 +45,7 @@
 	hipEvent_t e_t0 = ctx->pool_event(), e_t1 = ctx->pool_event(), e_t2 = ctx->pool_event();
 	LSFM_REC_T(e_t0, ctx->stream);
 	level_gap(ctx, e_t0);
+	if (ctx->side_k2) { LSFM_CHECK_HIP(hipStreamWaitEvent(ctx->stream, ctx->ev_side[3], 0)); ctx->side_k2 = false; }
 	const int so = t->slot < 0 ? 0 : (t->slot + 1) % 3, sm = t->slot < 0 ? 1 : (t->slot + 2) % 3;
 	Arena& other = ctx->arena[so];
 	Arena& mine = ctx->arena[sm];
@@ -68,6 +69,7 @@
 			join_stereo_prepare(ctx, mine, mid, Y, js);
 			TrRedirect rd;
 			rd.wbase = js.wbase; rd.newf = js.newf; rd.W = Y.W; rd.photo = Y.photo; rd.feature = Y.feature; rd.srcf = js.srcf;
+			rd.U = Y.U; rd.Ui = Y.Ui; rd.Uj = Y.Uj;
 			return rd;
 		};
 		{ Range r("lsfm transform"); transform_batch(ctx, other, X, tref, tscap, tfix, false, Xt, false, &hook); }
@@ -173,18 +175,19 @@
 		if (ctx->comm)
 		{
 			pass_error.reset(new Error(e));
-			(void)hipStreamSynchronize(ctx->stream); (void)hipGetLastError();
+			(void)hipStreamSynchronize(ctx->stream); ctx->sync_side_streams(); (void)hipGetLastError();
 			ctx->drop_prepared();
 			return Pass::DONE;
 		}
 		if (e.code == LSFM_ERR_NOT_SPD && attempt < 3)
 		{
-			(void)hipStreamSynchronize(ctx->stream); (void)hipGetLastError();
+			(void)hipStreamSynchronize(ctx->stream); ctx->sync_side_streams(); (void)hipGetLastError();
 			ctx->stats = st; ctx->plan = nullptr;
 			t->step_hint.clear(); t->plans.clear();
 			if (getenv("LSFM_DEBUG_CONV")) fprintf(stderr, "[lsfm conv] attempt %d: %s -- joining the tree again\n", attempt, e.msg.c_str());
 			return Pass::AGAIN;
 		}
+		(void)hipStreamSynchronize(ctx->stream); ctx->sync_side_streams();
 		if (e.code != LSFM_ERR_OOM || !ctx->grow_arenas()) throw;
 		if (getenv("LSFM_DEBUG")) fprintf(stderr, "[lsfm] arenas grown to %zu MiB each after: %s\n", ctx->arena_bytes >> 20, e.msg.c_str());
 		return Pass::AGAIN_GROWN;
@@ -271,7 +274,7 @@
 		ctx->mark("end");
 		if (ctx->timeline_on) print_timeline(ctx);
 		RunStatsDev rs;
-		LSFM_CHECK_HIP(hipStreamSynchronize(ctx->stream2));
+		ctx->sync_side_streams();
 		LSFM_CHECK_HIP(hipMemcpy(&rs, ctx->d_run, sizeof rs, hipMemcpyDeviceToHost));
 		if (ctx->comm) exchange_flags(ctx, t, rs, st, inj.undone, pass_error.get());
 		if (rs.floored && getenv("LSFM_DEBUG_CONV")) fprintf(stderr, "[lsfm conv] %d pivot(s) of the separators held at their lower bound in this run\n", rs.floored);
@@ -311,7 +314,7 @@
 		ctx->flush_times();
 		if (getenv("LSFM_LEVEL_GAPS")) { fprintf(stderr, "[lsfm] device idle between the levels of this run: %.3f ms\n", ctx->dbg_gap_ms); ctx->dbg_gap_ms = 0.0; }
 	}
-	catch (...) { ctx->stats = nullptr; throw; }
+	catch (...) { ctx->stats = nullptr; (void)hipStreamSynchronize(ctx->stream); ctx->sync_side_streams(); throw; }
 	ctx->stats = nullptr;
 	t->done = true;
 	t->generation = ctx->generation;
```

New measurement: 32.02. About the same (+0.9%).
